# davide-coccomini/MINTIME-Multi-Identity-size-iNvariant-TIMEsformer-for-Video-Deepfake-Detection

Measured on AMD Instinct MI355X. Metric: clips/sec (8-frame, 2-identity, 224^2 crops) fwd+bwd, higher is better.
Workload: dtype f32; 1 GPU; config 3: EfficientNet-B0 + SizeInvariantTimeSformer(dim 512, depth 9, heads 8), B=32/GPU, 8 frames, 2 identities (identity-masked), 224x224 crops, random-init seeded weights (restored before every step), train-mode BN + drop-connect 0.2, step = fwd + BCE loss + bwd + SGD(lr .01, wd 1e-4); global_batch=32, frames=8, parallelism=dp1

## Files before the change

include/mintime_hip.h:

```cpp
#ifndef MINTIME_HIP_H
#define MINTIME_HIP_H
#include <stdint.h>
#ifdef __cplusplus
extern "C" {
#endif

#define MT_VERSION 121

int mt_version(void);
const char* mt_last_error(void);

int mt_set_deterministic(int on);
int mt_get_deterministic(void);
int mt_det_release(void* stream);
int mt_det_bn_sums(const float* x, const float* z, const float* mean_invstd, int64_t rows, int C, int mode, double* stats, void* stream);

typedef struct { int gin, gout, off; } mt_rowmap;

enum { MT_OP_NT = 0,
       MT_OP_NN = 1,
       MT_OP_TN = 2 };

enum { MT_PRO_NONE = 0, MT_PRO_BN_SWISH_GATE = 1, MT_PRO_BN_SWISH = 2, MT_PRO_AFFINE = 3,
       MT_PRO_BN_BWD = 4,
       MT_PRO_IM2COL = 5 };
enum { MT_BPRO_NONE = 0, MT_BPRO_BN_SWISH_GATE = 1, MT_BPRO_IM2COL = 2 };
enum { MT_EPI_STORE = 0, MT_EPI_BIAS_RES = 1, MT_EPI_GEGLU = 2, MT_EPI_STATS = 3, MT_EPI_ATOMIC = 4,
       MT_EPI_GEGLU_BWD = 5, MT_EPI_ACCUM = 6,
       MT_EPI_SE_RED = 7, MT_EPI_ACT_BWD = 8 };

typedef struct {
  int op, prologue, epilogue;
  const float* A; const float* B; float* C;
  int M, N, K;
  int64_t lda, ldb, ldc;
  mt_rowmap a_map, b_map, c_map;
  const float* bias;
  const float* R; int64_t ldr;
  const float* scale; const float* shift; const float* gate; int hw;
  float* C2; int64_t ldc2;
  double* stats; int stats_slots;
  int n_half;
  int split_k;
  const float* A2;
  int b_prologue; const float* b_scale; const float* b_shift; const float* b_gate; int b_hw;
  int conv_H, conv_W, conv_C, conv_Ho, conv_Wo, conv_k, conv_stride, conv_pad, conv_act;
  int conv_src_u8;
  float* col_sum;
  const void* b_planes;
  int64_t b_plane_stride;
  const float* e_scale; const float* e_shift;
  const float* e_gate; const float* e_dpool;
  const float* e_mi; int e_hw;
} mt_gemm_desc;

int mt_gemm(const mt_gemm_desc* d, void* stream);

int mt_gemm_set_split(int on);
int mt_gemm_get_split(void);

int mt_split_planes(const float* src, void* planes, int64_t n, void* stream);

int64_t mt_planes_elems(int rows, int cols);

int mt_split_planes_blk(const float* src, int64_t ld, int rows, int cols, void* planes, void* stream);

int mt_split_planes_blk_multi(const void* items, int count, int64_t total_blocks, void* stream);

int mt_bn_bwd_apply_planes(const float* du, const float* z, const float* kabc, void* planes, int rows, int C, void* stream);

typedef struct {
  int op;
  int epilogue;
  int M, N, K;
  const void* a_planes;
  const void* b_planes;
  float* C; int64_t ldc;
  const float* bias;
  const float* R; int64_t ldr;
  float* C2; int64_t ldc2;
  int n_half;
  float* col_sum;
  void* c_planes;
  int split_k;
  void* sk_workspace;
  int64_t sk_workspace_bytes;
  double* stats; int stats_slots;
} mt_gemm_planes_desc;

int mt_gemm_planes(const mt_gemm_planes_desc* d, void* stream);

int mt_mul_planes(const float* x, const float* m, void* planes, float* out, int rows, int cols, void* stream);
int mt_mul_add(const float* y, const float* m, const float* r, float* out, int64_t n, void* stream);
int mt_geglu_bwd(const float* dh, const float* m, const float* u, void* du_planes, float* du, int rows, int n_half, void* stream);
int64_t mt_gemm_planes_workspace_bytes(void);
int mt_gemm_planes_set_persist(int blocks_per_cu);


int mt_layernorm_fwd(const float* x, const float* gamma, const float* beta, float* y, float* stats,
                     int rows, int dim, float eps, void* y_planes, void* stream);

int mt_embed_fwd(float* x, const float* cls, const float* pos_emb, const float* size_emb,
                 const int64_t* positions, const int32_t* sizes, int B, int F, int n, int dim, int pos_rows, int size_rows,
                 int* err_flag, void* stream);

int mt_attn_fwd(const float* qkv, float* out, float* cls_att, const uint8_t* mask, const uint8_t* ident,
                int B, int H, int F, int n, int mode, float scale, void* out_planes, void* stream);

int mt_head_fwd(const float* x, const float* gamma, const float* beta, const float* w, const float* bias,
                float* logits, int B, int N, int dim, int classes, float eps, void* stream);


int mt_stem_conv_fwd(const void* x, int x_is_u8, const float* w, float* z, double* stats, int slots, int N, int H, int W,
                     void* stream);
int mt_stem_conv_fwd_valid(const void* x, int x_is_u8, const float* w, float* z, double* stats, int slots, int N, int H, int W,
                           void* stream);

int mt_dwconv_fwd(const float* zin, const float* scale, const float* shift, const float* w, float* zout,
                  double* stats, int slots, int N, int H, int W, int C, int k, int stride, int act, void* stream);
int mt_dwconv_rc_supported(int cin, int C, int k, int stride, int H);
int mt_dwconv_fwd_rc(const float* y, const float* we, int cin, const float* scale, const float* shift, const float* w, float* zout,
                     double* stats, int slots, int N, int H, int W, int C, int k, int stride, void* stream);
int mt_dwconv_fwd_planes(const float* zin, const float* scale, const float* shift, const float* w, void* planes, int N, int H,
                         int W, int C, int k, int stride, int act, void* stream);

int mt_bn_finalize(const double* stats, int slots, double count, const float* gamma, const float* beta,
                   float* running_mean, float* running_var, float* scale, float* shift, float* mean_invstd,
                   int C, float eps, float momentum, int training, void* stream);

int mt_se_pool_parts(int N, int HW, int C);
int mt_se_pool_fwd(const float* z, const float* scale, const float* shift, float* partial, int N, int HW, int C, int parts,
                   void* stream);

int mt_se_gate_fwd(const float* partial, int parts, const float* w1, const float* b1, const float* w2, const float* b2,
                   float* pooled, float* gate, float* hidden, int N, int C, int CS, void* stream);

int mt_bn_act_fwd(const float* z, const float* scale, const float* shift, const float* res, float* y,
                  int64_t rows, int C, int act, const float* rowscale, int rows_per_group, void* stream);

int mt_attn_aggregate(const float* space_att, const float* time_att, float* out, int BH, int N, int F,
                      float scale_factor, void* stream);

int mt_build_clip_inputs(const int* slots, const int* valid, const int* frames, const int* ratio, unsigned char* mask,
                         unsigned char* identities_mask, int* size_embedding, int64_t* positions, int B, int F,
                         int num_patches, int max_identities, int mask_mode, void* stream);


int mt_layernorm_bwd(const float* dy, const float* x, const float* stats, const float* gamma, float* dx,
                     float* dgamma, float* dbeta, int rows, int dim, int accumulate, float* dx_colsum, int skip_period,
                     const float* dx_in, void* stream);
int mt_layernorm_bwd_rows(const float* dy, const float* x, const float* stats, const float* gamma, float* dx, const float* dx_in,
                          int rows, int dim, void* dx_planes, void* stream);
int mt_layernorm_bwd_cols(const float* dy, const float* x, const float* stats, const float* dx_new, float* dgamma, float* dbeta,
                          float* dx_colsum, int skip_period, int rows, int dim, void* stream);

int mt_layernorm_bwd_rows_blocks(int rows);
int mt_layernorm_bwd_rows_sums(const float* dy, const float* x, const float* stats, const float* gamma, float* dx, const float* dx_in,
                               int rows, int dim, void* dx_planes, float* partials, int skip_period, void* stream);
int mt_layernorm_bwd_cols_reduce(const float* partials, int blocks, int dim, float* dgamma, float* dbeta, float* dx_colsum,
                                 void* stream);

int mt_colsum(const float* A, int64_t lda, mt_rowmap map, int M, int N, float* out, void* stream);

int mt_head_bwd(const float* dlogits, const float* x, const float* gamma, const float* beta, const float* w,
                float* dx, float* dgamma, float* dbeta, float* dw, float* dbias, int B, int N, int dim, int classes,
                float eps, void* stream);

int mt_embed_bwd(const float* dx, float* dcls, float* dpos_emb, float* dsize_emb, const int64_t* positions,
                 const int32_t* sizes, int B, int F, int n, int dim, int pos_rows, int size_rows, void* stream);

int mt_attn_bwd(const float* qkv, const float* dout, float* dqkv, const uint8_t* mask, const uint8_t* ident,
                int B, int H, int F, int n, int mode, float scale, void* dqkv_planes, void* stream);


int mt_bn_act_bwd(const float* din, const float* z, const float* scale, const float* shift,
                  const float* mean_invstd, const float* gate, const float* dpool, const float* rowscale,
                  float* dout, double* stats, int slots, int64_t rows, int C, int hw, int act, void* stream);

int mt_bn_bwd_finalize(const double* stats, int slots, double count, const float* gamma, const float* mean_invstd,
                       float* kabc, float* dgamma, float* dbeta, int C, int training, void* stream);

int mt_se_scratch_floats(int N, int C, int CS);
int mt_se_bwd(const float* da, const float* z, const float* scale, const float* shift, const float* gate,
              const float* hidden, const float* pooled, const float* w1, const float* w2, float* dgate,
              float* dpre2, float* dhid, float* dpooled, float* dw1, float* db1, float* dw2, float* db2, int N,
              int HW, int C, int CS, int parts, float* scratch, void* stream);

int mt_dwconv_bwd(const float* du, const float* z, const float* kabc, const float* w, const float* zin,
                  const float* scale_in, const float* shift_in, const float* mean_invstd_in, float* du_in,
                  double* stats_in, int slots, float* dw, int N, int H, int W, int C, int k, int stride,
                  int parts, int act, const float* res_pre, const float* res_post, void* stream);
int mt_dwconv_bwd_rc(const float* du, const float* z, const float* kabc, const float* w, const float* y, const float* we, int cin,
                     const float* scale_in, const float* shift_in, const float* mean_invstd_in, float* du_in, double* stats_in,
                     int slots, float* dw, int N, int H, int W, int C, int k, int stride, int parts, void* stream);
int mt_dwconv_bwd_res2(const float* du, const float* z, const float* kabc, const float* w, const float* zin,
                       const float* scale_in, const float* shift_in, const float* mean_invstd_in, float* du_in,
                       double* stats_in, int slots, float* dw, int N, int H, int W, int C, int k, int stride,
                       int parts, int act, const float* res_pre, const float* res_post, void* stream);

int mt_stem_conv_wgrad(const float* du, const float* z, const float* kabc, const void* x, int x_is_u8, float* dw, int N,
                       int H, int W, void* stream);
int mt_stem_conv_wgrad_valid(const float* du, const float* z, const float* kabc, const void* x, int x_is_u8, float* dw, int N,
                             int H, int W, void* stream);

int mt_conv1x1_wgrad_supported(int Cout, int Cin);
int mt_conv1x1_bwd_fused_supported(int Cout, int Cin);
int mt_se_stage_fused_supported(int Co, int C, int hw);
int mt_se_stage_fused(const float* du_p, const float* z_p, const float* kabc_p, const float* w_p, const float* z_d,
                      const float* scale_d, const float* shift_d, int mode, float* dgate, const float* gate, const float* dpooled,
                      const float* mean_invstd_d, float* du_d, double* stats, int slots, int64_t rows, int Co, int C, int hw,
                      void* stream);
int mt_conv1x1_bwd_fused(const float* du, const float* kabc, const float* x, const float* w, const float* res, float* dx,
                         float* dw, int64_t rows, int Cout, int Cin, void* stream);
int mt_conv1x1_wgrad(const float* du, const float* z, const float* kabc, const float* x, const float* sc, const float* sh,
                     const float* gate, int hw, float* dw, int64_t rows, int Cout, int Cin, void* stream);
int mt_conv1x1_wgrad_wide_supported(int Cout, int Cin);
int mt_conv1x1_wgrad_wide(const float* du, const float* z, const float* kabc, const float* x, const float* sc, const float* sh,
                          const float* gate, int hw, float* dw, int64_t rows, int Cout, int Cin, void* stream);

int mt_conv1x1_rows_supported(int Cin, int Cout, int amode);
int mt_conv1x1_rows_instance(int Cin, int Cout);
int mt_conv1x1_rows(const float* x, const float* x2, const float* w, int ldw, int w_transposed, const float* c0, const float* c1,
                    const float* c2, int hw, int amode, const float* res, float* out, double* stats, int slots, int64_t rows,
                    int Cin, int Cout, void* stream);

int mt_transpose_multi(const void* items, int count, int64_t total_tiles, void* stream);
int mt_bce_logits(const float* logits, const float* labels, float pos_weight, float* loss, float* dlogits, int n, void* stream);
int mt_sgd_multi(const void* items, int count, int64_t total_blocks, float lr, float weight_decay, void* stream);
int mt_adam_multi(const void* items, int count, int64_t total_blocks, float lr, float weight_decay, double beta1, double beta2,
                  float eps, float step_size, float bias_correction2_sqrt, int decoupled_weight_decay, void* stream);


int mt_conv_weight_pack(const float* w, float* out, int Co, int Ci, int k, int ld, int transpose, void* stream);
int mt_conv_weight_unpack_grad(const float* dwp, float* dw, int Co, int Ci, int k, int ld, void* stream);

int mt_maxpool_add_fwd(const float* z, const float* scale, const float* shift, const float* zs, const float* scale_s,
                       const float* shift_s, float* y, int N, int H, int W, int C, void* stream);
int mt_maxpool_bwd(const float* dy, const float* z, const float* scale, const float* shift, float* du, int N, int H,
                   int W, int C, void* stream);
int mt_maxpool_add_fwd_arg(const float* z, const float* scale, const float* shift, const float* zs, const float* scale_s,
                           const float* shift_s, float* y, uint8_t* arg, float* zmax, int N, int H, int W, int C, void* stream);
int mt_maxpool_bwd_arg(const float* dy, const uint8_t* arg, float* du, int N, int H, int W, int C, void* stream);
int mt_maxpool_bn_bwd_apply_planes(const float* dy, const uint8_t* arg, const float* z, const float* kabc, void* planes, int N, int H,
                                   int W, int C, void* stream);
int mt_bn_bwd_apply(const float* du, const float* z, const float* kabc, float* dz, int64_t rows, int C, void* stream);

int mt_bn_act_fwd_planes(const float* z, const float* scale, const float* shift, const float* res, float* y, int rows, int C, int act,
                         const float* rowscale, int rows_per_group, void* y_planes, void* stream);
int mt_bn_swish_gate_planes(const float* z, const float* scale, const float* shift, const float* gate, int hw, void* planes, int rows,
                            int C, void* stream);

int mt_baseline_head_fwd(const float* x, int layout, int n, int hw, int C, int m, const float* w1, const float* b1, const float* w2,
                         const float* b2, float* vc, float* pooled, float* part, float* logits, void* stream);
int mt_baseline_head_bwd(const float* dlogits, const float* pooled, const float* vc, int n, int hw, int C, int m, const float* w1,
                         const float* b1, const float* w2, float* dw1, float* db1, float* dw2, float* db2, float* dx, int layout,
                         float* work, void* stream);

typedef struct {
  int N, T, H, W, C;
  int To, Ho, Wo, K;
  int kt, kh, kw, st, sh, sw, pt, ph, pw;
  int64_t ldx, ldy;
} mt_conv3d_desc;
// ... 45 lines not shown
```

mintime-multi-identity-size-invariant-timesformer-for-video-deepfake-detection_amd/csrc/effnet_bwd.hip:

```cpp
#include "../../include/mintime_hip.h"
#include "common.hpp"
#include <type_traits>
#include "rc.hpp"
#include "det.hpp"
#include <stdlib.h>

using namespace mt;

namespace {

__device__ __forceinline__ float sigmoidf_(float x) { return __builtin_amdgcn_rcpf(1.0f + __expf(-x)); }
__device__ __forceinline__ float swishf_(float x) { return x * sigmoidf_(x); }
__device__ __forceinline__ float dswishf_(float u) { const float s = sigmoidf_(u); return s * (1.0f + u * (1.0f - s)); }

__device__ __forceinline__ float4 f4(float a, float b, float c, float d) { return make_float4(a, b, c, d); }
__device__ __forceinline__ float4 ld4(const float* p) { return *reinterpret_cast<const float4*>(p); }
__device__ __forceinline__ void st4(float* p, float4 v) { *reinterpret_cast<float4*>(p) = v; }
__device__ __forceinline__ float4 fma4(float4 a, float4 b, float4 c) {
  return f4(fmaf(a.x, b.x, c.x), fmaf(a.y, b.y, c.y), fmaf(a.z, b.z, c.z), fmaf(a.w, b.w, c.w));
}
__device__ __forceinline__ float4 mul4(float4 a, float4 b) { return f4(a.x * b.x, a.y * b.y, a.z * b.z, a.w * b.w); }
__device__ __forceinline__ float4 add4(float4 a, float4 b) { return f4(a.x + b.x, a.y + b.y, a.z + b.z, a.w + b.w); }

template <int ACT>
__device__ __forceinline__ float4 act4(float4 u) {
  if (ACT == 1) return f4(swishf_(u.x), swishf_(u.y), swishf_(u.z), swishf_(u.w));
  if (ACT == 2) return f4(fmaxf(u.x, 0.f), fmaxf(u.y, 0.f), fmaxf(u.z, 0.f), fmaxf(u.w, 0.f));
  return u;
}
template <int ACT>
__device__ __forceinline__ float4 dact4(float4 u) {
  if (ACT == 1) return f4(dswishf_(u.x), dswishf_(u.y), dswishf_(u.z), dswishf_(u.w));
  if (ACT == 2) return f4(u.x > 0.f ? 1.f : 0.f, u.y > 0.f ? 1.f : 0.f, u.z > 0.f ? 1.f : 0.f, u.w > 0.f ? 1.f : 0.f);
  return f4(1.f, 1.f, 1.f, 1.f);
}

__device__ __forceinline__ void reduce_stats(float* red, float4 s1, float4 s2, int cql, int pl, int CQB, int PB, int CQ,
                                             int C, double* stats, int slots) {
  if (pl < PB) {
    float* rr = red + (pl * CQB + cql) * 8;
    rr[0] = s1.x; rr[1] = s1.y; rr[2] = s1.z; rr[3] = s1.w;
    rr[4] = s2.x; rr[5] = s2.y; rr[6] = s2.z; rr[7] = s2.w;
  }
  __syncthreads();
  for (int i = threadIdx.x; i < CQB * 8; i += blockDim.x) {
    const int q = i >> 3, e = i & 7;
    const int cqq = blockIdx.y * CQB + q;
    if (cqq < CQ) {
      float v = 0.f;
      for (int p = 0; p < PB; ++p) v += red[(p * CQB + q) * 8 + e];
      const int ch = cqq * 4 + (e & 3), which = e >> 2;
      stat_add(stats + ((int64_t)(blockIdx.x % stat_slots(slots)) * 2 + which) * C + ch, stat_limb(slots, C), v);
    }
  }
}

__global__ __launch_bounds__(256) void bn_act_bwd_kernel(const float* __restrict__ din, const float* __restrict__ z,
                                                         const float* __restrict__ scale, const float* __restrict__ shift,
                                                         const float* __restrict__ mean_invstd, const float* __restrict__ gate,
                                                         const float* __restrict__ dpool, const float* __restrict__ rowscale,
                                                         float* __restrict__ dout, double* __restrict__ stats, int slots,
                                                         int64_t rows, int C, int hw, int act, int CQB, int PB) {
  extern __shared__ float red[];
  const int tid = threadIdx.x;
  const int cql = tid % CQB, pl = tid / CQB;
  const int CQ = C >> 2;
  const int cq = blockIdx.y * CQB + cql;
  float4 s1 = f4(0, 0, 0, 0), s2 = s1;
  if (pl < PB && cq < CQ) {
    const int c = cq * 4;
    const float4 sc = ld4(scale + c), sh = ld4(shift + c);
    const float4 mean = ld4(mean_invstd + c), istd = ld4(mean_invstd + C + c);
    const float inv_hw = 1.0f / (float)hw;
    for (int64_t r = (int64_t)blockIdx.x * PB + pl; r < rows; r += (int64_t)gridDim.x * PB) {
      const int n = (int)(r / hw);
      float4 d = ld4(din + r * C + c);
      const float4 zz = ld4(z + r * C + c);
      if (gate) {
        const float4 g = ld4(gate + (int64_t)n * C + c), dp = ld4(dpool + (int64_t)n * C + c);
        d = f4(fmaf(d.x, g.x, dp.x * inv_hw), fmaf(d.y, g.y, dp.y * inv_hw), fmaf(d.z, g.z, dp.z * inv_hw), fmaf(d.w, g.w, dp.w * inv_hw));
      }
      if (rowscale) { const float rs = rowscale[n]; d = f4(d.x * rs, d.y * rs, d.z * rs, d.w * rs); }
      if (act == 1) {
        const float4 u = fma4(zz, sc, sh);
        d = f4(d.x * dswishf_(u.x), d.y * dswishf_(u.y), d.z * dswishf_(u.z), d.w * dswishf_(u.w));
      } else if (act == 2) {
        const float4 u = fma4(zz, sc, sh);
        d = f4(u.x > 0.f ? d.x : 0.f, u.y > 0.f ? d.y : 0.f, u.z > 0.f ? d.z : 0.f, u.w > 0.f ? d.w : 0.f);
      }
      if (dout) st4(dout + r * C + c, d);
      const float4 xh = f4((zz.x - mean.x) * istd.x, (zz.y - mean.y) * istd.y, (zz.z - mean.z) * istd.z, (zz.w - mean.w) * istd.w);
      s1 = add4(s1, d);
      s2 = fma4(d, xh, s2);
    }
  }
  reduce_stats(red, s1, s2, cql, pl, CQB, PB, CQ, C, stats, slots);
}

__global__ __launch_bounds__(256) void bn_bwd_finalize_kernel(const double* __restrict__ stats, int slots, double count,
                                                              const float* __restrict__ gamma, const float* __restrict__ mean_invstd,
                                                              float* __restrict__ kabc, float* __restrict__ dgamma,
                                                              float* __restrict__ dbeta, int C, int training) {
  __shared__ double red[8][32][2];
  const int cl = threadIdx.x & 31, sg = threadIdx.x >> 5;
  const int c = blockIdx.x * 32 + cl;
  double a = 0.0, b = 0.0;
  if (c < C)
    for (int i = sg; i < stat_slots(slots); i += 8) {
      a += stat_get(stats + ((int64_t)i * 2) * C + c, stat_limb(slots, C));
      b += stat_get(stats + ((int64_t)i * 2 + 1) * C + c, stat_limb(slots, C));
    }
  red[sg][cl][0] = a; red[sg][cl][1] = b;
  __syncthreads();
  if (sg != 0 || c >= C) return;
  double s1 = 0.0, s2 = 0.0;
#pragma unroll
  for (int g = 0; g < 8; ++g) { s1 += red[g][cl][0]; s2 += red[g][cl][1]; }
  const float mean = mean_invstd[c], istd = mean_invstd[C + c];
  const float ka = gamma[c] * istd;
  float kb = 0.f, kc = 0.f;
  if (training) {
    const float c1 = (float)(s1 / count), c2 = (float)(s2 / count);
    kb = -ka * c2 * istd;
    kc = ka * c2 * istd * mean - ka * c1;
  }
  kabc[c] = ka; kabc[C + c] = kb; kabc[2 * C + c] = kc;
  if (dgamma) dgamma[c] += (float)s2;
  if (dbeta) dbeta[c] += (float)s1;
}

__global__ __launch_bounds__(256) void se_bwd_reduce_kernel(const float* __restrict__ da, const float* __restrict__ z,
                                                            const float* __restrict__ scale, const float* __restrict__ shift,
                                                            float* __restrict__ dgate, int HW, int C, int CQB, int PB) {
  extern __shared__ float red[];
  const int tid = threadIdx.x;
  const int cql = tid % CQB, pl = tid / CQB;
  const int cq = blockIdx.y * CQB + cql;
  const int CQ = C >> 2;
  const int n = blockIdx.x;
  float4 s = f4(0, 0, 0, 0);
  if (pl < PB && cq < CQ) {
    const float4 sc = ld4(scale + cq * 4), sh = ld4(shift + cq * 4);
    const int64_t base = (int64_t)n * HW * C + cq * 4;
    const int per = (HW + gridDim.z - 1) / gridDim.z;
    const int p_lo = blockIdx.z * per, p_hi = min(HW, p_lo + per);
    int p = p_lo + pl;
    for (; p + PB < p_hi; p += 2 * PB) {
      const float4 z0 = ld4(z + base + (int64_t)p * C), z1 = ld4(z + base + (int64_t)(p + PB) * C);
      const float4 d0 = ld4(da + base + (int64_t)p * C), d1 = ld4(da + base + (int64_t)(p + PB) * C);
      const float4 u0 = fma4(z0, sc, sh), u1 = fma4(z1, sc, sh);
      s = f4(fmaf(d0.x, swishf_(u0.x), s.x), fmaf(d0.y, swishf_(u0.y), s.y), fmaf(d0.z, swishf_(u0.z), s.z), fmaf(d0.w, swishf_(u0.w), s.w));
      s = f4(fmaf(d1.x, swishf_(u1.x), s.x), fmaf(d1.y, swishf_(u1.y), s.y), fmaf(d1.z, swishf_(u1.z), s.z), fmaf(d1.w, swishf_(u1.w), s.w));
    }
    for (; p < p_hi; p += PB) {
      const float4 u = fma4(ld4(z + base + (int64_t)p * C), sc, sh);
      const float4 d = ld4(da + base + (int64_t)p * C);
      s = f4(fmaf(d.x, swishf_(u.x), s.x), fmaf(d.y, swishf_(u.y), s.y), fmaf(d.z, swishf_(u.z), s.z), fmaf(d.w, swishf_(u.w), s.w));
    }
  }
  if (pl < PB) st4(red + (pl * CQB + cql) * 4, s);
  __syncthreads();
  if (pl == 0 && cq < CQ) {
    float4 t = f4(0, 0, 0, 0);
    for (int p = 0; p < PB; ++p) t = add4(t, ld4(red + (p * CQB + cql) * 4));
    float* out = dgate + (int64_t)n * C + cq * 4;
    if (gridDim.z == 1) {
      st4(out, t);
    } else {
      atomicAdd(out + 0, t.x); atomicAdd(out + 1, t.y); atomicAdd(out + 2, t.z); atomicAdd(out + 3, t.w);
    }
  }
}

constexpr int SE_SLAB = 128;
constexpr int SE_JW = 12;
__device__ __forceinline__ void se_load_slab(float* slab, const float* __restrict__ src, int count, int CS, int tid) {
  const int pitch = CS + 1;
  const float inv_cs = 1.0f / (float)CS;
  for (int e0 = tid; e0 < count; e0 += 256 * 8) {
    float v[8];
#pragma unroll
    for (int u = 0; u < 8; ++u) v[u] = src[min(e0 + 256 * u, count - 1)];
#pragma unroll
    for (int u = 0; u < 8; ++u) {
      const int e = e0 + 256 * u;
      const int r = (int)(((float)e + 0.5f) * inv_cs);
      if (e < count) slab[r * pitch + (e - r * CS)] = v[u];
    }
  }
}

__global__ __launch_bounds__(256) void se_bwd_slab_kernel(const float* __restrict__ dgate, const float* __restrict__ gate,
                                                          const float* __restrict__ w2, float* __restrict__ dpre2,
                                                          float* __restrict__ dh_part, int C, int CS) {
  extern __shared__ float sm[];
  float* dp2 = sm;
  float* slab = sm + SE_SLAB;
  const int n = blockIdx.x, sl = blockIdx.y, c0 = sl * SE_SLAB, tid = threadIdx.x, lane = tid & 63, wave = tid >> 6;
  const int rows = min(SE_SLAB, C - c0), pitch = CS + 1;
  if (tid < SE_SLAB) {
    float v = 0.f;
    if (tid < rows) {
      const float g = gate[(int64_t)n * C + c0 + tid];
      v = dgate[(int64_t)n * C + c0 + tid] * g * (1.0f - g);
      dpre2[(int64_t)n * C + c0 + tid] = v;
    }
    dp2[tid] = v;
  }
  se_load_slab(slab, w2 + (int64_t)c0 * CS, rows * CS, CS, tid);
  __syncthreads();
  const float d0 = dp2[lane], d1 = dp2[lane + 64];
// ... 189 lines not shown
        const float4 v = act4<ACT>(fma4(zraw, sc, sh));
        const bool ok = (pre_ok >> i) & 1u;
        st4(a_t + (iy * IWP + ix) * CC + f_q * 4, f4(ok ? v.x : 0.f, ok ? v.y : 0.f, ok ? v.z : 0.f, ok ? v.w : 0.f));
      }
    }
#pragma unroll
    for (int i = 0; i < ND; ++i) {
      const int pix = slot + i * NSL;
      if (pix < T * T) {
        const float4 v = fma4(ka, pdu[i], fma4(kb, pz[i], kc));
        const bool ok = (pd_ok >> i) & 1u;
        st4(dz_t + pix * CC + cq * 4, f4(ok ? v.x : 0.f, ok ? v.y : 0.f, ok ? v.z : 0.f, ok ? v.w : 0.f));
      }
    }
    __syncthreads();
    if (tile + tile_stride < ntiles) fetch(tile + tile_stride);
    if (worker) {
      for (int p = ps; p < T * T; p += PS) {
        const int oy = p / T, ox = p - oy * T;
        const float4 d = ld4(dz_t + p * CC + cq * 4);
        const float* arow = a_t + ((oy * S + kh) * IWP + ox * S) * CC + cq * 4;
#pragma unroll
        for (int kw = 0; kw < K; ++kw) acc[kw] = fma4(d, ld4(arow + kw * CC), acc[kw]);
      }
    }
  }
  __syncthreads();
  float* red = lds;
  if (worker) {
#pragma unroll
    for (int kw = 0; kw < K; ++kw) st4(red + (((ps * K + kh) * CQN + cq) * K + kw) * 4, acc[kw]);
  }
  __syncthreads();
  if (tid < K * CQN * K) {
    const int kw = tid % K, q = (tid / K) % CQN, khh = tid / (CQN * K);
    float4 t = f4(0, 0, 0, 0);
    for (int g = 0; g < PS; ++g) t = add4(t, ld4(red + (((g * K + khh) * CQN + q) * K + kw) * 4));
    const int c = c0 + q * 4, tp = khh * K + kw;
    if (det.vals) {
      const int rk = (int)tile0, jb = q * 4 * K * K + tp;
      det_put(det, chunk_id, rk, jb, t.x); det_put(det, chunk_id, rk, jb + K * K, t.y);
      det_put(det, chunk_id, rk, jb + 2 * K * K, t.z); det_put(det, chunk_id, rk, jb + 3 * K * K, t.w);
      if (rk == 0 && tid == 0) det_base(det, chunk_id, (int64_t)c0 * K * K);
    } else {
      atomicAdd(dw + (c + 0) * K * K + tp, t.x); atomicAdd(dw + (c + 1) * K * K + tp, t.y);
      atomicAdd(dw + (c + 2) * K * K + tp, t.z); atomicAdd(dw + (c + 3) * K * K + tp, t.w);
    }
  }
}

template <int K, int S, int T, int ACT, int CC, int RC = 0>
int launch_dw_wgrad_tiled(const float* du, const float* z, const float* kabc, const float* zin, const float* scale_in,
                          const float* shift_in, float* dw, int N, int H, int W, int C, int Ho, int Wo, hipStream_t s,
                          const float* we = nullptr) {
  constexpr int IH = (T - 1) * S + K;
  constexpr int IWP = IH | 1;
  constexpr int CQN = CC / 4;
  constexpr int PS = (256 / CQN) / K;
  size_t lds = (size_t)(IH * IWP * CC + T * T * CC) * sizeof(float);
  const size_t red = (size_t)PS * K * CQN * K * 4 * sizeof(float);
  if (red > lds) lds = red;
  const int chunks = C / CC;
  const int64_t ntiles = (int64_t)N * ((Ho + T - 1) / T) * ((Wo + T - 1) / T);
  const unsigned bx = xcd_chunk_grid(chunks, ntiles, 4096);
  auto k = dwconv_wgrad_tiled_kernel<K, S, T, ACT, CC, RC>;
  if (lds > 48 * 1024) {
    hipError_t e = ensure_dynamic_lds(reinterpret_cast<const void*>(k), lds);
    if (e != hipSuccess) return fail(MT_ERR_LAUNCH, "mt_dwconv_bwd: cannot reserve %zu B of LDS: %s", lds, hipGetErrorString(e));
  }
  DetScope det(s, chunks, (int)((bx >> 3) / chunks) * 8, CC * K * K);
  hipLaunchKernelGGL(k, dim3(bx), dim3(256), lds, s, du, z, kabc, zin, scale_in, shift_in, dw, N, H, W, C, Ho, Wo, det.log, we);
  const int rc = check_launch("mt_dwconv_bwd(weight, tiled)");
  return rc ? rc : det.reduce_f32(dw);
}

thread_local int g_res_stride = 1;

template <int K, int S, int T, int ACT, int CC, bool WG = false, int RC = 0>
__global__ __launch_bounds__(256) void dwconv_dgrad_tiled_kernel(
    const float* __restrict__ du, const float* __restrict__ z, const float* __restrict__ kabc, const float* __restrict__ w,
    const float* __restrict__ zin, const float* __restrict__ scale_in, const float* __restrict__ shift_in,
    const float* __restrict__ mi_in, float* __restrict__ du_in, double* __restrict__ stats, int slots, int N, int H, int W,
    int C, int Ho, int Wo, const float* __restrict__ res_pre, const float* __restrict__ res_post, float* __restrict__ dw,
    int res_stride, const float* __restrict__ we) {
  static_assert(RC == 0 || CC == 16, "the recompute yields 16-channel chunks");
  constexpr int P = S == 1 ? (K - 1) / 2 : (K - 2) / 2;
  constexpr int CQN = CC / 4, NSLOT = 256 / CQN;
  constexpr int OT = (T - 1 + K - 1) / S + 2;
  constexpr int OTP = OT | 1;
  extern __shared__ __attribute__((aligned(16))) float lds[];
  const int tid = threadIdx.x;
  const int cq = tid % CQN, slot = tid / CQN;
  int chunk_id; int64_t tile0, tile_stride;
  xcd_chunk_tile(C / CC, chunk_id, tile0, tile_stride);
  const int c0 = chunk_id * CC;
  const int ty_n = (H + T - 1) / T, tx_n = (W + T - 1) / T;
  const int64_t ntiles = (int64_t)N * ty_n * tx_n;
  const int c = c0 + cq * 4;
  const float4 sc = ld4(scale_in + c), sh = ld4(shift_in + c);
  const float4 mean = mi_in ? ld4(mi_in + c) : f4(0, 0, 0, 0), istd = mi_in ? ld4(mi_in + C + c) : f4(0, 0, 0, 0);
  constexpr bool WLDS = K > 3 || S == 1;
  float* w_t = lds + OT * OTP * CC;
  float* z_t = w_t + (WLDS ? K * K * CC : 0);
  constexpr int RCW = RC ? RC : 8;
  constexpr int NLZ = (T * T + 63) / 64;
  const int lane = tid & 63;
  const int f_q = lane >> 4, f_slot = (tid >> 6) * 16 + (lane & 15);
  RcFrag<RCW> wfrag, ypre[RC ? NLZ : 1];
  if constexpr (RC > 0) rc_load<RCW>(wfrag, we + (int64_t)(c0 + (lane & 15)) * RC, lane);
  float4 wt[WLDS ? 1 : K * K];
  if constexpr (WLDS) {
    if (slot == 0)
      for (int i = 0; i < K * K; ++i)
        st4(w_t + i * CC + cq * 4, f4(w[(c + 0) * K * K + i], w[(c + 1) * K * K + i], w[(c + 2) * K * K + i], w[(c + 3) * K * K + i]));
  } else {
#pragma unroll
    for (int i = 0; i < K * K; ++i)
      wt[i] = f4(w[(c + 0) * K * K + i], w[(c + 1) * K * K + i], w[(c + 2) * K * K + i], w[(c + 3) * K * K + i]);
  }
  const float4 ka = ld4(kabc + c), kb = ld4(kabc + C + c), kc = ld4(kabc + 2 * C + c);
  float4 s1 = f4(0, 0, 0, 0), s2 = s1;
  float* a_t = z_t + (RC ? T * T * CC : 0);
  constexpr int PS2 = NSLOT / K;
  const int r2 = tid / CQN, kh2 = r2 % K, ps2 = r2 / K;
  float4 wacc[WG ? K : 1];
#pragma unroll
  for (int i = 0; i < (WG ? K : 1); ++i) wacc[i] = f4(0, 0, 0, 0);
  constexpr int ND = (OT * OT + NSLOT - 1) / NSLOT;
  static_assert(ND <= 32, "validity mask is 32 bits");
  float4 pdu[ND], pz[ND];
  unsigned pd_ok = 0;
  auto lows = [&](int64_t tile, int& n, int& ih0, int& iw0, int& oh_lo, int& ow_lo) {
    int ty, tx;
    tile_nyx(tile, ty_n, tx_n, n, ty, tx);
    ih0 = ty * T; iw0 = tx * T;
    const int nh = ih0 + P - (K - 1), nw = iw0 + P - (K - 1);
    oh_lo = nh >= 0 ? (nh + S - 1) / S : -((-nh) / S);
    ow_lo = nw >= 0 ? (nw + S - 1) / S : -((-nw) / S);
  };
  auto fetch = [&](int64_t tile) {
    int n, ih0, iw0, oh_lo, ow_lo;
    lows(tile, n, ih0, iw0, oh_lo, ow_lo);
    const int64_t obase = (int64_t)n * Ho * Wo * C + c;
    pd_ok = 0;
#pragma unroll
    for (int i = 0; i < ND; ++i) {
      const int pix = slot + i * NSLOT;
      const int oy = pix / OT, ox = pix - oy * OT;
      const int oh = oh_lo + oy, ow = ow_lo + ox;
      if (pix < OT * OT && oh >= 0 && oh < Ho && ow >= 0 && ow < Wo) pd_ok |= 1u << i;
      const int64_t off = obase + ((int64_t)min(max(oh, 0), Ho - 1) * Wo + min(max(ow, 0), Wo - 1)) * C;
      pdu[i] = ld4(du + off);
      pz[i] = ld4(z + off);
    }
    if constexpr (RC > 0) {
      const float* img = zin + (int64_t)n * H * W * RC;
#pragma unroll
      for (int i = 0; i < NLZ; ++i) {
        const int pix = f_slot + i * 64;
        const int iy = pix / T, ix = pix - iy * T;
        rc_load<RCW>(ypre[i], img + ((int64_t)min(ih0 + iy, H - 1) * W + min(iw0 + ix, W - 1)) * RC, lane);
      }
    }
  };
  int64_t tile = tile0;
  if (tile < ntiles) fetch(tile);
  for (; tile < ntiles; tile += tile_stride) {
// ... 65 lines not shown
          auto taps = [&](auto PH, auto PW) {
            constexpr int ph_ = decltype(PH)::value, pw_ = decltype(PW)::value;
#pragma unroll
            for (int kh = ph_; kh < K; kh += 2) {
#pragma unroll
              for (int kw = pw_; kw < K; kw += 2) tap(kh, kw, oyb - (kh - ph_) / 2, oxb - (kw - pw_) / 2);
              __builtin_amdgcn_sched_barrier(0);
            }
          };
          using I0 = std::integral_constant<int, 0>;
          using I1 = std::integral_constant<int, 1>;
          if (ph == 0) { if (pw == 0) taps(I0{}, I0{}); else taps(I0{}, I1{}); }
          else { if (pw == 0) taps(I1{}, I0{}); else taps(I1{}, I1{}); }
        }
        const bool r_on = res_stride == 1 || !((ih | iw) & 1);
        const int64_t roff = res_stride == 1 ? off : (((int64_t)n * ((H + 1) >> 1) + (ih >> 1)) * ((W + 1) >> 1) + (iw >> 1)) * C + c;
        if (res_pre && r_on) acc = add4(acc, ld4(res_pre + roff));
        float4 d = mul4(acc, dact4<ACT>(u));
        if (res_post && r_on) d = add4(d, ld4(res_post + roff));
        st4(du_in + off, d);
        const float4 xh = f4((zz.x - mean.x) * istd.x, (zz.y - mean.y) * istd.y, (zz.z - mean.z) * istd.z, (zz.w - mean.w) * istd.w);
        s1 = add4(s1, d);
        s2 = fma4(d, xh, s2);
      }
    }
    if constexpr (WG) {
      __syncthreads();
      if (ps2 < PS2) {
        const int ohb = ih0 + P - kh2;
#pragma unroll 1
        for (int p = ps2; p < T * T; p += PS2) {
          const int iy = p / T, ix = p - iy * T;
          const int ohn = ohb + iy;
          if (S == 2 && (ohn & 1)) continue;
          const float4 a = ld4(a_t + p * CC + cq * 4);
          const float* drow = lds + (((ohn >> (S - 1)) - oh_lo) * OTP) * CC + cq * 4;
          const int owb = iw0 + ix + P;
          if constexpr (S == 1) {
#pragma unroll
            for (int kw = 0; kw < K; ++kw) wacc[kw] = fma4(ld4(drow + (owb - kw - ow_lo) * CC), a, wacc[kw]);
          } else {
            const int pw = owb & 1, oxb = ((owb - pw) >> 1) - ow_lo;
            if (pw == 0) {
#pragma unroll
              for (int kw = 0; kw < K; kw += 2) wacc[kw] = fma4(ld4(drow + (oxb - kw / 2) * CC), a, wacc[kw]);
            } else {
#pragma unroll
              for (int kw = 1; kw < K; kw += 2) wacc[kw] = fma4(ld4(drow + (oxb - (kw - 1) / 2) * CC), a, wacc[kw]);
            }
          }
        }
      }
    }
  }
  if constexpr (WG) {
    __syncthreads();
    float* red = lds;
    if (ps2 < PS2) {
#pragma unroll
      for (int kw = 0; kw < K; ++kw) st4(red + (((ps2 * K + kh2) * CQN + cq) * K + kw) * 4, wacc[kw]);
    }
    __syncthreads();
    if (tid < K * CQN * K) {
      const int kw = tid % K, q = (tid / K) % CQN, khh = tid / (CQN * K);
      float4 t = f4(0, 0, 0, 0);
      for (int g = 0; g < PS2; ++g) t = add4(t, ld4(red + (((g * K + khh) * CQN + q) * K + kw) * 4));
      const int ch = c0 + q * 4, tp = khh * K + kw;
      atomicAdd(dw + (ch + 0) * K * K + tp, t.x); atomicAdd(dw + (ch + 1) * K * K + tp, t.y);
      atomicAdd(dw + (ch + 2) * K * K + tp, t.z); atomicAdd(dw + (ch + 3) * K * K + tp, t.w);
    }
  }
  if (!stats) return;
  __syncthreads();
  float* rr = lds + tid * 8;
  rr[0] = s1.x; rr[1] = s1.y; rr[2] = s1.z; rr[3] = s1.w; rr[4] = s2.x; rr[5] = s2.y; rr[6] = s2.z; rr[7] = s2.w;
  __syncthreads();
  if (tid < CQN * 8) {
    const int q = tid >> 3, e = tid & 7;
    float v = 0.f;
    for (int sl = 0; sl < NSLOT; ++sl) v += lds[(sl * CQN + q) * 8 + e];
    const int ch = c0 + q * 4 + (e & 3), which = e >> 2;
    stat_add(stats + ((int64_t)(blockIdx.x % stat_slots(slots)) * 2 + which) * C + ch, stat_limb(slots, C), v);
  }
}

template <int K, int S, int T, int ACT, int CC, bool WG = false, int RC = 0>
int launch_dw_dgrad_tiled(const float* du, const float* z, const float* kabc, const float* w, const float* zin,
                          const float* scale_in, const float* shift_in, const float* mi_in, float* du_in, double* stats, int slots,
                          int N, int H, int W, int C, int Ho, int Wo, const float* res_pre, const float* res_post, hipStream_t s,
                          float* dw = nullptr, const float* we = nullptr) {
  constexpr int OT = (T - 1 + K - 1) / S + 2;
  constexpr int OTP = OT | 1;
  constexpr int CQN = CC / 4, NSLOT = 256 / CQN;
  size_t lds = (size_t)(OT * OTP * CC + ((K > 3 || S == 1) ? K * K * CC : 0) + (RC ? T * T * CC : 0) + (WG ? T * T * CC : 0)) * sizeof(float);
  if (lds < 256 * 8 * sizeof(float)) lds = 256 * 8 * sizeof(float);
  if (WG && lds < (size_t)(NSLOT / K) * K * CQN * K * 4 * sizeof(float)) lds = (size_t)(NSLOT / K) * K * CQN * K * 4 * sizeof(float);
  const int chunks = C / CC;
  const int64_t ntiles = (int64_t)N * ((H + T - 1) / T) * ((W + T - 1) / T);
  const unsigned bx = xcd_chunk_grid(chunks, ntiles, WG ? 4096 : 8192);
  auto kfn = dwconv_dgrad_tiled_kernel<K, S, T, ACT, CC, WG, RC>;
  if (lds > 48 * 1024) {
    hipError_t e = ensure_dynamic_lds(reinterpret_cast<const void*>(kfn), lds);
    if (e != hipSuccess) return fail(MT_ERR_LAUNCH, "mt_dwconv_bwd: cannot reserve %zu B of LDS: %s", lds, hipGetErrorString(e));
  }
  hipLaunchKernelGGL(kfn, dim3(bx), dim3(256), lds, s, du, z, kabc, w, zin,
                     scale_in, shift_in, mi_in, du_in, stats, slots != 0 ? slots : 1, N, H, W, C, Ho, Wo, res_pre, res_post, dw,
                     g_res_stride, we);
  return check_launch(WG ? "mt_dwconv_bwd(data + weight, fused)" : "mt_dwconv_bwd(data, tiled)");
}

template <int K, int S, int ACT>
int launch_dw_bwd_tiled_any(const float* du, const float* z, const float* kabc, const float* w, const float* zin, const float* scale_in,
                            const float* shift_in, const float* mi_in, float* du_in, double* stats, int slots, float* dw, int N, int H,
                            int W, int C, int Ho, int Wo, int parts, const float* res_pre, const float* res_post, hipStream_t s) {
  int rc = 0;
  static const int t7_mask = getenv("MT_DW_T7") ? atoi(getenv("MT_DW_T7")) : 0;
  const bool t14o = Ho >= 14 && !(t7_mask & 4), t14i = H >= 14 && !(t7_mask & 2);
  if (parts == 3) {
    if (C % 16 == 0) return t14i ? launch_dw_dgrad_tiled<K, S, 14, ACT, 16, true>(du, z, kabc, w, zin, scale_in, shift_in, mi_in, du_in, stats, slots, N, H, W, C, Ho, Wo, res_pre, res_post, s, dw)
                                 : launch_dw_dgrad_tiled<K, S, 7, ACT, 16, true>(du, z, kabc, w, zin, scale_in, shift_in, mi_in, du_in, stats, slots, N, H, W, C, Ho, Wo, res_pre, res_post, s, dw);
    return t14i ? launch_dw_dgrad_tiled<K, S, 14, ACT, 8, true>(du, z, kabc, w, zin, scale_in, shift_in, mi_in, du_in, stats, slots, N, H, W, C, Ho, Wo, res_pre, res_post, s, dw)
                : launch_dw_dgrad_tiled<K, S, 7, ACT, 8, true>(du, z, kabc, w, zin, scale_in, shift_in, mi_in, du_in, stats, slots, N, H, W, C, Ho, Wo, res_pre, res_post, s, dw);
  }
  if (parts & 1) {
    if (C % 16 == 0) rc = t14o ? launch_dw_wgrad_tiled<K, S, 14, ACT, 16>(du, z, kabc, zin, scale_in, shift_in, dw, N, H, W, C, Ho, Wo, s)
                               : launch_dw_wgrad_tiled<K, S, 7, ACT, 16>(du, z, kabc, zin, scale_in, shift_in, dw, N, H, W, C, Ho, Wo, s);
    else rc = t14o ? launch_dw_wgrad_tiled<K, S, 14, ACT, 8>(du, z, kabc, zin, scale_in, shift_in, dw, N, H, W, C, Ho, Wo, s)
                   : launch_dw_wgrad_tiled<K, S, 7, ACT, 8>(du, z, kabc, zin, scale_in, shift_in, dw, N, H, W, C, Ho, Wo, s);
    if (rc) return rc;
  }
  if (parts & 2) {
    if (C % 16 == 0) rc = t14i ? launch_dw_dgrad_tiled<K, S, 14, ACT, 16>(du, z, kabc, w, zin, scale_in, shift_in, mi_in, du_in, stats, slots, N, H, W, C, Ho, Wo, res_pre, res_post, s)
                               : launch_dw_dgrad_tiled<K, S, 7, ACT, 16>(du, z, kabc, w, zin, scale_in, shift_in, mi_in, du_in, stats, slots, N, H, W, C, Ho, Wo, res_pre, res_post, s);
    else rc = t14i ? launch_dw_dgrad_tiled<K, S, 14, ACT, 8>(du, z, kabc, w, zin, scale_in, shift_in, mi_in, du_in, stats, slots, N, H, W, C, Ho, Wo, res_pre, res_post, s)
                   : launch_dw_dgrad_tiled<K, S, 7, ACT, 8>(du, z, kabc, w, zin, scale_in, shift_in, mi_in, du_in, stats, slots, N, H, W, C, Ho, Wo, res_pre, res_post, s);
  }
  return rc;
}

__global__ __launch_bounds__(256) void stem_wgrad_kernel(const float* __restrict__ du, const float* __restrict__ z,
                                                         const float* __restrict__ kabc, const void* __restrict__ xv, int x_u8,
                                                         float* __restrict__ dw, int N, int H, int W, int Ho, int Wo, int pad0,
                                                         const DetLog det) {
  const float* x = reinterpret_cast<const float*>(xv);
  const uint8_t* xb = reinterpret_cast<const uint8_t*>(xv);
  constexpr int CO = 32, TP = 64, TAPS = 27;
  __shared__ float dzt[TP][CO + 1];
  __shared__ float xt[TP][TAPS + 1];
  const int tid = threadIdx.x;
  const int co = tid & 31, g = tid >> 5;
  const float ka = kabc[co], kb = kabc[CO + co], kc = kabc[2 * CO + co];
  float acc[4] = {0.f, 0.f, 0.f, 0.f};
  const int64_t total = (int64_t)N * Ho * Wo;
  const int64_t ntiles = (total + TP - 1) / TP;
  for (int64_t tile = blockIdx.x; tile < ntiles; tile += gridDim.x) {
    const int64_t p0 = tile * TP;
    __syncthreads();
    for (int i = tid; i < TP * CO; i += 256) {
      const int p = i >> 5, c2 = i & 31;
      const int64_t pix = p0 + p;
      float v = 0.f;
      if (pix < total) v = fmaf(kabc[c2], du[pix * CO + c2], fmaf(kabc[CO + c2], z[pix * CO + c2], kabc[2 * CO + c2]));
      dzt[p][c2] = v;
    }
    for (int i = tid; i < TP * TAPS; i += 256) {
      const int p = i / TAPS, tp = i - p * TAPS;
      const int ci = tp % 3, kk = tp / 3, kw = kk % 3, kh = kk / 3;
      const int64_t pix = p0 + p;
      float v = 0.f;
      if (pix < total) {
        const int ow = (int)(pix % Wo);
        const int64_t t = pix / Wo;
        const int oh = (int)(t % Ho), n = (int)(t / Ho);
        const int ih = oh * 2 + kh - pad0, iw = ow * 2 + kw - pad0;
        if (ih >= 0 && ih < H && iw >= 0 && iw < W) {
          const int64_t off = (((int64_t)n * H + ih) * W + iw) * 3 + ci;
          v = x_u8 ? (float)xb[off] : x[off];
        }
      }
      xt[p][tp] = v;
    }
    __syncthreads();
#pragma unroll 8
    for (int p = 0; p < TP; ++p) {
      const float d = dzt[p][co];
#pragma unroll
      for (int i = 0; i < 4; ++i) {
        const int tp = g + 8 * i;
        if (tp < TAPS) acc[i] = fmaf(d, xt[p][tp], acc[i]);
      }
    }
  }
  (void)ka; (void)kb; (void)kc;
#pragma unroll
  for (int i = 0; i < 4; ++i) {
    const int tp = g + 8 * i;
    if (tp < TAPS) {
      const int ci = tp % 3, kk = tp / 3, kw = kk % 3, kh = kk / 3;
      if (det.vals) det_put(det, 0, blockIdx.x, ((co * 3 + ci) * 3 + kh) * 3 + kw, acc[i]);
      else atomicAdd(dw + ((co * 3 + ci) * 3 + kh) * 3 + kw, acc[i]);
    }
  }
}

int pick_cqb(int CQ) {
  int best = 1;
  for (int d = 1; d <= 64 && d <= CQ; ++d)
    if (CQ % d == 0) best = d;
  return best;
}

template <int K, int S>
int launch_dw_bwd(const float* du, const float* z, const float* kabc, const float* w, const float* zin, const float* scale_in,
                  const float* shift_in, const float* mi_in, float* du_in, double* stats, int slots, float* dw, int N, int H,
                  int W, int C, int parts, int act, const float* res_pre, const float* res_post, hipStream_t s) {
  const int Ho = (H + S - 1) / S, Wo = (W + S - 1) / S;
  if (C % 8 != 0) return fail(MT_ERR_UNSUPPORTED, "mt_dwconv_bwd: channel count %d is not a multiple of 8", C);
  if (act == 1) return launch_dw_bwd_tiled_any<K, S, 1>(du, z, kabc, w, zin, scale_in, shift_in, mi_in, du_in, stats, slots, dw, N, H, W, C, Ho, Wo, parts, res_pre, res_post, s);
  if (act == 2) return launch_dw_bwd_tiled_any<K, S, 2>(du, z, kabc, w, zin, scale_in, shift_in, mi_in, du_in, stats, slots, dw, N, H, W, C, Ho, Wo, parts, res_pre, res_post, s);
  return launch_dw_bwd_tiled_any<K, S, 0>(du, z, kabc, w, zin, scale_in, shift_in, mi_in, du_in, stats, slots, dw, N, H, W, C, Ho, Wo, parts, res_pre, res_post, s);
}

}

extern "C" int mt_bn_act_bwd(const float* din, const float* z, const float* scale, const float* shift,
                             const float* mean_invstd, const float* gate, const float* dpool, const float* rowscale,
                             float* dout, double* stats, int slots, int64_t rows, int C, int hw, int act, void* stream) {
  if (!din || !z || !scale || !shift || !mean_invstd || !stats) return fail(MT_ERR_ARG, "mt_bn_act_bwd: null pointer");
  if ((gate == nullptr) != (dpool == nullptr)) return fail(MT_ERR_ARG, "mt_bn_act_bwd: gate and dpool go together");
  if (C & 3) return fail(MT_ERR_ARG, "mt_bn_act_bwd: C %% 4 != 0");
  const int CQ = C / 4, CQB = pick_cqb(CQ), PB = 256 / CQB;
  int64_t nb = (rows + PB - 1) / PB;
  const int64_t cap = 4096 / (CQ / CQB) > 0 ? 4096 / (CQ / CQB) : 1;
  if (nb > cap) nb = cap;
  hipLaunchKernelGGL(bn_act_bwd_kernel, dim3((unsigned)nb, CQ / CQB), dim3(CQB * PB), (size_t)PB * CQB * 8 * sizeof(float),
                     (hipStream_t)stream, din, z, scale, shift, mean_invstd, gate, dpool, rowscale, dout, stats,
                     slots != 0 ? slots : 1, rows, C, hw > 0 ? hw : 1, act, CQB, PB);
  return check_launch("mt_bn_act_bwd");
}

extern "C" int mt_bn_bwd_finalize(const double* stats, int slots, double count, const float* gamma, const float* mean_invstd,
                                  float* kabc, float* dgamma, float* dbeta, int C, int training, void* stream) {
  if (!stats || !gamma || !mean_invstd || !kabc) return fail(MT_ERR_ARG, "mt_bn_bwd_finalize: null pointer");
  hipLaunchKernelGGL(bn_bwd_finalize_kernel, dim3((C + 31) / 32), dim3(256), 0, (hipStream_t)stream, stats, slots, count, gamma,
                     mean_invstd, kabc, dgamma, dbeta, C, training);
  return check_launch("mt_bn_bwd_finalize");
}

static int se_adjoint(const float* dgate, const float* gate, const float* hidden, const float* w1, const float* w2, float* dpre2,
                      float* dhid, float* dpooled, float* scratch, int N, int C, int CS, hipStream_t s) {
  const int slabs = (C + SE_SLAB - 1) / SE_SLAB;
  hipLaunchKernelGGL(se_bwd_slab_kernel, dim3(N, slabs), dim3(256), (size_t)(SE_SLAB + SE_SLAB * (CS + 1)) * sizeof(float), s, dgate, gate,
                     w2, dpre2, scratch, C, CS);
  int rc = check_launch("mt_se_bwd(slab)");
  if (rc) return rc;
  hipLaunchKernelGGL(se_bwd_finish_kernel, dim3(N, (C + 255) / 256), dim3(256), (size_t)CS * sizeof(float), s, scratch, slabs, hidden, w1,
                     dhid, dpooled, C, CS);
  return check_launch("mt_se_bwd(finish)");
}

extern "C" int mt_se_scratch_floats(int N, int C, int CS) { return N * ((C + SE_SLAB - 1) / SE_SLAB) * CS; }

extern "C" int mt_se_bwd(const float* da, const float* z, const float* scale, const float* shift, const float* gate,
                         const float* hidden, const float* pooled, const float* w1, const float* w2, float* dgate,
                         float* dpre2, float* dhid, float* dpooled, float* dw1, float* db1, float* dw2, float* db2, int N,
                         int HW, int C, int CS, int parts_mask, float* scratch, void* stream) {
  if (((parts_mask & 1) && (!da || !z || !scale || !shift)) || !gate || !hidden || !pooled || !w1 || !w2 || !dgate || !dpre2 || !dhid ||
      !dpooled || !dw1 || !db1 || !dw2 || !db2 || ((parts_mask & 5) && !scratch))
    return fail(MT_ERR_ARG, "mt_se_bwd: null pointer");
  if (C & 3) return fail(MT_ERR_ARG, "mt_se_bwd: C %% 4 != 0");
  if (CS > CS_MAX) return fail(MT_ERR_UNSUPPORTED, "mt_se_bwd: squeeze width %d > %d", CS, CS_MAX);
  hipStream_t s = (hipStream_t)stream;
  const int CQ = C / 4, CQB = pick_cqb(CQ), PB = 256 / CQB;
  int rc = 0;
  if (parts_mask & 1) {
  int parts = 1;
  while ((int64_t)N * (CQ / CQB) * parts < 2048 && HW / (parts * 2) >= PB * 16) parts *= 2;
  if (det_enabled()) parts = 1;
  if (parts > 1 && hipMemsetAsync(dgate, 0, (size_t)N * C * sizeof(float), s) != hipSuccess)
    return fail(MT_ERR_LAUNCH, "mt_se_bwd: memset failed");
  hipLaunchKernelGGL(se_bwd_reduce_kernel, dim3(N, CQ / CQB, parts), dim3(CQB * PB), (size_t)PB * CQB * 4 * sizeof(float), s, da, z,
                     scale, shift, dgate, HW, C, CQB, PB);
  rc = check_launch("mt_se_bwd(reduce)");
  if (rc) return rc;
  rc = se_adjoint(dgate, gate, hidden, w1, w2, dpre2, dhid, dpooled, scratch, N, C, CS, s);
  if (rc) return rc;
  }
  if (parts_mask & 4) {
    rc = se_adjoint(dgate, gate, hidden, w1, w2, dpre2, dhid, dpooled, scratch, N, C, CS, s);
    if (rc) return rc;
  }
  if (!(parts_mask & 2)) return 0;
  int ipb = 64;
  while (ipb > 16 && (int64_t)((C + 63) / 64) * ((N + ipb - 1) / ipb) < 128) ipb >>= 1;
  if (det_enabled()) ipb = N;
  hipLaunchKernelGGL(se_wgrad_kernel, dim3((C + 63) / 64, (N + ipb - 1) / ipb), dim3(256), 0, s, dpre2, dhid, hidden, pooled, dw1,
                     db1, dw2, db2, N, C, CS, ipb);
  return check_launch("mt_se_bwd(wgrad)");
}

extern "C" int mt_dwconv_bwd(const float* du, const float* z, const float* kabc, const float* w, const float* zin,
                             const float* scale_in, const float* shift_in, const float* mean_invstd_in, float* du_in,
                             double* stats_in, int slots, float* dw, int N, int H, int W, int C, int k, int stride,
                             int parts, int act, const float* res_pre, const float* res_post, void* stream) {
  if (!du || !z || !kabc || !zin || !scale_in || !shift_in) return fail(MT_ERR_ARG, "mt_dwconv_bwd: null pointer");
  if ((parts & 1) && !dw) return fail(MT_ERR_ARG, "mt_dwconv_bwd: weight part needs dw");
  if ((parts & 2) && (!w || !du_in)) return fail(MT_ERR_ARG, "mt_dwconv_bwd: data part needs w and du_in");
  if ((parts & 2) && ((stats_in == nullptr) != (mean_invstd_in == nullptr))) return fail(MT_ERR_ARG, "mt_dwconv_bwd: stats_in and mean_invstd_in go together");
  if (stride == 2 && ((H & 1) || (W & 1))) return fail(MT_ERR_UNSUPPORTED, "mt_dwconv_bwd: stride 2 needs even H, W");
  hipStream_t s = (hipStream_t)stream;
  if (k == 3 && stride == 1) return launch_dw_bwd<3, 1>(du, z, kabc, w, zin, scale_in, shift_in, mean_invstd_in, du_in, stats_in, slots, dw, N, H, W, C, parts, act, res_pre, res_post, s);
  if (k == 3 && stride == 2) return launch_dw_bwd<3, 2>(du, z, kabc, w, zin, scale_in, shift_in, mean_invstd_in, du_in, stats_in, slots, dw, N, H, W, C, parts, act, res_pre, res_post, s);
  if (k == 5 && stride == 1) return launch_dw_bwd<5, 1>(du, z, kabc, w, zin, scale_in, shift_in, mean_invstd_in, du_in, stats_in, slots, dw, N, H, W, C, parts, act, res_pre, res_post, s);
  if (k == 5 && stride == 2) return launch_dw_bwd<5, 2>(du, z, kabc, w, zin, scale_in, shift_in, mean_invstd_in, du_in, stats_in, slots, dw, N, H, W, C, parts, act, res_pre, res_post, s);
  return fail(MT_ERR_UNSUPPORTED, "mt_dwconv_bwd: k=%d stride=%d unsupported", k, stride);
}

#define MT_DW_RC_INSTANCES(X) X(3, 2, 16, 14) X(3, 1, 24, 14) X(5, 2, 24, 7)
extern "C" int mt_dwconv_rc_supported(int cin, int C, int k, int stride, int H);

// ... 63 lines not shown
```

mintime-multi-identity-size-invariant-timesformer-for-video-deepfake-detection_amd/csrc/effnet_fwd.hip:

```cpp
#include "../../include/mintime_hip.h"
#include "common.hpp"
#include "planes.hpp"
#include "rc.hpp"
#include <stdlib.h>

using namespace mt;

#ifndef MT_DW_FWD_ROLL5
#define MT_DW_FWD_ROLL5 1
#endif

namespace {

__device__ __forceinline__ float sigmoidf_(float x) { return __builtin_amdgcn_rcpf(1.0f + __expf(-x)); }
__device__ __forceinline__ float swishf_(float x) { return x * sigmoidf_(x); }

__device__ __forceinline__ float4 bn_swish4(float4 z, float4 sc, float4 sh) {
  float4 a;
  a.x = swishf_(fmaf(z.x, sc.x, sh.x)); a.y = swishf_(fmaf(z.y, sc.y, sh.y));
  a.z = swishf_(fmaf(z.z, sc.z, sh.z)); a.w = swishf_(fmaf(z.w, sc.w, sh.w));
  return a;
}

__device__ __forceinline__ void atomic_add_f64(double* p, double v) { atomicAdd(p, v); }

template <int ACT>
__device__ __forceinline__ float4 act_affine4(float4 z, float4 sc, float4 sh) {
  float4 a = make_float4(fmaf(z.x, sc.x, sh.x), fmaf(z.y, sc.y, sh.y), fmaf(z.z, sc.z, sh.z), fmaf(z.w, sc.w, sh.w));
  if (ACT == 1) { a.x = swishf_(a.x); a.y = swishf_(a.y); a.z = swishf_(a.z); a.w = swishf_(a.w); }
  if (ACT == 2) { a.x = fmaxf(a.x, 0.f); a.y = fmaxf(a.y, 0.f); a.z = fmaxf(a.z, 0.f); a.w = fmaxf(a.w, 0.f); }
  return a;
}

template <int K, int S, int T, int ACT, int CC, int RC = 0>
__global__ __launch_bounds__(256) void dwconv_tiled_kernel(const float* __restrict__ zin, const float* __restrict__ scale,
                                                           const float* __restrict__ shift, const float* __restrict__ w,
                                                           float* __restrict__ zout, double* __restrict__ stats, int slots,
                                                           int N, int H, int W, int C, int Ho, int Wo, int pad0, PlaneRef po,
                                                           const float* __restrict__ we) {
  static_assert(RC == 0 || CC == 16, "the recompute yields 16-channel chunks");
  constexpr int CQN = CC / 4, NSLOT = 256 / CQN;
  constexpr int IH = (T - 1) * S + K;
  constexpr int IWP = IH | 1;
  extern __shared__ __attribute__((aligned(16))) float lds[];
  const int tid = threadIdx.x;
  const int cq = tid % CQN, slot = tid / CQN;
  int chunk_id; int64_t tile0, tile_stride;
  xcd_chunk_tile(C / CC, chunk_id, tile0, tile_stride);
  const int c0 = chunk_id * CC;
  const int ty_n = (Ho + T - 1) / T, tx_n = (Wo + T - 1) / T;
  const int64_t ntiles = (int64_t)N * ty_n * tx_n;
  constexpr bool WLDS = K > 3;
  constexpr bool ROLL5 = MT_DW_FWD_ROLL5;
  float* w_t = lds + IH * IWP * CC;
  float4 wt[WLDS ? 1 : K * K];
  {
    const int c = c0 + cq * 4;
    if constexpr (WLDS) {
      if (slot == 0)
        for (int i = 0; i < K * K; ++i)
          *reinterpret_cast<float4*>(w_t + i * CC + cq * 4) =
              make_float4(w[(c + 0) * K * K + i], w[(c + 1) * K * K + i], w[(c + 2) * K * K + i], w[(c + 3) * K * K + i]);
    } else {
#pragma unroll
      for (int i = 0; i < K * K; ++i)
        wt[i] = make_float4(w[(c + 0) * K * K + i], w[(c + 1) * K * K + i], w[(c + 2) * K * K + i], w[(c + 3) * K * K + i]);
    }
  }
  float4 s1 = make_float4(0.f, 0.f, 0.f, 0.f), s2 = s1;
  constexpr int NSL = 256 / CQN;
  constexpr int NL = (IH * IH + NSL - 1) / NSL;
  static_assert(NL <= 32, "validity mask is 32 bits");
  const int lane = tid & 63;
  const int f_q = RC ? (lane >> 4) : cq, f_slot = RC ? ((tid >> 6) * 16 + (lane & 15)) : slot;
  const float4 sc_q = *reinterpret_cast<const float4*>(scale + c0 + f_q * 4);
  const float4 sh_q = *reinterpret_cast<const float4*>(shift + c0 + f_q * 4);
  constexpr int RCW = RC ? RC : 8;
  RcFrag<RCW> wfrag, ypre[RC ? NL : 1];
  if constexpr (RC > 0) rc_load<RCW>(wfrag, we + (int64_t)(c0 + (lane & 15)) * RC, lane);
  float4 pre[RC ? 1 : NL];
  unsigned pre_ok = 0;
  auto fetch = [&](int64_t tile) {
    int n, ty, tx;
    tile_nyx(tile, ty_n, tx_n, n, ty, tx);
    const int ih0 = ty * T * S - pad0, iw0 = tx * T * S - pad0;
    const float* img = RC ? zin + (int64_t)n * H * W * RC : zin + (int64_t)n * H * W * C + c0 + cq * 4;
    pre_ok = 0;
#pragma unroll
    for (int i = 0; i < NL; ++i) {
      const int pix = f_slot + i * NSL;
      const int iy = pix / IH, ix = pix - iy * IH;
      const int ih = ih0 + iy, iw = iw0 + ix;
      if (pix < IH * IH && ih >= 0 && ih < H && iw >= 0 && iw < W) pre_ok |= 1u << i;
      const int ihc = min(max(ih, 0), H - 1), iwc = min(max(iw, 0), W - 1);
      if constexpr (RC > 0) rc_load<RCW>(ypre[i], img + ((int64_t)ihc * W + iwc) * RC, lane);
      else pre[i] = *reinterpret_cast<const float4*>(img + ((int64_t)ihc * W + iwc) * C);
    }
  };
  int64_t tile = tile0;
  if (tile < ntiles) fetch(tile);
  for (; tile < ntiles; tile += tile_stride) {
    int n, ty, tx;
    tile_nyx(tile, ty_n, tx_n, n, ty, tx);
    const int oh0 = ty * T, ow0 = tx * T;
    __syncthreads();
#pragma unroll
    for (int i = 0; i < NL; ++i) {
      const int pix = f_slot + i * NSL;
      float4 zraw;
      if constexpr (RC > 0) zraw = rc_mma<RCW>(wfrag, ypre[i]);
      else zraw = pre[i];
      if (pix < IH * IH) {
        const int iy = pix / IH, ix = pix - iy * IH;
        const float4 a = act_affine4<ACT>(zraw, sc_q, sh_q);
        const bool ok = (pre_ok >> i) & 1u;
        *reinterpret_cast<float4*>(lds + (iy * IWP + ix) * CC + f_q * 4) =
            make_float4(ok ? a.x : 0.f, ok ? a.y : 0.f, ok ? a.z : 0.f, ok ? a.w : 0.f);
      }
    }
    __syncthreads();
    if (tile + tile_stride < ntiles) fetch(tile + tile_stride);
    for (int p = slot; p < T * T; p += NSLOT) {
      const int oy = p / T, ox = p - oy * T;
      const int oh = oh0 + oy, ow = ow0 + ox;
      if (oh < Ho && ow < Wo) {
        float4 acc = make_float4(0.f, 0.f, 0.f, 0.f);
        const float* base = lds + ((oy * S) * IWP + ox * S) * CC + cq * 4;
        auto row = [&](int kh) {
#pragma unroll
          for (int kw = 0; kw < K; ++kw) {
            const float4 a = *reinterpret_cast<const float4*>(base + (kh * IWP + kw) * CC);
            float4 ww;
            if constexpr (WLDS) ww = *reinterpret_cast<const float4*>(w_t + (kh * K + kw) * CC + cq * 4);
            else ww = wt[kh * K + kw];
            acc.x = fmaf(a.x, ww.x, acc.x); acc.y = fmaf(a.y, ww.y, acc.y);
            acc.z = fmaf(a.z, ww.z, acc.z); acc.w = fmaf(a.w, ww.w, acc.w);
          }
        };
        if constexpr (WLDS && ROLL5) {
#pragma unroll 1
          for (int kh = 0; kh < K; ++kh) row(kh);
        } else {
#pragma unroll
          for (int kh = 0; kh < K; ++kh) row(kh);
        }
        if (po.p) {
          const int row = (n * Ho + oh) * Wo + ow, c = c0 + cq * 4;
          planes_store4(po, row, c, acc.x, acc.y, acc.z, acc.w);
          if (c + 4 == C)
            for (int cz = C; cz < po.cb16 * 16; cz += 4) planes_store4(po, row, cz, 0.f, 0.f, 0.f, 0.f);
        } else {
          *reinterpret_cast<float4*>(zout + (((int64_t)n * Ho + oh) * Wo + ow) * C + c0 + cq * 4) = acc;
        }
        s1.x += acc.x; s1.y += acc.y; s1.z += acc.z; s1.w += acc.w;
        s2.x += acc.x * acc.x; s2.y += acc.y * acc.y; s2.z += acc.z * acc.z; s2.w += acc.w * acc.w;
      }
    }
  }
  if (stats) {
    __syncthreads();
    float* rr = lds + tid * 8;
    rr[0] = s1.x; rr[1] = s1.y; rr[2] = s1.z; rr[3] = s1.w; rr[4] = s2.x; rr[5] = s2.y; rr[6] = s2.z; rr[7] = s2.w;
    __syncthreads();
    if (tid < CQN * 8) {
      const int q = tid >> 3, e = tid & 7;
      float v = 0.f;
      for (int sl = 0; sl < NSLOT; ++sl) v += lds[(sl * CQN + q) * 8 + e];
      const int ch = c0 + q * 4 + (e & 3), which = e >> 2;
      stat_add(stats + ((int64_t)(blockIdx.x % stat_slots(slots)) * 2 + which) * C + ch, stat_limb(slots, C), v);
    }
  }
}

template <int K, int S, int T, int ACT, int CC, int RC = 0>
int launch_dw_tiled(const float* zin, const float* scale, const float* shift, const float* w, float* zout, double* stats, int slots,
                    int N, int H, int W, int C, int Ho, int Wo, int pad0, hipStream_t s, const PlaneRef& po,
                    const float* we = nullptr) {
  constexpr int IH = (T - 1) * S + K;
  constexpr int IWP = IH | 1;
  size_t lds = (size_t)(IH * IWP * CC + (K > 3 ? K * K * CC : 0)) * sizeof(float);
  if (lds < 256 * 8 * sizeof(float)) lds = 256 * 8 * sizeof(float);
  const int chunks = C / CC;
  const int64_t ntiles = (int64_t)N * ((Ho + T - 1) / T) * ((Wo + T - 1) / T);
  const unsigned bx = xcd_chunk_grid(chunks, ntiles, 8192);
  auto k = dwconv_tiled_kernel<K, S, T, ACT, CC, RC>;
  if (lds > 48 * 1024) {
    hipError_t e = ensure_dynamic_lds(reinterpret_cast<const void*>(k), lds);
    if (e != hipSuccess) return fail(MT_ERR_LAUNCH, "mt_dwconv_fwd: cannot reserve %zu B of LDS: %s", lds, hipGetErrorString(e));
  }
  hipLaunchKernelGGL(k, dim3(bx), dim3(256), lds, s, zin, scale, shift, w, zout, stats, slots != 0 ? slots : 1, N, H,
                     W, C, Ho, Wo, pad0, po, we);
  return check_launch("mt_dwconv_fwd(tiled)");
}

template <int K, int S, int ACT>
int launch_dw_tiled_any(const float* zin, const float* scale, const float* shift, const float* w, float* zout, double* stats,
                        int slots, int N, int H, int W, int C, int Ho, int Wo, int pad0, hipStream_t s, const PlaneRef& po) {
  static const int t7_mask = getenv("MT_DW_T7") ? atoi(getenv("MT_DW_T7")) : 0;
  const bool t14 = Ho >= 14 && !(t7_mask & 1);
  if (C % 16 == 0) {
    if (t14) return launch_dw_tiled<K, S, 14, ACT, 16>(zin, scale, shift, w, zout, stats, slots, N, H, W, C, Ho, Wo, pad0, s, po);
    return launch_dw_tiled<K, S, 7, ACT, 16>(zin, scale, shift, w, zout, stats, slots, N, H, W, C, Ho, Wo, pad0, s, po);
  }
  if (t14) return launch_dw_tiled<K, S, 14, ACT, 8>(zin, scale, shift, w, zout, stats, slots, N, H, W, C, Ho, Wo, pad0, s, po);
  return launch_dw_tiled<K, S, 7, ACT, 8>(zin, scale, shift, w, zout, stats, slots, N, H, W, C, Ho, Wo, pad0, s, po);
}

__global__ __launch_bounds__(256) void bn_finalize_kernel(const double* __restrict__ stats, int slots, double count,
                                                          const float* __restrict__ gamma, const float* __restrict__ beta,
                                                          float* __restrict__ running_mean, float* __restrict__ running_var,
                                                          float* __restrict__ scale, float* __restrict__ shift,
                                                          float* __restrict__ mean_invstd, int C, float eps, float momentum,
                                                          int training) {
  __shared__ double red[8][32][2];
  const int cl = threadIdx.x & 31, sg = threadIdx.x >> 5;
  const int c = blockIdx.x * 32 + cl;
  if (training) {
    double s = 0.0, q = 0.0;
    if (c < C)
      for (int i = sg; i < stat_slots(slots); i += 8) {
        s += stat_get(stats + ((int64_t)i * 2) * C + c, stat_limb(slots, C));
        q += stat_get(stats + ((int64_t)i * 2 + 1) * C + c, stat_limb(slots, C));
      }
    red[sg][cl][0] = s; red[sg][cl][1] = q;
    __syncthreads();
  }
  if (sg != 0 || c >= C) return;
  float mean, var;
  if (training) {
    double s = 0.0, q = 0.0;
#pragma unroll
    for (int g = 0; g < 8; ++g) { s += red[g][cl][0]; q += red[g][cl][1]; }
    const double m = s / count;
    double v = q / count - m * m;
    if (v < 0.0) v = 0.0;
    mean = (float)m; var = (float)v;
    if (running_mean) {
      const double unb = count > 1.0 ? v * count / (count - 1.0) : v;
      running_mean[c] = (1.f - momentum) * running_mean[c] + momentum * mean;
      running_var[c] = (1.f - momentum) * running_var[c] + momentum * (float)unb;
    }
  } else {
    mean = running_mean[c]; var = running_var[c];
  }
  const float invstd = 1.0f / sqrtf(var + eps);
  const float sc = gamma[c] * invstd;
  scale[c] = sc;
  shift[c] = beta[c] - mean * sc;
  if (mean_invstd) { mean_invstd[c] = mean; mean_invstd[C + c] = invstd; }
}

__global__ __launch_bounds__(256) void se_pool_kernel(const float* __restrict__ z, const float* __restrict__ scale,
                                                      const float* __restrict__ shift, float* __restrict__ pooled,
                                                      int HW, int C, int CQB, int PB) {
  extern __shared__ float red[];
  const int tid = threadIdx.x;
  const int cql = tid % CQB, pl = tid / CQB;
  const int cq = blockIdx.y * CQB + cql;
  const int CQ = C >> 2;
  const int n = blockIdx.x;
  const int per = (HW + gridDim.z - 1) / gridDim.z;
  const int p_lo = blockIdx.z * per, p_hi = min(HW, p_lo + per);
  float4 s = make_float4(0.f, 0.f, 0.f, 0.f);
  if (pl < PB && cq < CQ) {
    const float4 sc = *reinterpret_cast<const float4*>(scale + cq * 4);
    const float4 sh = *reinterpret_cast<const float4*>(shift + cq * 4);
    const float* base = z + (int64_t)n * HW * C + cq * 4;
    int p = p_lo + pl;
    for (; p + 3 * PB < p_hi; p += 4 * PB) {
      const float4 v0 = *reinterpret_cast<const float4*>(base + (int64_t)p * C);
      const float4 v1 = *reinterpret_cast<const float4*>(base + (int64_t)(p + PB) * C);
      const float4 v2 = *reinterpret_cast<const float4*>(base + (int64_t)(p + 2 * PB) * C);
      const float4 v3 = *reinterpret_cast<const float4*>(base + (int64_t)(p + 3 * PB) * C);
      const float4 a0 = bn_swish4(v0, sc, sh), a1 = bn_swish4(v1, sc, sh), a2 = bn_swish4(v2, sc, sh), a3 = bn_swish4(v3, sc, sh);
      s.x += (a0.x + a1.x) + (a2.x + a3.x); s.y += (a0.y + a1.y) + (a2.y + a3.y);
      s.z += (a0.z + a1.z) + (a2.z + a3.z); s.w += (a0.w + a1.w) + (a2.w + a3.w);
    }
    for (; p < p_hi; p += PB) {
      const float4 a = bn_swish4(*reinterpret_cast<const float4*>(base + (int64_t)p * C), sc, sh);
      s.x += a.x; s.y += a.y; s.z += a.z; s.w += a.w;
    }
  }
  if (pl < PB) *reinterpret_cast<float4*>(red + (pl * CQB + cql) * 4) = s;
  __syncthreads();
  if (pl == 0 && cq < CQ) {
    float4 t = make_float4(0.f, 0.f, 0.f, 0.f);
    for (int q = 0; q < PB; ++q) {
      const float4 v = *reinterpret_cast<const float4*>(red + (q * CQB + cql) * 4);
      t.x += v.x; t.y += v.y; t.z += v.z; t.w += v.w;
    }
    const float inv = 1.0f / (float)HW;
    float* out = pooled + ((int64_t)n * gridDim.z + blockIdx.z) * C + cq * 4;
    *reinterpret_cast<float4*>(out) = make_float4(t.x * inv, t.y * inv, t.z * inv, t.w * inv);
  }
}

constexpr int SE_SLAB = 128;
__global__ __launch_bounds__(256) void se_hidden_kernel(const float* __restrict__ partial, int parts, const float* __restrict__ w1,
                                                        const float* __restrict__ b1, float* __restrict__ pooled,
                                                        float* __restrict__ hidden, int C, int CS) {
  extern __shared__ float pv[];
  const int n = blockIdx.x, tid = threadIdx.x, lane = tid & 63, wave = tid >> 6;
  for (int i = tid; i < C; i += 256) {
    float v = 0.f;
    for (int q = 0; q < parts; ++q) v += partial[((int64_t)n * parts + q) * C + i];
    pv[i] = v;
    if (pooled && blockIdx.y == 0) pooled[(int64_t)n * C + i] = v;
  }
  __syncthreads();
  const int j0 = (blockIdx.y * 4 + wave) * 4;
  if (j0 >= CS) return;
  const float* r0 = w1 + (int64_t)min(j0 + 0, CS - 1) * C;
  const float* r1 = w1 + (int64_t)min(j0 + 1, CS - 1) * C;
  const float* r2 = w1 + (int64_t)min(j0 + 2, CS - 1) * C;
  const float* r3 = w1 + (int64_t)min(j0 + 3, CS - 1) * C;
  float a0 = 0.f, a1 = 0.f, a2 = 0.f, a3 = 0.f;
#pragma unroll 2
  for (int i = lane; i < C; i += 64) {
    const float w0 = r0[i], w1v = r1[i], w2v = r2[i], w3 = r3[i], pvi = pv[i];
    a0 = fmaf(w0, pvi, a0); a1 = fmaf(w1v, pvi, a1); a2 = fmaf(w2v, pvi, a2); a3 = fmaf(w3, pvi, a3);
  }
#pragma unroll
  for (int o = 32; o > 0; o >>= 1) {
    a0 += __shfl_xor(a0, o); a1 += __shfl_xor(a1, o); a2 += __shfl_xor(a2, o); a3 += __shfl_xor(a3, o);
  }
  if (lane < 4 && j0 + lane < CS) {
    const float a = lane == 0 ? a0 : (lane == 1 ? a1 : (lane == 2 ? a2 : a3));
    hidden[(int64_t)n * CS + j0 + lane] = a + b1[j0 + lane];
  }
}

__device__ __forceinline__ void se_load_slab(float* slab, const float* __restrict__ src, int count, int CS, int tid) {
// ... 196 lines not shown
```

mintime-multi-identity-size-invariant-timesformer-for-video-deepfake-detection_amd/csrc/gen_plan.py:

```python
#!/usr/bin/env python3
import re
import sys


def prototypes(text):
    text = re.sub(r"/\*.*?\*/", " ", text, flags=re.S)
    out = []
    for m in re.finditer(r"^(int|int64_t)\s+(mt_\w+)\s*\(([^;{]*?)\)\s*;", text, flags=re.M | re.S):
        ret, name, params = m.group(1), m.group(2), " ".join(m.group(3).split())
        if params in ("void", ""):
            continue
        ps = []
        for p in params.split(","):
            p = p.strip()
            mm = re.match(r"^(.*?)(\w+)$", p)
            ps.append((mm.group(1).strip(), mm.group(2)))
        out.append((ret, name, ps))
    return out


SKIP = {"mt_plan_run", "mt_plan_fork"}


def main(header, rename_h, thunks_inc):
    protos = [p for p in prototypes(open(header).read())
              if p[2][-1] == ("void*", "stream") and p[0] == "int" and p[1] not in SKIP]
    with open(rename_h, "w") as f:
        f.write("// generated by gen_plan.py from include/mintime_hip.h -- do not edit\n#pragma once\n")
        for _, name, _ in protos:
            f.write(f"#define {name} mti_{name[3:]}\n")
    with open(thunks_inc, "w") as f:
        f.write("// generated by gen_plan.py from include/mintime_hip.h -- do not edit\n")
        for _, name, ps in protos:
            inner = "mti_" + name[3:]
            decl = ", ".join(f"{t} {n}" for t, n in ps)
            f.write(f'extern "C" int {inner}({decl});\n')
            f.write(f'extern "C" int {name}({decl}) {{\n')
            call, pre = [], []
            for t, n in ps:
                if re.match(r"^const mt_\w+_desc\s*\*$", t):
                    pre.append(f"    const auto {n}_v = *{n};\n")
                    call.append(f"&{n}_v")
                else:
                    call.append(n)
            f.write(f"  const int rc = {inner}({', '.join(n for _, n in ps)});\n")
            f.write("  if (rc == 0) if (mt::Plan* p_ = mt::plan_recording()) {\n")
            f.write("".join(pre))
            f.write(f"    p_->add(stream, [=]() {{ return {inner}({', '.join(call)}); }});\n")
            f.write("  }\n  return rc;\n}\n")
    return 0


if __name__ == "__main__":
    sys.exit(main(*sys.argv[1:4]))
```

mintime-multi-identity-size-invariant-timesformer-for-video-deepfake-detection_amd/csrc/plan.hip:

```cpp
#include <hip/hip_runtime.h>
#include <stdint.h>
#include <functional>
#include <vector>

#include "../../include/mintime_hip.h"
#include "common.hpp"

namespace mt {

struct PlanOp {
  std::function<int()> fn;
  int tag;
  double work;
  void* stream;
};

struct ProbeHit {
  int tag;
  double work;
  hipEvent_t e0, e1;
};

struct Plan {
  std::vector<PlanOp> ops;
  std::vector<hipEvent_t> fork_events;
  std::vector<hipEvent_t> free_timing;
  std::vector<ProbeHit> hits;
  int device = 0;
  bool recording = false;

  void add(void* stream, std::function<int()> fn);
};

static thread_local Plan* g_recording = nullptr;
static thread_local int g_next_tag = 0;
static thread_local double g_next_work = 0.0;

Plan* plan_recording() { return g_recording; }

void Plan::add(void* stream, std::function<int()> fn) {
  ops.push_back(PlanOp{std::move(fn), g_next_tag, g_next_work, stream});
  g_next_tag = 0;
  g_next_work = 0.0;
}

static hipEvent_t ring_event() {
  static thread_local hipEvent_t ring[64] = {nullptr};
  static thread_local int ring_dev[64];
  static thread_local unsigned next = 0;
  const unsigned i = next++ & 63;
  int dev = 0;
  (void)hipGetDevice(&dev);
  if (ring[i] && ring_dev[i] != dev) {
    (void)hipEventDestroy(ring[i]);
    ring[i] = nullptr;
  }
  if (!ring[i]) {
    if (hipEventCreateWithFlags(&ring[i], hipEventDisableTiming) != hipSuccess) return nullptr;
    ring_dev[i] = dev;
  }
  return ring[i];
}

static int fork_with(hipEvent_t ev, void* from, void* to) {
  hipError_t e = hipEventRecord(ev, (hipStream_t)from);
  if (e == hipSuccess) e = hipStreamWaitEvent((hipStream_t)to, ev, 0);
  if (e != hipSuccess) return fail(MT_ERR_LAUNCH, "mt_plan_fork: %s", hipGetErrorString(e));
  return 0;
}

}

using mt::fail;
using mt::Plan;

#include "plan_thunks.inc"

extern "C" int mt_plan_create(mt_plan** out) {
  if (!out) return fail(mt::MT_ERR_ARG, "mt_plan_create: null pointer");
  Plan* p = new Plan();
  (void)hipGetDevice(&p->device);
  *out = reinterpret_cast<mt_plan*>(p);
  return 0;
}

extern "C" int mt_plan_destroy(mt_plan* plan) {
  Plan* p = reinterpret_cast<Plan*>(plan);
  if (!p) return 0;
  if (mt::g_recording == p) mt::g_recording = nullptr;
  for (hipEvent_t e : p->fork_events) (void)hipEventDestroy(e);
  for (hipEvent_t e : p->free_timing) (void)hipEventDestroy(e);
  for (auto& h : p->hits) {
    (void)hipEventDestroy(h.e0);
    (void)hipEventDestroy(h.e1);
  }
  delete p;
  return 0;
}

extern "C" int mt_plan_record_begin(mt_plan* plan) {
  Plan* p = reinterpret_cast<Plan*>(plan);
  if (!p) return fail(mt::MT_ERR_ARG, "mt_plan_record_begin: null plan");
  if (mt::g_recording) return fail(mt::MT_ERR_ARG, "mt_plan_record_begin: this thread is already recording a plan");
  if (!p->ops.empty()) return fail(mt::MT_ERR_ARG, "mt_plan_record_begin: the plan already holds a recording");
  p->recording = true;
  mt::g_recording = p;
  mt::g_next_tag = 0;
  return 0;
}

extern "C" int mt_plan_record_end(mt_plan* plan) {
  Plan* p = reinterpret_cast<Plan*>(plan);
  if (!p || mt::g_recording != p) return fail(mt::MT_ERR_ARG, "mt_plan_record_end: this thread is not recording that plan");
  p->recording = false;
  mt::g_recording = nullptr;
  mt::g_next_tag = 0;
  return 0;
}

extern "C" int mt_plan_size(const mt_plan* plan) {
  const Plan* p = reinterpret_cast<const Plan*>(plan);
  return p ? (int)p->ops.size() : 0;
}

extern "C" int mt_plan_tag(int tag, double work) {
  if (tag < 0 || tag > 31) return fail(mt::MT_ERR_ARG, "mt_plan_tag: tag must lie in [0, 31]");
  mt::g_next_tag = tag;
  mt::g_next_work = work;
  return 0;
}

extern "C" int mt_plan_fork(void* from_stream, void* to_stream) {
  if (Plan* p = mt::plan_recording()) {
    hipEvent_t ev = nullptr;
    if (hipEventCreateWithFlags(&ev, hipEventDisableTiming) != hipSuccess) return fail(mt::MT_ERR_LAUNCH, "mt_plan_fork: event");
    p->fork_events.push_back(ev);
    const int rc = mt::fork_with(ev, from_stream, to_stream);
    if (rc == 0) p->add(to_stream, [=]() { return mt::fork_with(ev, from_stream, to_stream); });
    return rc;
  }
  hipEvent_t ev = mt::ring_event();
  if (!ev) return fail(mt::MT_ERR_LAUNCH, "mt_plan_fork: event");
  return mt::fork_with(ev, from_stream, to_stream);
}

extern "C" int mt_plan_run(mt_plan* plan, unsigned probe_mask) {
  Plan* p = reinterpret_cast<Plan*>(plan);
  if (!p) return fail(mt::MT_ERR_ARG, "mt_plan_run: null plan");
  if (p->recording) return fail(mt::MT_ERR_ARG, "mt_plan_run: the plan is still recording");
  if (mt::g_recording) return fail(mt::MT_ERR_ARG, "mt_plan_run: this thread is recording another plan");
  int dev = 0;
  (void)hipGetDevice(&dev);
  if (dev != p->device) return fail(mt::MT_ERR_ARG, "mt_plan_run: recorded on device %d, current device is %d", p->device, dev);
  const size_t n = p->ops.size();
  for (size_t i = 0; i < n; ++i) {
    mt::PlanOp& op = p->ops[i];
    const bool probe = op.tag && ((probe_mask >> op.tag) & 1u);
    hipEvent_t e0 = nullptr, e1 = nullptr;
    if (probe) {
      for (hipEvent_t* e : {&e0, &e1}) {
        if (!p->free_timing.empty()) {
          *e = p->free_timing.back();
          p->free_timing.pop_back();
        } else if (hipEventCreate(e) != hipSuccess) {
          return fail(mt::MT_ERR_LAUNCH, "mt_plan_run: probe event");
        }
      }
      (void)hipEventRecord(e0, (hipStream_t)op.stream);
    }
    const int rc = op.fn();
    if (probe) {
      (void)hipEventRecord(e1, (hipStream_t)op.stream);
      p->hits.push_back(mt::ProbeHit{op.tag, op.work, e0, e1});
    }
    if (rc != 0) return rc;
  }
  return 0;
}

extern "C" int mt_plan_probe_read(mt_plan* plan, int tag, int* launches, double* ms, double* work) {
  Plan* p = reinterpret_cast<Plan*>(plan);
  if (!p || !launches || !ms || !work) return fail(mt::MT_ERR_ARG, "mt_plan_probe_read: null pointer");
  int n = 0;
  double t = 0.0, w = 0.0;
  std::vector<mt::ProbeHit> rest;
  for (auto& h : p->hits) {
    if (h.tag != tag) {
      rest.push_back(h);
      continue;
    }
    float el = 0.f;
    hipError_t e = hipEventSynchronize(h.e1);
    if (e == hipSuccess) e = hipEventElapsedTime(&el, h.e0, h.e1);
    if (e != hipSuccess) return fail(mt::MT_ERR_LAUNCH, "mt_plan_probe_read: %s", hipGetErrorString(e));
    t += el;
    w += h.work;
    ++n;
    p->free_timing.push_back(h.e0);
    p->free_timing.push_back(h.e1);
  }
  p->hits.swap(rest);
  *launches = n;
  *ms = t;
  *work = w;
  return 0;
}

extern "C" int mti_memset_async(void* p, int value, int64_t bytes, void* stream) {
  if (bytes <= 0) return 0;
  if (!p) return fail(mt::MT_ERR_ARG, "mt_memset_async: null pointer");
  const hipError_t e = hipMemsetAsync(p, value, (size_t)bytes, (hipStream_t)stream);
  if (e != hipSuccess) return fail(mt::MT_ERR_LAUNCH, "mt_memset_async: %s", hipGetErrorString(e));
  return 0;
}

extern "C" int mti_copy_async(void* dst, const void* src, int64_t bytes, void* stream) {
  if (bytes <= 0) return 0;
  if (!dst || !src) return fail(mt::MT_ERR_ARG, "mt_copy_async: null pointer");
  const hipError_t e = hipMemcpyAsync(dst, src, (size_t)bytes, hipMemcpyDeviceToDevice, (hipStream_t)stream);
  if (e != hipSuccess) return fail(mt::MT_ERR_LAUNCH, "mt_copy_async: %s", hipGetErrorString(e));
  return 0;
}
```

mintime-multi-identity-size-invariant-timesformer-for-video-deepfake-detection_amd/effnet_backward.py:

```python
import torch

from . import arch
from . import lib as L
from .effnet_engine import SLOTS, STREAM_ROWS, _StatsPool


FUSED_DW = __import__("os").environ.get("MT_DW_FUSED", "3")
SE_FUSED = __import__("os").environ.get("MT_SE_FUSED", "0") != "0"
EXPAND_FUSED = __import__("os").environ.get("MT_EXPAND_FUSED", "1") != "0"
WIDE_WGRAD = __import__("os").environ.get("MT_WIDE_WGRAD", "1") != "0"
SE_STREAM = __import__("os").environ.get("MT_SE_STREAM", "1") != "0"


def _new(dev, *shape):
    return torch.empty(*shape, dtype=torch.float32, device=dev)


def _splits(rows):
    return max(1, min(64, rows // 1024))


LAST_RUN = {"blocks_run": 0, "wgrad_launches": 0, "stem_run": False}


def effnet_backward(model, params, saved, shape, training, dfeat, need_dx, need_dparams, keep_saved=False, plan=None):
    lib = L.get()
    st = L.stream_ptr()
    dev = dfeat.device
    N, H, W = shape
    blocks = model._blocks
    P = list(params)
    grads, flat_grads = L.zero_grads(list(params), with_flat=True)
    pos = 3
    bidx = []
    for blk in blocks:
        d = {}
        if blk.spec.has_expand:
            d["e"] = pos
            pos += 3
        d["d"] = pos
        d["se"] = pos + 3
        d["p"] = pos + 7
        pos += 10
        bidx.append(d)
    ih = pos
    need = [bool(x) for x in need_dparams]
    first_of = [3 if bi == 0 else (bidx[bi]["e"] if "e" in bidx[bi] else bidx[bi]["d"]) for bi in range(len(blocks))]
    need_below = [any(need[:first_of[bi]]) for bi in range(len(blocks))]
    lowest = min((bi for bi in range(len(blocks)) if any(need[first_of[bi]:(first_of[bi + 1] if bi + 1 < len(blocks) else ih)])),
                 default=len(blocks))
    if any(need[:3]):
        lowest = -1
    run = {"blocks_run": 0, "wgrad_launches": 0, "stem_run": False}
    total_c = arch.STEM_COUT + arch.HEAD_COUT + sum((b.spec.cexp if b.spec.has_expand else 0) + b.spec.cexp + b.spec.cout
                                                    for b in blocks)
    tr = 1 if training else 0
    side = L.SideStream(dev, hold=True)

    det = L.deterministic()
    pool = _StatsPool(dev, total_c, det)
    slots = -SLOTS if det else SLOTS
    expand_fused, wide_wgrad, se_stream, se_fused = (EXPAND_FUSED and not det, WIDE_WGRAD and not det, SE_STREAM and not det,
                                                     SE_FUSED and not det)
    fused_dw = "0" if det else FUSED_DW

    def bn_finalize(bnctx, sums, gidx_gamma, d=None, z=None, rows=0):
        kabc = _new(dev, 3, bnctx.C)
        L.check(lib.mt_bn_bwd_finalize(L.ptr(sums), slots, bnctx.count, L.ptr(P[gidx_gamma]), L.ptr(bnctx.mean_invstd), L.ptr(kabc),
                                       L.ptr(grads[gidx_gamma]), L.ptr(grads[gidx_gamma + 1]), bnctx.C, tr, st), "mt_bn_bwd_finalize")
        return kabc

    def act_bwd(din, z, bnctx, dout, rows, hw, act, gate=None, dpool=None, rowscale=None):
        sums = pool.take(bnctx.C)
        L.check(lib.mt_bn_act_bwd(L.ptr(din), L.ptr(z), L.ptr(bnctx.scale), L.ptr(bnctx.shift), L.ptr(bnctx.mean_invstd), L.ptr(gate),
                                  L.ptr(dpool), L.ptr(rowscale), L.ptr(dout), L.ptr(sums), slots, rows, bnctx.C, hw, act, st),
                "mt_bn_act_bwd")
        return sums

    def conv1x1_bwd(du, z, kabc, w, x_in, rows, cout, cin, gw_idx, need_dx_in, res=None, b_pro=None, epi=None, pl=None):
        if pl is not None and epi is None:
            dz_p = L.planes_empty(rows, cout, dev)
            L.check(lib.mt_bn_bwd_apply_planes(L.ptr(du), L.ptr(z), L.ptr(kabc), L.ptr(dz_p), rows, cout, st), "mt_bn_bwd_apply_planes")
            wdone = False
            if need[gw_idx] and pl.get("x_p") is not None:
                run["wgrad_launches"] += 1
                side.launch(lambda: L.gemm_planes(L.OP_TN, dz_p, pl["x_p"], cout, cin, rows, Cout=grads[gw_idx].view(cout, cin), ldc=cin,
                                                  epilogue=L.EPI_ATOMIC), reads=(dz_p, pl["x_p"]))
                wdone = True
            dx_in = None
            if need_dx_in:
                dx_in = _new(dev, rows, cin)
                if res is not None:
                    L.gemm_planes(L.OP_NN, dz_p, pl["w_p"], rows, cin, cout, Cout=dx_in, ldc=cin, epilogue=L.EPI_BIAS_RES, R=res, ldr=cin)
                else:
                    L.gemm_planes(L.OP_NN, dz_p, pl["w_p"], rows, cin, cout, Cout=dx_in, ldc=cin)
            if wdone or not need[gw_idx]:
                return dx_in
            need_dx_in, keep_dx = False, dx_in
        else:
            keep_dx = None
        kw = {}
        if b_pro is not None:
            kw = dict(b_prologue=L.BPRO_BN_SWISH_GATE, b_scale=b_pro[0], b_shift=b_pro[1], b_gate=b_pro[2], b_hw=b_pro[3])
        reads = (du, z, x_in, kabc) + (tuple(b_pro[:3]) if b_pro is not None else ())
        if (expand_fused and b_pro is None and epi is None and need[gw_idx] and need_dx_in and rows >= 100000
                and lib.mt_conv1x1_bwd_fused_supported(cout, cin)):
            run["wgrad_launches"] += 1
            dx_in = _new(dev, rows, cin)
            L.check(lib.mt_conv1x1_bwd_fused(L.ptr(du), L.ptr(kabc), L.ptr(x_in), L.ptr(w), L.ptr(res), L.ptr(dx_in),
                                             L.ptr(grads[gw_idx]), rows, cout, cin, st), "mt_conv1x1_bwd_fused")
            return dx_in
        if not need[gw_idx]:
            pass
        elif rows >= 100000 and not det and lib.mt_conv1x1_wgrad_supported(cout, cin):
            run["wgrad_launches"] += 1
            bp = b_pro if b_pro is not None else (None, None, None, 1)
            side.launch(lambda: L.check(lib.mt_conv1x1_wgrad(L.ptr(du), L.ptr(z), L.ptr(kabc), L.ptr(x_in), L.ptr(bp[0]), L.ptr(bp[1]),
                                                             L.ptr(bp[2]), bp[3], L.ptr(grads[gw_idx]), rows, cout, cin,
                                                             L.stream_ptr()), "mt_conv1x1_wgrad"), reads=reads)
        elif wide_wgrad and b_pro is not None and lib.mt_conv1x1_wgrad_wide_supported(cout, cin):
            run["wgrad_launches"] += 1
            side.launch(lambda: L.check(lib.mt_conv1x1_wgrad_wide(L.ptr(du), L.ptr(z), L.ptr(kabc), L.ptr(x_in), L.ptr(b_pro[0]),
                                                                  L.ptr(b_pro[1]), L.ptr(b_pro[2]), b_pro[3], L.ptr(grads[gw_idx]), rows,
                                                                  cout, cin, L.stream_ptr()), "mt_conv1x1_wgrad_wide"), reads=reads)
        else:
            run["wgrad_launches"] += 1
            side.launch(lambda: L.gemm(L.OP_TN, du, x_in, grads[gw_idx], cout, cin, rows, cout, cin, cin, prologue=L.PRO_BN_BWD,
                                       epilogue=L.EPI_ATOMIC, split_k=0, A2=z, scale=kabc[0], shift=kabc[1], gate=kabc[2], **kw),
                        reads=reads)
        if not need_dx_in:
            return keep_dx
        if epi is not None:
            for kind, out, kw2 in epi:
                L.gemm(L.OP_NN, du, w, out, rows, cin, cout, cout, cin, cin, prologue=L.PRO_BN_BWD, epilogue=kind, A2=z,
                       scale=kabc[0], shift=kabc[1], gate=kabc[2], **kw2)
            return None
        dx_in = _new(dev, rows, cin)
        if rows >= STREAM_ROWS and lib.mt_conv1x1_rows_supported(cout, cin, 2):
            L.check(lib.mt_conv1x1_rows(L.ptr(du), L.ptr(z), L.ptr(w), cin, 1, L.ptr(kabc[0]), L.ptr(kabc[1]), L.ptr(kabc[2]), 1, 2,
                                        L.ptr(res), L.ptr(dx_in), None, 1, rows, cout, cin, st), "mt_conv1x1_rows")
            return dx_in
        if res is not None:
            L.gemm(L.OP_NN, du, w, dx_in, rows, cin, cout, cout, cin, cin, prologue=L.PRO_BN_BWD, epilogue=L.EPI_BIAS_RES, A2=z,
                   scale=kabc[0], shift=kabc[1], gate=kabc[2], R=res, ldr=cin)
        else:
            L.gemm(L.OP_NN, du, w, dx_in, rows, cin, cout, cout, cin, cin, prologue=L.PRO_BN_BWD, A2=z, scale=kabc[0], shift=kabc[1],
                   gate=kabc[2])
        return dx_in

    hd = saved["head"]
    s_last = blocks[-1].spec
    M = N * s_last.hout * s_last.hout
    du_h = _new(dev, M, arch.HEAD_COUT)
    sums = act_bwd(dfeat, hd["z"], hd["bn"], du_h, M, 1, 1)
    kabc = bn_finalize(hd["bn"], sums, ih + 1, du_h, hd["z"], M)
    dy = conv1x1_bwd(du_h, hd["z"], kabc, P[ih], hd["y_in"], M, arch.HEAD_COUT, arch.HEAD_CIN, ih, lowest < len(blocks),
                     pl=dict(w_p=hd["w_p"], x_p=hd["y_p"]) if hd.get("w_p") is not None else None)
    del du_h

    for bi in reversed(range(len(blocks))):
        if bi < lowest:
            break
        run["blocks_run"] += 1
        blk, rec, ix = blocks[bi], saved["blocks"][bi], bidx[bi]
        s = rec["spec"]
        M_in, M_out = N * s.hin * s.hin, N * s.hout * s.hout
        hw = s.hout * s.hout
        dc = rec["dc"]
        dyb = _new(dev, M_out, s.cout) if dc is not None else None
        sums = act_bwd(dy, rec["z_p"], rec["bn_p"], dyb, M_out, hw, 0, rowscale=dc)
        dsrc = dyb if dc is not None else dy
        kabc_p = bn_finalize(rec["bn_p"], sums, ix["p"] + 1, dsrc, rec["z_p"], M_out)
        bn_d = rec["bn_d"]
        b_pro = (bn_d.scale, bn_d.shift, rec["gate"], hw)
        dgate, dpre2, dpooled = _new(dev, N, s.cexp), _new(dev, N, s.cexp), _new(dev, N, s.cexp)
        dhid = _new(dev, N, s.cse)
        se_scr = _new(dev, lib.mt_se_scratch_floats(N, s.cexp, s.cse))
        se = ix["se"]
        def se_part(parts, _da=None, _rec=rec, _bn=bn_d, _se=se, _s=s, _dg=dgate, _dp=dpre2, _dh=dhid, _dpo=dpooled, _hw=hw, _scr=se_scr):
            L.check(lib.mt_se_bwd(L.ptr(_da), L.ptr(_rec["z_d"]), L.ptr(_bn.scale), L.ptr(_bn.shift), L.ptr(_rec["gate"]),
                                  L.ptr(_rec["hidden"]), L.ptr(_rec["pooled"]), L.ptr(P[_se]), L.ptr(P[_se + 2]), L.ptr(_dg), L.ptr(_dp),
                                  L.ptr(_dh), L.ptr(_dpo), L.ptr(grads[_se]), L.ptr(grads[_se + 1]), L.ptr(grads[_se + 2]),
                                  L.ptr(grads[_se + 3]), N, _hw, _s.cexp, _s.cse, parts, L.ptr(_scr), L.stream_ptr()), "mt_se_bwd")
        if (se_stream and not se_fused and M_out >= 100000
                and lib.mt_se_stage_fused_supported(s.cout, s.cexp, hw)):
            conv1x1_bwd(dsrc, rec["z_p"], kabc_p, P[ix["p"]], rec["z_d"], M_out, s.cout, s.cexp, ix["p"], False, b_pro=b_pro)
            def stage(mode, dg, g_, dpo, mi, out, st_):
                L.check(lib.mt_se_stage_fused(L.ptr(dsrc), L.ptr(rec["z_p"]), L.ptr(kabc_p), L.ptr(P[ix["p"]]), L.ptr(rec["z_d"]),
                                              L.ptr(bn_d.scale), L.ptr(bn_d.shift), mode, L.ptr(dg), L.ptr(g_), L.ptr(dpo), L.ptr(mi),
                                              L.ptr(out), L.ptr(st_), slots, M_out, s.cout, s.cexp, hw, st), "mt_se_stage_fused")
            L.zero_(dgate)
            stage(0, dgate, None, None, None, None, None)
            se_part(4)
            if any(need[se:se + 4]):
                run["wgrad_launches"] += 1
                side.launch(lambda: se_part(2), reads=(dpre2, dhid, rec["hidden"], rec["pooled"]))
            da = _new(dev, M_out, s.cexp)
            sums = pool.take(s.cexp)
            stage(1, None, rec["gate"], dpooled, bn_d.mean_invstd, da, sums)
        elif se_fused:
            L.zero_(dgate)
            conv1x1_bwd(dsrc, rec["z_p"], kabc_p, P[ix["p"]], rec["z_d"], M_out, s.cout, s.cexp, ix["p"], True, b_pro=b_pro,
                        epi=[(L.EPI_SE_RED, dgate, dict(C2=rec["z_d"], ldc2=s.cexp, epi=(bn_d.scale, bn_d.shift, None, None, None, hw)))])
            se_part(4)
            if any(need[se:se + 4]):
                run["wgrad_launches"] += 1
                side.launch(lambda: se_part(2), reads=(dpre2, dhid, rec["hidden"], rec["pooled"]))
            da = _new(dev, M_out, s.cexp)
            sums = pool.take(s.cexp)
            need_save, need[ix["p"]] = need[ix["p"]], False
            conv1x1_bwd(dsrc, rec["z_p"], kabc_p, P[ix["p"]], rec["z_d"], M_out, s.cout, s.cexp, ix["p"], True, b_pro=b_pro,
                        epi=[(L.EPI_ACT_BWD, da, dict(C2=rec["z_d"], ldc2=s.cexp, stats=sums, stats_slots=slots,
                                                      epi=(bn_d.scale, bn_d.shift, rec["gate"], dpooled, bn_d.mean_invstd, hw)))])
            need[ix["p"]] = need_save
        else:
            da = conv1x1_bwd(dsrc, rec["z_p"], kabc_p, P[ix["p"]], rec["z_d"], M_out, s.cout, s.cexp, ix["p"], True, b_pro=b_pro,
                             pl=dict(w_p=rec["wp_p"], x_p=rec["a_p"]) if rec.get("wp_p") is not None else None)
            se_part(1, da)
            if any(need[se:se + 4]):
                run["wgrad_launches"] += 1
                side.launch(lambda: se_part(2), reads=(dpre2, dhid, rec["hidden"], rec["pooled"]))
            sums = act_bwd(da, rec["z_d"], bn_d, da, M_out, hw, 1, gate=rec["gate"], dpool=dpooled)
        kabc_d = bn_finalize(bn_d, sums, ix["d"] + 1, da, rec["z_d"], M_out)
        in_bn = rec["dw_bn"]
        du_in = _new(dev, M_in, s.cexp)
        sums_in = pool.take(s.cexp)
        def dw_part(parts, _da=da, _rec=rec, _kabc=kabc_d, _bn=in_bn, _du_in=du_in, _sums=sums_in, _s=s, _ix=ix):
            if _rec.get("rc"):
                L.check(lib.mt_dwconv_bwd_rc(L.ptr(_da), L.ptr(_rec["z_d"]), L.ptr(_kabc), L.ptr(P[_ix["d"]]), L.ptr(_rec["y_in"]),
                                             L.ptr(_rec["w_e"]), _s.cin, L.ptr(_bn.scale), L.ptr(_bn.shift), L.ptr(_bn.mean_invstd),
                                             L.ptr(_du_in), L.ptr(_sums), slots, L.ptr(grads[_ix["d"]]), N, _s.hin, _s.hin, _s.cexp,
                                             _s.k, _s.s, parts, L.stream_ptr()), "mt_dwconv_bwd_rc")
                return
            L.check(lib.mt_dwconv_bwd(L.ptr(_da), L.ptr(_rec["z_d"]), L.ptr(_kabc), L.ptr(P[_ix["d"]]), L.ptr(_rec["dw_in"]),
                                      L.ptr(_bn.scale), L.ptr(_bn.shift), L.ptr(_bn.mean_invstd), L.ptr(_du_in), L.ptr(_sums), slots,
                                      L.ptr(grads[_ix["d"]]), N, _s.hin, _s.hin, _s.cexp, _s.k, _s.s, parts, 1, None, None, L.stream_ptr()),
                    "mt_dwconv_bwd")
        need_du_in = need_below[bi] or (s.has_expand and any(need[ix["e"]:ix["e"] + 3]))
        dw_src = rec["y_in"] if rec.get("rc") else rec["dw_in"]
        dw_bytes = (4.0 * (s.cexp * (2 * M_out + M_in) + s.cin * M_in) if rec.get("rc") else 4.0 * s.cexp * (2 * M_out + 2 * M_in))
        if not need_du_in or not need[ix["d"]]:
            if need[ix["d"]]:
                run["wgrad_launches"] += 1
                side.launch(lambda: dw_part(1), reads=(da, rec["z_d"], kabc_d, dw_src, in_bn.scale, in_bn.shift))
            if need_du_in:
                L.timed("dwconv_dgrad", lambda: dw_part(2), dw_bytes)
        elif not rec.get("rc") and (fused_dw == "1" or (fused_dw == "3" and s.k == 3)):
            run["wgrad_launches"] += 1
            L.timed("dwconv_dgrad", lambda: dw_part(3), 4.0 * s.cexp * (2 * M_out + 2 * M_in))
        else:
            run["wgrad_launches"] += 1
            side.launch(lambda: dw_part(1), reads=(da, rec["z_d"], kabc_d, dw_src, in_bn.scale, in_bn.shift))
            L.timed("dwconv_dgrad", lambda: dw_part(2), dw_bytes)
        del da
        if not need_du_in:
            dy = None
        elif s.has_expand:
            kabc_e = bn_finalize(in_bn, sums_in, ix["e"] + 1, du_in, rec["dw_in"], M_in)
            z_e = rec["z_e"]
            if z_e is None and not (expand_fused and need[ix["e"]] and need_below[bi] and M_in >= 100000
                                    and lib.mt_conv1x1_bwd_fused_supported(s.cexp, s.cin)):
                z_e = _new(dev, M_in, s.cexp)
                L.gemm(L.OP_NT, rec["y_in"], P[ix["e"]], z_e, M_in, s.cexp, s.cin, s.cin, s.cin, s.cexp)
            dy = conv1x1_bwd(du_in, z_e, kabc_e, P[ix["e"]], rec["y_in"], M_in, s.cexp, s.cin, ix["e"], need_below[bi],
                             res=dy if s.skip else None,
                             pl=dict(w_p=rec["we_p"], x_p=rec["y_p"]) if rec.get("we_p") is not None else None)
        else:
            kabc0 = bn_finalize(in_bn, sums_in, 1, du_in, rec["dw_in"], M_in)
            stem = saved["stem"]
            run["stem_run"] = True
            if need[0]:
                run["wgrad_launches"] += 1
                L.check(lib.mt_stem_conv_wgrad(L.ptr(du_in), L.ptr(stem["z"]), L.ptr(kabc0), L.ptr(stem["x"]), 1 if stem["x"].dtype == torch.uint8 else 0, L.ptr(grads[0]), N, H, W, st),
                        "mt_stem_conv_wgrad")
            dy = None
        del du_in
        if not keep_saved:
            rec.clear()
        side.release_point()

    side.wait()
    if need_dx:
        raise NotImplementedError("gradient w.r.t. the input crops is not part of the MINTIME training path "
                                  "(train.py never sets requires_grad on videos)")
    LAST_RUN.update(run)
    if plan is not None:
        plan.extra.update(flat_grads=flat_grads, last_run=dict(LAST_RUN))
    L.grads_ready(model, params, flat_grads)
    out = [g if nd else None for nd, g in zip(need_dparams, grads)]
    return None, out
```

mintime-multi-identity-size-invariant-timesformer-for-video-deepfake-detection_amd/effnet_engine.py:

```python
import threading

import torch

from . import arch
from . import lib as L
from . import plans

SLOTS = 32
STEM_DIRECT = __import__("os").environ.get("MT_STEM_DIRECT", "1") != "0"
STREAM_ROWS = int(__import__("os").environ.get("MT_STREAM_ROWS", "100000"))
EF_RC = __import__("os").environ.get("MT_EF_RC", "0") != "0"
EF_RC_MIN_ROWS = int(__import__("os").environ.get("MT_EF_RC_ROWS", "100000"))
EF_PLANES = __import__("os").environ.get("MT_EF_PLANES", "1") != "0"
EF_PLANES_EXPAND_HW = int(__import__("os").environ.get("MT_EF_PLANES_EXPAND_HW", "14"))
EF_PLANES_PROJECT_HW = int(__import__("os").environ.get("MT_EF_PLANES_PROJECT_HW", "7"))


def _new(dev, *shape):
    return torch.empty(*shape, dtype=torch.float32, device=dev)


def param_list(model):
    ps = [model._conv_stem.weight, model._bn0.weight, model._bn0.bias]
    for blk in model._blocks:
        if blk.spec.has_expand:
            ps += [blk._expand_conv.weight, blk._bn0.weight, blk._bn0.bias]
        ps += [blk._depthwise_conv.weight, blk._bn1.weight, blk._bn1.bias, blk._se_reduce.weight, blk._se_reduce.bias,
               blk._se_expand.weight, blk._se_expand.bias, blk._project_conv.weight, blk._bn2.weight, blk._bn2.bias]
    ps += [model._conv_head.weight, model._bn1.weight, model._bn1.bias]
    return ps


class _BNCtx:

    def __init__(self, dev, C, training, stats_pool):
        self.C = C
        self.scale, self.shift = _new(dev, C), _new(dev, C)
        self.mean_invstd = _new(dev, 2, C)
        self.stats = stats_pool.take(C) if training else None
        self.count = 0.0


class _StatsPool:

    def __init__(self, dev, total_channels, det=False):
        self.limbs = 2 if det else 1
        self.buf = L.zeros(total_channels * 2 * SLOTS * self.limbs, torch.float64, dev)
        self.off = 0

    def take(self, C):
        n = 2 * SLOTS * C * self.limbs
        v = self.buf[self.off:self.off + n]
        self.off += n
        return v


def _finalize(lib, st, bn_mod, ctx, count, training, gamma, beta, slots=SLOTS):
    ctx.count = float(count)
    L.check(lib.mt_bn_finalize(L.ptr(ctx.stats), slots, float(count), L.ptr(gamma), L.ptr(beta), L.ptr(bn_mod.running_mean),
                               L.ptr(bn_mod.running_var), L.ptr(ctx.scale), L.ptr(ctx.shift), L.ptr(ctx.mean_invstd), ctx.C,
                               bn_mod.eps, bn_mod.momentum, 1 if training else 0, st), "mt_bn_finalize")
    if training:
        _track(bn_mod.num_batches_tracked)


_TLS = threading.local()


def _track(counter):
    if not hasattr(_TLS, "tracked"):
        _TLS.tracked = []
    _TLS.tracked.append(counter)


def planes_scope(model, N):
    on = EF_PLANES and L.gemm_split_enabled()
    blocks = model._blocks
    exp = [on and b.spec.has_expand and b.spec.hin <= EF_PLANES_EXPAND_HW and N * b.spec.hin * b.spec.hin >= 512 and b.spec.cin % 4 == 0
           for b in blocks]
    proj = [on and b.spec.hout <= EF_PLANES_PROJECT_HW and N * b.spec.hout * b.spec.hout >= 512 for b in blocks]
    last = blocks[-1].spec
    head = on and last.hout <= EF_PLANES_EXPAND_HW and N * last.hout * last.hout >= 512
    return exp, proj, head


def weight_planes(model, params, exp, proj, head):
    lib = L.get()
    blocks = model._blocks
    sel, pos = [], 3
    for bi, blk in enumerate(blocks):
        if blk.spec.has_expand:
            if exp[bi]:
                sel.append((("e", bi), params[pos], blk.spec.cexp, blk.spec.cin))
            pos += 3
        if proj[bi]:
            sel.append((("p", bi), params[pos + 7], blk.spec.cout, blk.spec.cexp))
        pos += 10
    if head:
        sel.append(("head", params[pos], arch.HEAD_COUT, arch.HEAD_CIN))
    if not sel:
        return {}, None
    ident = tuple((k, w.data_ptr()) for k, w, _, _ in sel)
    caches = model.__dict__.setdefault("_ef_wplanes_cache", {})
    if len(caches) > 4 and ident not in caches:
        caches.pop(next(iter(caches)))
    cache = caches.get(ident)
    if cache is None:
        holder, rows, first = {}, [], 0
        dev = sel[0][1].device
        for key, w, r, c in sel:
            if w.dtype != torch.float32 or not w.is_contiguous() or w.numel() != r * c:
                raise L.MintimeHipError("plane path needs contiguous fp32 1x1-conv weights")
            t = L.planes_empty(r, c, dev)
            holder[key] = t
            rows.append((w.data_ptr(), t.data_ptr(), r, c, first))
            first += t.shape[1] * t.shape[2]
        host = torch.tensor(rows, dtype=torch.int64).pin_memory()
        cache = caches[ident] = dict(holder=holder, host=host, table=host.to(dev, non_blocking=True), blocks=first, count=len(rows),
                                     serial=plans.PlaneSerial("the 1x1-conv weights"))
    L.check(lib.mt_split_planes_blk_multi(L.ptr(cache["table"]), cache["count"], cache["blocks"], L.stream_ptr()),
            "mt_split_planes_blk_multi")
    return cache["holder"], cache["serial"].touch([w for _, w, _, _ in sel])


def _bump_tracked(plan=None):
    tracked = getattr(_TLS, "tracked", None)
    if tracked:
        if plan is not None:
            plan.extra["tracked"] = list(tracked)
        torch._foreach_add_(tracked, 1)
        tracked.clear()


def _dc_gates(model, N, dev):
    blocks = model._blocks
    if not (model.training and model.drop_connect_rate > 0):
        return [], None
    gated = [bi for bi, blk in enumerate(blocks) if blk.spec.skip and model.drop_connect_rate * float(bi) / len(blocks) > 0]
    if not gated:
        return [], None
    sampler = getattr(model, "drop_connect_uniform", None)
    u = sampler(len(gated), N, dev) if sampler is not None else torch.rand(len(gated), N, device=dev, dtype=torch.float32)
    cache = model.__dict__.setdefault("_dc_keep_cache", {})
    key = (str(dev), model.drop_connect_rate)
    if key not in cache:
        cache[key] = torch.tensor([1.0 - model.drop_connect_rate * float(bi) / len(blocks) for bi in gated],
                                  dtype=torch.float32, device=dev).unsqueeze(1)
    keep = cache[key]
    return gated, torch.floor(keep + u.to(device=dev, dtype=torch.float32)) / keep


def effnet_forward(model, x_nhwc, params, training, save, want_blocks=False, plan=None):
    lib = L.get()
    st = L.stream_ptr()
    dev = x_nhwc.device
    N, H, W, _ = x_nhwc.shape
    blocks = model._blocks
    total_c = arch.STEM_COUT + arch.HEAD_COUT + sum((b.spec.cexp if b.spec.has_expand else 0) + b.spec.cexp + b.spec.cout
                                                    for b in blocks)
    det = training and L.deterministic()
    pool = _StatsPool(dev, total_c, det) if training else None
    it = iter(params)
    slots = -SLOTS if det else SLOTS
    epi = L.EPI_STATS if training else L.EPI_STORE
    sptr = (lambda b_: L.ptr(b_.stats)) if training else (lambda b_: None)
    saved = {"blocks": []} if save else None
    pl_exp, pl_proj, pl_head = planes_scope(model, N)
    wpl, w_serial = weight_planes(model, params, pl_exp, pl_proj, pl_head)
    y_p = None

    w_stem, g0, b0 = next(it), next(it), next(it)
    Hc, Wc = (H + 1) // 2, (W + 1) // 2
    bn = _BNCtx(dev, arch.STEM_COUT, training, pool)
    z = _new(dev, N * Hc * Wc, arch.STEM_COUT)
    if W <= 512 and H == W and STEM_DIRECT:
        L.check(lib.mt_stem_conv_fwd(L.ptr(x_nhwc), 1 if x_nhwc.dtype == torch.uint8 else 0, L.ptr(w_stem), L.ptr(z),
                                     sptr(bn), slots, N, H, W, st), "mt_stem_conv_fwd")
    else:
        wp = _new(dev, arch.STEM_COUT, 28)
        L.check(lib.mt_conv_weight_pack(L.ptr(w_stem), L.ptr(wp), arch.STEM_COUT, 3, 3, 28, 0, st), "mt_conv_weight_pack")
        L.gemm(L.OP_NT, x_nhwc, wp, z, N * Hc * Wc, arch.STEM_COUT, 28, 28, 28, arch.STEM_COUT, prologue=L.PRO_IM2COL, epilogue=epi,
               stats=bn.stats, stats_slots=slots, conv=(H, W, 3, Hc, Wc, 3, 2, 0, 0, 1 if x_nhwc.dtype == torch.uint8 else 0))
    _finalize(lib, st, model._bn0, bn, N * Hc * Wc, training, g0, b0, slots)
    if save:
        saved["stem"] = dict(x=x_nhwc, z=z, bn=bn)
    cur_z, cur_bn = z, bn
    y = None
    ys = [] if want_blocks else None

    gated, gates = _dc_gates(model, N, dev) if training else ([], None)
    dc_gates = {bi: gates[j] for j, bi in enumerate(gated)}
    if plan is not None:
        plan.extra["gates"] = gates
    for bi, blk in enumerate(blocks):
        s = blk.spec
        M_in = N * s.hin * s.hin
        M_out = N * s.hout * s.hout
        rec = {"spec": s}
        if s.has_expand:
            w_e, g, b = next(it), next(it), next(it)
            bn_e = _BNCtx(dev, s.cexp, training, pool)
            rc_on = (EF_RC and not L.deterministic() and M_in >= EF_RC_MIN_ROWS and w_e.data_ptr() % 16 == 0
                     and lib.mt_dwconv_rc_supported(s.cin, s.cexp, s.k, s.s, s.hin) and lib.mt_conv1x1_rows_instance(s.cin, s.cexp))
            z_e = None if rc_on else _new(dev, M_in, s.cexp)
            if rc_on:
                if training:
                    L.check(lib.mt_conv1x1_rows(L.ptr(y), None, L.ptr(w_e), s.cin, 0, None, None, None, 1, 0, None, None,
                                                sptr(bn_e), slots, M_in, s.cin, s.cexp, st), "mt_conv1x1_rows")
            elif pl_exp[bi]:
                L.gemm_planes(L.OP_NT, y_p, wpl[("e", bi)], M_in, s.cexp, s.cin, Cout=z_e, ldc=s.cexp, epilogue=epi, stats=bn_e.stats,
                              stats_slots=slots)
                rec.update(y_p=y_p, we_p=wpl[("e", bi)])
            elif M_in >= STREAM_ROWS and lib.mt_conv1x1_rows_supported(s.cin, s.cexp, 0):
                L.check(lib.mt_conv1x1_rows(L.ptr(y), None, L.ptr(w_e), s.cin, 0, None, None, None, 1, 0, None, L.ptr(z_e),
                                            sptr(bn_e), slots, M_in, s.cin, s.cexp, st), "mt_conv1x1_rows")
            else:
                L.gemm(L.OP_NT, y, w_e, z_e, M_in, s.cexp, s.cin, s.cin, s.cin, s.cexp, epilogue=epi, stats=bn_e.stats, stats_slots=slots)
            _finalize(lib, st, blk._bn0, bn_e, M_in, training, g, b, slots)
            rec.update(z_e=z_e, bn_e=bn_e, rc=rc_on, w_e=w_e)
            dw_in, dw_bn = z_e, bn_e
        else:
            rc_on = False
            dw_in, dw_bn = cur_z, cur_bn
        w_d, g, b = next(it), next(it), next(it)
        bn_d = _BNCtx(dev, s.cexp, training, pool)
        z_d = _new(dev, M_out, s.cexp)
        if rc_on:
            L.check(lib.mt_dwconv_fwd_rc(L.ptr(y), L.ptr(w_e), s.cin, L.ptr(dw_bn.scale), L.ptr(dw_bn.shift), L.ptr(w_d), L.ptr(z_d),
                                         sptr(bn_d), slots, N, s.hin, s.hin, s.cexp, s.k, s.s, st), "mt_dwconv_fwd_rc")
        else:
            L.check(lib.mt_dwconv_fwd(L.ptr(dw_in), L.ptr(dw_bn.scale), L.ptr(dw_bn.shift), L.ptr(w_d), L.ptr(z_d), sptr(bn_d),
                                      slots, N, s.hin, s.hin, s.cexp, s.k, s.s, 1, st), "mt_dwconv_fwd")
        _finalize(lib, st, blk._bn1, bn_d, M_out, training, g, b, slots)
        w_r, b_r, w_x, b_x = next(it), next(it), next(it), next(it)
        pooled, gate = _new(dev, N, s.cexp), _new(dev, N, s.cexp)
        hidden = _new(dev, N, s.cse)
        hw = s.hout * s.hout
        parts = lib.mt_se_pool_parts(N, hw, s.cexp)
        partial = _new(dev, N, parts, s.cexp)
        L.check(lib.mt_se_pool_fwd(L.ptr(z_d), L.ptr(bn_d.scale), L.ptr(bn_d.shift), L.ptr(partial), N, hw, s.cexp, parts, st),
                "mt_se_pool_fwd")
        L.check(lib.mt_se_gate_fwd(L.ptr(partial), parts, L.ptr(w_r), L.ptr(b_r), L.ptr(w_x), L.ptr(b_x), L.ptr(pooled), L.ptr(gate),
                                   L.ptr(hidden), N, s.cexp, s.cse, st), "mt_se_gate_fwd")
        w_p, g, b = next(it), next(it), next(it)
        bn_p = _BNCtx(dev, s.cout, training, pool)
        z_p = _new(dev, M_out, s.cout)
        if pl_proj[bi]:
            a_p = L.planes_empty(M_out, s.cexp, dev)
            L.check(lib.mt_bn_swish_gate_planes(L.ptr(z_d), L.ptr(bn_d.scale), L.ptr(bn_d.shift), L.ptr(gate), hw, L.ptr(a_p), M_out,
                                                s.cexp, st), "mt_bn_swish_gate_planes")
            L.gemm_planes(L.OP_NT, a_p, wpl[("p", bi)], M_out, s.cout, s.cexp, Cout=z_p, ldc=s.cout, epilogue=epi, stats=bn_p.stats,
                          stats_slots=slots)
            rec.update(a_p=a_p, wp_p=wpl[("p", bi)])
        elif M_out >= STREAM_ROWS and lib.mt_conv1x1_rows_supported(s.cexp, s.cout, 1):
            L.check(lib.mt_conv1x1_rows(L.ptr(z_d), None, L.ptr(w_p), s.cexp, 0, L.ptr(bn_d.scale), L.ptr(bn_d.shift), L.ptr(gate), hw, 1,
                                        None, L.ptr(z_p), sptr(bn_p), slots, M_out, s.cexp, s.cout, st), "mt_conv1x1_rows")
        else:
            L.gemm(L.OP_NT, z_d, w_p, z_p, M_out, s.cout, s.cexp, s.cexp, s.cexp, s.cout, prologue=L.PRO_BN_SWISH_GATE, epilogue=epi,
                   scale=bn_d.scale, shift=bn_d.shift, gate=gate, hw=hw, stats=bn_p.stats, stats_slots=slots)
        _finalize(lib, st, blk._bn2, bn_p, M_out, training, g, b, slots)
        dc = dc_gates.get(bi)
        y_new = _new(dev, M_out, s.cout)
        next_planes = pl_exp[bi + 1] if bi + 1 < len(blocks) else pl_head
        if next_planes:
            y_p = L.planes_empty(M_out, s.cout, dev)
            L.check(lib.mt_bn_act_fwd_planes(L.ptr(z_p), L.ptr(bn_p.scale), L.ptr(bn_p.shift), L.ptr(y if s.skip else None), L.ptr(y_new),
                                             M_out, s.cout, 0, L.ptr(dc), hw, L.ptr(y_p), st), "mt_bn_act_fwd_planes")
        else:
            y_p = None
            L.check(lib.mt_bn_act_fwd(L.ptr(z_p), L.ptr(bn_p.scale), L.ptr(bn_p.shift), L.ptr(y if s.skip else None), L.ptr(y_new),
                                      M_out, s.cout, 0, L.ptr(dc), hw, st), "mt_bn_act_fwd")
        if save:
            rec.update(y_in=y, dw_in=dw_in, dw_bn=dw_bn, z_d=z_d, bn_d=bn_d, pooled=pooled, hidden=hidden, gate=gate, z_p=z_p,
                       bn_p=bn_p, dc=dc)
            saved["blocks"].append(rec)
        y = y_new
        if want_blocks:
            ys.append(y.view(N, s.hout, s.hout, s.cout).permute(0, 3, 1, 2))

    w_h, g, b = next(it), next(it), next(it)
    s = blocks[-1].spec
    M = N * s.hout * s.hout
    bn_h = _BNCtx(dev, arch.HEAD_COUT, training, pool)
    z_h = _new(dev, M, arch.HEAD_COUT)
    if pl_head:
        L.gemm_planes(L.OP_NT, y_p, wpl["head"], M, arch.HEAD_COUT, arch.HEAD_CIN, Cout=z_h, ldc=arch.HEAD_COUT, epilogue=epi,
                      stats=bn_h.stats, stats_slots=slots)
    else:
        L.gemm(L.OP_NT, y, w_h, z_h, M, arch.HEAD_COUT, arch.HEAD_CIN, arch.HEAD_CIN, arch.HEAD_CIN, arch.HEAD_COUT, epilogue=epi,
               stats=bn_h.stats, stats_slots=slots)
    _finalize(lib, st, model._bn1, bn_h, M, training, g, b, slots)
    feat = _new(dev, M, arch.HEAD_COUT)
    L.check(lib.mt_bn_act_fwd(L.ptr(z_h), L.ptr(bn_h.scale), L.ptr(bn_h.shift), None, L.ptr(feat), M, arch.HEAD_COUT, 1, None, 1,
                              st), "mt_bn_act_fwd")
    if save:
        saved["head"] = dict(y_in=y, z=z_h, bn=bn_h, y_p=y_p if pl_head else None, w_p=wpl.get("head"))
        saved["w_serial"] = w_serial
    _bump_tracked(plan)
    return feat, saved, ys


class _EffNetFunction(torch.autograd.Function):
    @staticmethod
    def forward(ctx, model, want_blocks, x_nhwc, *params):
        want_blocks, grad_on = want_blocks
        save = grad_on and any(ctx.needs_input_grad)
        N, H, W, _ = x_nhwc.shape
        ctx.shape = (N, H, W)
        ctx.model, ctx.params, ctx.training = model, params, model.training
        stream = key = state = None
        if save and not want_blocks:
            stream = torch.cuda.current_stream(x_nhwc.device).cuda_stream
            state = list(params) + list(model.buffers())
            key = ("ef", tuple(x_nhwc.shape), x_nhwc.dtype, model.training, L.deterministic(), L.gemm_split_enabled(),
                   float(model.drop_connect_rate), tuple(ctx.needs_input_grad[3:]), stream,
                   float(model._bn0.momentum), float(model._bn0.eps))
# ... 43 lines not shown
```

mintime-multi-identity-size-invariant-timesformer-for-video-deepfake-detection_amd/lib.py:

```python
import ctypes as C
import os
import subprocess
import threading

import torch

_HERE = os.path.dirname(os.path.abspath(__file__))
CSRC = os.path.join(_HERE, "csrc")
LIB_PATH = os.environ.get("MT_LIB") or os.path.join(CSRC, "libmintime_hip.so")

_lib = None

f32p = C.c_void_p
i64 = C.c_int64


class RowMap(C.Structure):
    _fields_ = [("gin", C.c_int), ("gout", C.c_int), ("off", C.c_int)]


class Conv3dDesc(C.Structure):
    _fields_ = [(n, C.c_int) for n in ("N", "T", "H", "W", "C", "To", "Ho", "Wo", "K", "kt", "kh", "kw", "st", "sh", "sw", "pt", "ph",
                                       "pw")] + [("ldx", i64), ("ldy", i64)]


class GemmDesc(C.Structure):
    _fields_ = [("op", C.c_int), ("prologue", C.c_int), ("epilogue", C.c_int),
                ("A", C.c_void_p), ("B", C.c_void_p), ("C", C.c_void_p),
                ("M", C.c_int), ("N", C.c_int), ("K", C.c_int),
                ("lda", i64), ("ldb", i64), ("ldc", i64),
                ("a_map", RowMap), ("b_map", RowMap), ("c_map", RowMap),
                ("bias", C.c_void_p), ("R", C.c_void_p), ("ldr", i64),
                ("scale", C.c_void_p), ("shift", C.c_void_p), ("gate", C.c_void_p), ("hw", C.c_int),
                ("C2", C.c_void_p), ("ldc2", i64), ("stats", C.c_void_p), ("stats_slots", C.c_int),
                ("n_half", C.c_int), ("split_k", C.c_int),
                ("A2", C.c_void_p), ("b_prologue", C.c_int), ("b_scale", C.c_void_p), ("b_shift", C.c_void_p),
                ("b_gate", C.c_void_p), ("b_hw", C.c_int),
                ("conv_H", C.c_int), ("conv_W", C.c_int), ("conv_C", C.c_int), ("conv_Ho", C.c_int), ("conv_Wo", C.c_int),
                ("conv_k", C.c_int), ("conv_stride", C.c_int), ("conv_pad", C.c_int), ("conv_act", C.c_int), ("conv_src_u8", C.c_int),
                ("col_sum", C.c_void_p), ("b_planes", C.c_void_p), ("b_plane_stride", C.c_int64),
                ("e_scale", C.c_void_p), ("e_shift", C.c_void_p), ("e_gate", C.c_void_p), ("e_dpool", C.c_void_p),
                ("e_mi", C.c_void_p), ("e_hw", C.c_int)]


class GemmPlanesDesc(C.Structure):
    _fields_ = [("op", C.c_int), ("epilogue", C.c_int), ("M", C.c_int), ("N", C.c_int), ("K", C.c_int),
                ("a_planes", C.c_void_p), ("b_planes", C.c_void_p), ("C", C.c_void_p), ("ldc", i64),
                ("bias", C.c_void_p), ("R", C.c_void_p), ("ldr", i64), ("C2", C.c_void_p), ("ldc2", i64),
                ("n_half", C.c_int), ("col_sum", C.c_void_p), ("c_planes", C.c_void_p), ("split_k", C.c_int),
                ("sk_workspace", C.c_void_p), ("sk_workspace_bytes", i64), ("stats", C.c_void_p), ("stats_slots", C.c_int)]


OP_NT, OP_NN, OP_TN = 0, 1, 2
PRO_NONE, PRO_BN_SWISH_GATE, PRO_BN_SWISH, PRO_AFFINE, PRO_BN_BWD, PRO_IM2COL = 0, 1, 2, 3, 4, 5
BPRO_NONE, BPRO_BN_SWISH_GATE, BPRO_IM2COL = 0, 1, 2
EPI_STORE, EPI_BIAS_RES, EPI_GEGLU, EPI_STATS, EPI_ATOMIC, EPI_GEGLU_BWD, EPI_ACCUM, EPI_SE_RED, EPI_ACT_BWD = 0, 1, 2, 3, 4, 5, 6, 7, 8

PROTOTYPES = {
    "mt_version": [],
    "mt_last_error": [],
    "mt_set_deterministic": [C.c_int],
    "mt_get_deterministic": [],
    "mt_det_release": [C.c_void_p],
    "mt_det_bn_sums": [f32p, f32p, f32p, i64, C.c_int, C.c_int, C.c_void_p, C.c_void_p],
    "mt_gemm": [C.POINTER(GemmDesc), C.c_void_p],
    "mt_gemm_set_split": [C.c_int],
    "mt_gemm_get_split": [],
    "mt_split_planes": [f32p, C.c_void_p, C.c_int64, C.c_void_p],
    "mt_planes_elems": [C.c_int, C.c_int],
    "mt_split_planes_blk": [f32p, i64, C.c_int, C.c_int, C.c_void_p, C.c_void_p],
    "mt_split_planes_blk_multi": [C.c_void_p, C.c_int, i64, C.c_void_p],
    "mt_bn_bwd_apply_planes": [f32p, f32p, f32p, C.c_void_p, C.c_int, C.c_int, C.c_void_p],
    "mt_gemm_planes": [C.POINTER(GemmPlanesDesc), C.c_void_p],
    "mt_gemm_planes_workspace_bytes": [],
    "mt_gemm_planes_set_persist": [C.c_int],
    "mt_mul_planes": [f32p, f32p, C.c_void_p, f32p, C.c_int, C.c_int, C.c_void_p],
    "mt_mul_add": [f32p, f32p, f32p, f32p, i64, C.c_void_p],
    "mt_geglu_bwd": [f32p, f32p, f32p, C.c_void_p, f32p, C.c_int, C.c_int, C.c_void_p],
    "mt_layernorm_fwd": [f32p, f32p, f32p, f32p, f32p, C.c_int, C.c_int, C.c_float, C.c_void_p, C.c_void_p],
    "mt_embed_fwd": [f32p, f32p, f32p, f32p, C.c_void_p, C.c_void_p, C.c_int, C.c_int, C.c_int, C.c_int, C.c_int, C.c_int, C.c_void_p,
                     C.c_void_p],
    "mt_attn_fwd": [f32p, f32p, f32p, C.c_void_p, C.c_void_p, C.c_int, C.c_int, C.c_int, C.c_int, C.c_int, C.c_float,
                    C.c_void_p, C.c_void_p],
    "mt_head_fwd": [f32p, f32p, f32p, f32p, f32p, f32p, C.c_int, C.c_int, C.c_int, C.c_int, C.c_float, C.c_void_p],
    "mt_stem_conv_fwd": [C.c_void_p, C.c_int, f32p, f32p, C.c_void_p, C.c_int, C.c_int, C.c_int, C.c_int, C.c_void_p],
    "mt_stem_conv_fwd_valid": [C.c_void_p, C.c_int, f32p, f32p, C.c_void_p, C.c_int, C.c_int, C.c_int, C.c_int, C.c_void_p],
    "mt_dwconv_fwd": [f32p, f32p, f32p, f32p, f32p, C.c_void_p, C.c_int, C.c_int, C.c_int, C.c_int, C.c_int, C.c_int, C.c_int,
                      C.c_int, C.c_void_p],
    "mt_dwconv_fwd_planes": [f32p] * 4 + [C.c_void_p] + [C.c_int] * 7 + [C.c_void_p],
    "mt_dwconv_rc_supported": [C.c_int] * 5,
    "mt_dwconv_fwd_rc": [f32p, f32p, C.c_int, f32p, f32p, f32p, f32p, C.c_void_p] + [C.c_int] * 7 + [C.c_void_p],
    "mt_dwconv_bwd_rc": [f32p] * 6 + [C.c_int] + [f32p] * 4 + [C.c_void_p, C.c_int, f32p] + [C.c_int] * 7 + [C.c_void_p],
    "mt_bn_finalize": [C.c_void_p, C.c_int, C.c_double, f32p, f32p, f32p, f32p, f32p, f32p, f32p, C.c_int, C.c_float,
                       C.c_float, C.c_int, C.c_void_p],
    "mt_se_pool_parts": [C.c_int, C.c_int, C.c_int],
    "mt_se_pool_fwd": [f32p, f32p, f32p, f32p, C.c_int, C.c_int, C.c_int, C.c_int, C.c_void_p],
    "mt_se_gate_fwd": [f32p, C.c_int, f32p, f32p, f32p, f32p, f32p, f32p, f32p, C.c_int, C.c_int, C.c_int, C.c_void_p],
    "mt_bn_act_fwd": [f32p, f32p, f32p, f32p, f32p, i64, C.c_int, C.c_int, f32p, C.c_int, C.c_void_p],
    "mt_attn_aggregate": [f32p, f32p, f32p, C.c_int, C.c_int, C.c_int, C.c_float, C.c_void_p],
    "mt_build_clip_inputs": [C.c_void_p] * 8 + [C.c_int] * 5 + [C.c_void_p],
    "mt_layernorm_bwd": [f32p, f32p, f32p, f32p, f32p, f32p, f32p, C.c_int, C.c_int, C.c_int, f32p, C.c_int, f32p, C.c_void_p],
    "mt_layernorm_bwd_rows": [f32p, f32p, f32p, f32p, f32p, f32p, C.c_int, C.c_int, C.c_void_p, C.c_void_p],
    "mt_layernorm_bwd_cols": [f32p, f32p, f32p, f32p, f32p, f32p, f32p, C.c_int, C.c_int, C.c_int, C.c_void_p],
    "mt_layernorm_bwd_rows_blocks": [C.c_int],
    "mt_layernorm_bwd_rows_sums": [f32p, f32p, f32p, f32p, f32p, f32p, C.c_int, C.c_int, C.c_void_p, f32p, C.c_int, C.c_void_p],
    "mt_layernorm_bwd_cols_reduce": [f32p, C.c_int, C.c_int, f32p, f32p, f32p, C.c_void_p],
    "mt_colsum": [f32p, i64, RowMap, C.c_int, C.c_int, f32p, C.c_void_p],
    "mt_head_bwd": [f32p, f32p, f32p, f32p, f32p, f32p, f32p, f32p, f32p, f32p, C.c_int, C.c_int, C.c_int, C.c_int, C.c_float,
                    C.c_void_p],
    "mt_embed_bwd": [f32p, f32p, f32p, f32p, C.c_void_p, C.c_void_p, C.c_int, C.c_int, C.c_int, C.c_int, C.c_int, C.c_int, C.c_void_p],
    "mt_attn_bwd": [f32p, f32p, f32p, C.c_void_p, C.c_void_p, C.c_int, C.c_int, C.c_int, C.c_int, C.c_int, C.c_float,
                    C.c_void_p, C.c_void_p],
    "mt_bn_act_bwd": [f32p] * 9 + [C.c_void_p, C.c_int, i64, C.c_int, C.c_int, C.c_int, C.c_void_p],
    "mt_bn_bwd_finalize": [C.c_void_p, C.c_int, C.c_double, f32p, f32p, f32p, f32p, f32p, C.c_int, C.c_int, C.c_void_p],
    "mt_se_bwd": [f32p] * 17 + [C.c_int, C.c_int, C.c_int, C.c_int, C.c_int, f32p, C.c_void_p],
    "mt_se_scratch_floats": [C.c_int, C.c_int, C.c_int],
    "mt_dwconv_bwd": [f32p] * 9 + [C.c_void_p, C.c_int, f32p, C.c_int, C.c_int, C.c_int, C.c_int, C.c_int, C.c_int, C.c_int,
                      C.c_int, f32p, f32p, C.c_void_p],
    "mt_dwconv_bwd_res2": [f32p] * 9 + [C.c_void_p, C.c_int, f32p, C.c_int, C.c_int, C.c_int, C.c_int, C.c_int, C.c_int, C.c_int,
                           C.c_int, f32p, f32p, C.c_void_p],
    "mt_conv_weight_pack": [f32p, f32p, C.c_int, C.c_int, C.c_int, C.c_int, C.c_int, C.c_void_p],
    "mt_conv_weight_unpack_grad": [f32p, f32p, C.c_int, C.c_int, C.c_int, C.c_int, C.c_void_p],
    "mt_maxpool_add_fwd": [f32p] * 7 + [C.c_int, C.c_int, C.c_int, C.c_int, C.c_void_p],
    "mt_maxpool_bwd": [f32p] * 5 + [C.c_int, C.c_int, C.c_int, C.c_int, C.c_void_p],
    "mt_maxpool_add_fwd_arg": [f32p] * 7 + [C.c_void_p, f32p, C.c_int, C.c_int, C.c_int, C.c_int, C.c_void_p],
    "mt_maxpool_bwd_arg": [f32p, C.c_void_p, f32p, C.c_int, C.c_int, C.c_int, C.c_int, C.c_void_p],
    "mt_maxpool_bn_bwd_apply_planes": [f32p, C.c_void_p, f32p, f32p, C.c_void_p, C.c_int, C.c_int, C.c_int, C.c_int, C.c_void_p],
    "mt_bn_bwd_apply": [f32p, f32p, f32p, f32p, i64, C.c_int, C.c_void_p],
    "mt_conv1x1_rows_supported": [C.c_int, C.c_int, C.c_int],
    "mt_conv1x1_rows_instance": [C.c_int, C.c_int],
    "mt_conv1x1_rows": [f32p, f32p, f32p, C.c_int, C.c_int, f32p, f32p, f32p, C.c_int, C.c_int, f32p, f32p, C.c_void_p, C.c_int, C.c_int64,
                        C.c_int, C.c_int, C.c_void_p],
    "mt_bce_logits": [f32p, f32p, C.c_float, f32p, f32p, C.c_int, C.c_void_p],
    "mt_transpose_multi": [C.c_void_p, C.c_int, C.c_int64, C.c_void_p],
    "mt_sgd_multi": [C.c_void_p, C.c_int, C.c_int64, C.c_float, C.c_float, C.c_void_p],
    "mt_adam_multi": [C.c_void_p, C.c_int, C.c_int64, C.c_float, C.c_float, C.c_double, C.c_double, C.c_float, C.c_float, C.c_float,
                      C.c_int, C.c_void_p],
    "mt_conv1x1_wgrad_supported": [C.c_int, C.c_int],
    "mt_conv1x1_wgrad": [f32p] * 7 + [C.c_int, f32p, C.c_int64, C.c_int, C.c_int, C.c_void_p],
    "mt_conv1x1_wgrad_wide_supported": [C.c_int, C.c_int],
    "mt_conv1x1_wgrad_wide": [f32p] * 7 + [C.c_int, f32p, C.c_int64, C.c_int, C.c_int, C.c_void_p],
    "mt_conv1x1_bwd_fused_supported": [C.c_int, C.c_int],
    "mt_se_stage_fused_supported": [C.c_int, C.c_int, C.c_int],
    "mt_se_stage_fused": [f32p] * 7 + [C.c_int] + [f32p] * 5 + [C.c_void_p, C.c_int, C.c_int64, C.c_int, C.c_int, C.c_int, C.c_void_p],
    "mt_conv1x1_bwd_fused": [f32p] * 7 + [C.c_int64, C.c_int, C.c_int, C.c_void_p],
    "mt_stem_conv_wgrad": [f32p] * 4 + [C.c_int, f32p, C.c_int, C.c_int, C.c_int, C.c_void_p],
    "mt_stem_conv_wgrad_valid": [f32p] * 4 + [C.c_int, f32p, C.c_int, C.c_int, C.c_int, C.c_void_p],
    "mt_bn_act_fwd_planes": [f32p, f32p, f32p, f32p, f32p, C.c_int, C.c_int, C.c_int, f32p, C.c_int, C.c_void_p, C.c_void_p],
    "mt_bn_swish_gate_planes": [f32p, f32p, f32p, f32p, C.c_int, C.c_void_p, C.c_int, C.c_int, C.c_void_p],
    "mt_baseline_head_fwd": [f32p, C.c_int, C.c_int, C.c_int, C.c_int, C.c_int] + [f32p] * 8 + [C.c_void_p],
    "mt_baseline_head_bwd": [f32p, f32p, f32p, C.c_int, C.c_int, C.c_int, C.c_int] + [f32p] * 8 + [C.c_int, f32p, C.c_void_p],
    "mt_conv3d_part_floats": [C.c_void_p],
    "mt_conv3d_wgrad_splits": [C.c_void_p],
    "mt_conv3d_fwd": [C.c_void_p, f32p, f32p, f32p, f32p, f32p, C.c_int, f32p, C.c_void_p, C.c_void_p],
    "mt_conv3d_dgrad": [C.c_void_p, f32p, f32p, f32p, C.c_int, C.c_void_p],
    "mt_conv3d_wgrad": [C.c_void_p, f32p, f32p, f32p, f32p, f32p, f32p, C.c_int, C.c_void_p],
    "mt_sf_bn_relu_fwd": [f32p, i64, f32p, f32p, f32p, i64, f32p, f32p, f32p, i64, i64, C.c_int, C.c_void_p],
    "mt_sf_bn_bwd_part_floats": [i64, C.c_int],
    "mt_sf_bn_relu_bwd_stats": [f32p, i64, f32p, i64, f32p, f32p, f32p, i64, f32p, f32p, C.c_void_p, i64, C.c_int, C.c_void_p],
    "mt_sf_bn_relu_bwd_apply": [f32p, i64, f32p, i64, f32p, f32p, f32p, i64, f32p, f32p, i64, C.c_int, i64, C.c_int, C.c_void_p],
    "mt_sf_maxpool_fwd": [f32p, f32p, f32p, f32p, i64, C.c_void_p, i64, C.c_int, C.c_int, C.c_int, C.c_void_p],
    "mt_sf_maxpool_bwd": [f32p, i64, C.c_void_p, f32p, i64, C.c_int, C.c_int, C.c_int, C.c_void_p],
    "mt_sf_head_pool": [f32p, i64, f32p, f32p] + [C.c_int] * 10 + [C.c_void_p],
    "mt_sf_head_proj": [f32p, f32p, f32p, f32p, C.c_int, C.c_int, C.c_int, C.c_int, C.c_void_p],
    "mt_sf_head_bwd": [f32p] * 7 + [C.c_int] * 4 + [C.c_void_p],
    "mt_sf_head_dfeat": [f32p, f32p, i64] + [C.c_int] * 10 + [C.c_void_p],
    "mt_sf_ingest": [C.c_void_p, C.c_int, i64, i64, i64, i64, i64, C.c_void_p] + [C.c_int] * 6 + [f32p, f32p, C.c_void_p],
    "mt_plan_create": [C.POINTER(C.c_void_p)],
    "mt_plan_destroy": [C.c_void_p],
    "mt_plan_record_begin": [C.c_void_p],
    "mt_plan_record_end": [C.c_void_p],
    "mt_plan_size": [C.c_void_p],
    "mt_plan_tag": [C.c_int, C.c_double],
    "mt_plan_fork": [C.c_void_p, C.c_void_p],
    "mt_plan_run": [C.c_void_p, C.c_uint],
    "mt_plan_probe_read": [C.c_void_p, C.c_int, C.POINTER(C.c_int), C.POINTER(C.c_double), C.POINTER(C.c_double)],
    "mt_memset_async": [C.c_void_p, C.c_int, i64, C.c_void_p],
    "mt_copy_async": [C.c_void_p, C.c_void_p, i64, C.c_void_p],
}
_RESTYPES = {"mt_last_error": C.c_char_p, "mt_planes_elems": C.c_int64, "mt_gemm_planes_workspace_bytes": C.c_int64,
             "mt_conv3d_part_floats": C.c_int64, "mt_sf_bn_bwd_part_floats": C.c_int64}


class MintimeHipError(RuntimeError):
    pass


def build(verbose: bool = False):
    cmd = ["make", "-C", CSRC, "-j", str(min(16, os.cpu_count() or 4))]
    res = subprocess.run(cmd, capture_output=True, text=True)
    if res.returncode != 0:
        raise MintimeHipError("building libmintime_hip.so failed:\n" + res.stdout[-4000:] + res.stderr[-8000:])
    if verbose:
        print(res.stdout[-2000:])
    global _lib
    _lib = None
    return LIB_PATH


ABI_VERSION = 121


def header_version() -> int:
    import re
    with open(os.path.join(_HERE, "..", "include", "mintime_hip.h")) as f:
        return int(re.search(r"#define\s+MT_VERSION\s+(\d+)", f.read()).group(1))


def get():
    global _lib
    if _lib is not None:
        return _lib
    if not os.path.exists(LIB_PATH):
        raise MintimeHipError(
            f"{LIB_PATH} is missing: the MINTIME hot path has no CPU/eager fallback. "
            "Build it with `python -c 'import __graft_entry__ as g; g.build()'` (needs hipcc).")
    lib = C.CDLL(LIB_PATH)
    for name, argtypes in PROTOTYPES.items():
        try:
            fn = getattr(lib, name)
        except AttributeError as e:
            raise MintimeHipError(f"libmintime_hip.so does not export {name}; rebuild it") from e
        fn.argtypes = argtypes
        fn.restype = _RESTYPES.get(name, C.c_int)
    v = lib.mt_version()
    if v != ABI_VERSION:
        raise MintimeHipError(f"libmintime_hip.so version {v} != binding version {ABI_VERSION}; rebuild it "
                              "(`python -c 'import __graft_entry__ as g; g.build()'`)")
    _lib = lib
    return lib


def set_deterministic(on: bool) -> bool:
    prev = bool(get().mt_get_deterministic())
    get().mt_set_deterministic(1 if on else 0)
    return prev


def deterministic() -> bool:
    return bool(get().mt_get_deterministic())


def set_gemm_split(on: bool) -> bool:
    return bool(get().mt_gemm_set_split(1 if on else 0))


def split_planes(w):
    w = w.detach()
    if not w.is_contiguous() or w.numel() % 8:
        raise MintimeHipError("split_planes: contiguous tensor with numel % 8 == 0 expected")
    out = torch.empty((3,) + tuple(w.shape), dtype=torch.bfloat16, device=w.device)
    check(get().mt_split_planes(ptr(w), ptr(out), w.numel(), stream_ptr()), "mt_split_planes")
    return out


def planes_shape(rows, cols):
    return (3, (rows + 31) // 32, (cols + 15) // 16, 32, 16)


def planes_empty(rows, cols, device):
    return torch.empty(planes_shape(rows, cols), dtype=torch.bfloat16, device=device)


def split_planes_blk(x, rows=None, cols=None, ld=None, out=None):
    if rows is None:
        rows, cols = x.shape[-2], x.shape[-1]
    if ld is None:
        ld = cols
    if out is None:
        out = planes_empty(rows, cols, x.device)
    check(get().mt_split_planes_blk(ptr(x), ld, rows, cols, ptr(out), stream_ptr()), "mt_split_planes_blk")
    return out


def planes_to_float(planes, rows, cols):
    p = planes.float().sum(0)
    return p.permute(0, 2, 1, 3).reshape(p.shape[0] * 32, p.shape[1] * 16)[:rows, :cols]


_SK_WORKSPACES = {}


def streamk_workspace(device=None):
# ... 337 lines not shown
```

Before: 708.1 clips/s.

## Fold BatchNorm finalize into producer kernels via last-block ticket tail

Adds an armed 'fold' mechanism: instead of launching separate BN finalize kernels after the depthwise conv forward, bn_act backward and dwconv backward kernels, the producer kernel's last block per channel group (found with an atomic ticket counter) reduces the stats and writes scale/shift or kabc directly. This removes several small finalize launches per MBConv block in forward and backward, and the serialization gaps around them. In exchange each producer kernel carries extra LDS and a tail path with atomics plus cross-block visibility of the stats. It also depends on thread-local arming state, which must match the next producer launch exactly.

```diff
diff --git a/include/mintime_hip.h b/include/mintime_hip.h
--- a/include/mintime_hip.h
+++ b/include/mintime_hip.h
@@ -5,7 +5,7 @@
 extern "C" {
 #endif
 
-#define MT_VERSION 121
+#define MT_VERSION 122
 
 int mt_version(void);
 const char* mt_last_error(void);
@@ -127,6 +127,9 @@
 int mt_bn_finalize(const double* stats, int slots, double count, const float* gamma, const float* beta,
                    float* running_mean, float* running_var, float* scale, float* shift, float* mean_invstd,
                    int C, float eps, float momentum, int training, void* stream);
+int mt_bn_finalize_fold(const double* stats, int slots, double count, const float* gamma, const float* beta,
+                        float* running_mean, float* running_var, float* scale, float* shift, float* mean_invstd,
+                        int C, float eps, float momentum, int training, void* stream);
 
 int mt_se_pool_parts(int N, int HW, int C);
 int mt_se_pool_fwd(const float* z, const float* scale, const float* shift, float* partial, int N, int HW, int C, int parts,
@@ -179,6 +182,8 @@
 
 int mt_bn_bwd_finalize(const double* stats, int slots, double count, const float* gamma, const float* mean_invstd,
                        float* kabc, float* dgamma, float* dbeta, int C, int training, void* stream);
+int mt_bn_bwd_finalize_fold(const double* stats, int slots, double count, const float* gamma, const float* mean_invstd,
+                            float* kabc, float* dgamma, float* dbeta, int C, int training, void* stream);
 
 int mt_se_scratch_floats(int N, int C, int CS);
 int mt_se_bwd(const float* da, const float* z, const float* scale, const float* shift, const float* gate,
diff --git a/mintime-multi-identity-size-invariant-timesformer-for-video-deepfake-detection_amd/csrc/bn_fold.hip b/mintime-multi-identity-size-invariant-timesformer-for-video-deepfake-detection_amd/csrc/bn_fold.hip
--- /dev/null
+++ b/mintime-multi-identity-size-invariant-timesformer-for-video-deepfake-detection_amd/csrc/bn_fold.hip
@@ -0,0 +1,88 @@
+#include "../../include/mintime_hip.h"
+#include "bn_fold.hpp"
+
+namespace mt {
+
+namespace {
+struct Armed {
+  BnFold f;
+  const void* stats;
+  int slots, C;
+  hipStream_t stream;
+};
+thread_local Armed g_armed{};
+
+unsigned* fold_tickets(hipStream_t stream) {
+  static std::mutex mu;
+  static std::map<std::pair<int, hipStream_t>, unsigned*> arenas;
+  int dev = 0;
+  (void)hipGetDevice(&dev);
+  std::lock_guard<std::mutex> g(mu);
+  unsigned*& p = arenas[std::make_pair(dev, stream)];
+  if (!p) {
+    if (hipMalloc(&p, FOLD_MAX_GROUPS * sizeof(unsigned)) != hipSuccess) { p = nullptr; return nullptr; }
+    if (hipMemset(p, 0, FOLD_MAX_GROUPS * sizeof(unsigned)) != hipSuccess || hipStreamSynchronize(nullptr) != hipSuccess) { (void)hipFree(p); p = nullptr; return nullptr; }
+  }
+  return p;
+}
+
+int arm(const BnFold& f, const void* stats, int slots, int C, void* stream, const char* who) {
+  if (g_armed.f.kind != 0) {
+    fold_clear();
+    return fail(MT_ERR_ARG, "%s: another BatchNorm fold is still armed on this thread (no producer took it)", who);
+  }
+  g_armed.f = f;
+  g_armed.stats = stats;
+  g_armed.slots = slots != 0 ? slots : 1;
+  g_armed.C = C;
+  g_armed.stream = (hipStream_t)stream;
+  return 0;
+}
+}
+
+bool fold_pending() { return g_armed.f.kind != 0; }
+void fold_clear() { g_armed = Armed{}; }
+
+int fold_take(const void* stats, int slots, int C, int groups, hipStream_t stream, BnFold* out, const char* who) {
+  *out = BnFold{};
+  if (g_armed.f.kind == 0) return 0;
+  const Armed a = g_armed;
+  fold_clear();
+  if (!stats || a.stats != stats || a.slots != slots || a.C != C || a.stream != stream)
+    return fail(MT_ERR_ARG, "%s: the armed BatchNorm fold is for other sums (stats %p / slots %d / C %d, this launch %p / %d / %d, or "
+                "another stream)", who, a.stats, a.slots, a.C, stats, slots, C);
+  if (groups < 1 || groups > FOLD_MAX_GROUPS) return fail(MT_ERR_UNSUPPORTED, "%s: %d channel groups (fold arena holds %d)", who, groups, (int)FOLD_MAX_GROUPS);
+  *out = a.f;
+  out->tickets = fold_tickets(stream);
+  if (!out->tickets) {
+    *out = BnFold{};
+    return fail(MT_ERR_LAUNCH, "%s: cannot allocate the fold's ticket arena", who);
+  }
+  return 0;
+}
+
+}
+
+using namespace mt;
+
+extern "C" int mt_bn_finalize_fold(const double* stats, int slots, double count, const float* gamma, const float* beta,
+                                   float* running_mean, float* running_var, float* scale, float* shift, float* mean_invstd, int C,
+                                   float eps, float momentum, int training, void* stream) {
+  if (!stats || !gamma || !beta || !scale || !shift) return fail(MT_ERR_ARG, "mt_bn_finalize_fold: null pointer");
+  if (!training) return fail(MT_ERR_ARG, "mt_bn_finalize_fold: eval mode has no producer (use mt_bn_finalize)");
+  if ((running_mean == nullptr) != (running_var == nullptr)) return fail(MT_ERR_ARG, "mt_bn_finalize_fold: running_mean and running_var go together");
+  BnFold f{};
+  f.kind = 1; f.training = 1; f.count = count; f.gamma = gamma; f.beta = beta;
+  f.running_mean = running_mean; f.running_var = running_var; f.scale = scale; f.shift = shift; f.mean_invstd = mean_invstd;
+  f.eps = eps; f.momentum = momentum;
+  return arm(f, stats, slots, C, stream, "mt_bn_finalize_fold");
+}
+
+extern "C" int mt_bn_bwd_finalize_fold(const double* stats, int slots, double count, const float* gamma, const float* mean_invstd,
+                                       float* kabc, float* dgamma, float* dbeta, int C, int training, void* stream) {
+  if (!stats || !gamma || !mean_invstd || !kabc) return fail(MT_ERR_ARG, "mt_bn_bwd_finalize_fold: null pointer");
+  BnFold f{};
+  f.kind = 2; f.training = training; f.count = count; f.gamma = gamma; f.mean_invstd_in = mean_invstd;
+  f.kabc = kabc; f.dgamma = dgamma; f.dbeta = dbeta;
+  return arm(f, stats, slots, C, stream, "mt_bn_bwd_finalize_fold");
+}
diff --git a/mintime-multi-identity-size-invariant-timesformer-for-video-deepfake-detection_amd/csrc/bn_fold.hpp b/mintime-multi-identity-size-invariant-timesformer-for-video-deepfake-detection_amd/csrc/bn_fold.hpp
--- /dev/null
+++ b/mintime-multi-identity-size-invariant-timesformer-for-video-deepfake-detection_amd/csrc/bn_fold.hpp
@@ -0,0 +1,145 @@
+#pragma once
+#include "common.hpp"
+
+namespace mt {
+
+struct BnFold {
+  int kind;
+  int training;
+  unsigned* tickets;
+  double count;
+  const float* gamma;
+  const float* beta;
+  const float* mean_invstd_in;
+  float* running_mean;
+  float* running_var;
+  float* scale;
+  float* shift;
+  float* mean_invstd;
+  float* kabc;
+  float* dgamma;
+  float* dbeta;
+  float eps, momentum;
+};
+
+enum { FOLD_MAX_GROUPS = 4096 };
+
+bool fold_pending();
+void fold_clear();
+int fold_take(const void* stats, int slots, int C, int groups, hipStream_t stream, BnFold* out, const char* who);
+int fold_left_armed(int rc, const char* who);
+
+__device__ __forceinline__ void bn_fwd_finish(int c, int C, double s, double q, double count, const float* __restrict__ gamma,
+                                              const float* __restrict__ beta, float* __restrict__ running_mean,
+                                              float* __restrict__ running_var, float* __restrict__ scale, float* __restrict__ shift,
+                                              float* __restrict__ mean_invstd, float eps, float momentum, int training) {
+  float mean, var;
+  if (training) {
+    const double m = s / count;
+    double v = q / count - m * m;
+    if (v < 0.0) v = 0.0;
+    mean = (float)m; var = (float)v;
+    if (running_mean) {
+      const double unb = count > 1.0 ? v * count / (count - 1.0) : v;
+      running_mean[c] = (1.f - momentum) * running_mean[c] + momentum * mean;
+      running_var[c] = (1.f - momentum) * running_var[c] + momentum * (float)unb;
+    }
+  } else {
+    mean = running_mean[c]; var = running_var[c];
+  }
+  const float invstd = 1.0f / sqrtf(var + eps);
+  const float sc = gamma[c] * invstd;
+  scale[c] = sc;
+  shift[c] = beta[c] - mean * sc;
+  if (mean_invstd) { mean_invstd[c] = mean; mean_invstd[C + c] = invstd; }
+}
+
+__device__ __forceinline__ void bn_bwd_finish(int c, int C, double s1, double s2, double count, const float* __restrict__ gamma,
+                                              const float* __restrict__ mean_invstd, float* __restrict__ kabc,
+                                              float* __restrict__ dgamma, float* __restrict__ dbeta, int training) {
+  const float mean = mean_invstd[c], istd = mean_invstd[C + c];
+  const float ka = gamma[c] * istd;
+  float kb = 0.f, kc = 0.f;
+  if (training) {
+    const float c1 = (float)(s1 / count), c2 = (float)(s2 / count);
+    kb = -ka * c2 * istd;
+    kc = ka * c2 * istd * mean - ka * c1;
+  }
+  kabc[c] = ka; kabc[C + c] = kb; kabc[2 * C + c] = kc;
+  if (dgamma) dgamma[c] += (float)s2;
+  if (dbeta) dbeta[c] += (float)s1;
+}
+
+__device__ __forceinline__ unsigned long long fold_peek(const double* p) {
+  return __hip_atomic_fetch_or(reinterpret_cast<unsigned long long*>(const_cast<double*>(p)), 0ull, __ATOMIC_RELAXED,
+                               __HIP_MEMORY_SCOPE_AGENT);
+}
+__device__ __forceinline__ double fold_decode(unsigned long long hi, unsigned long long lo, bool det) {
+  if (!det) return __longlong_as_double((long long)hi);
+  return (double)(long long)hi + (double)(long long)lo * 5.684341886080801486968994140625e-14;
+}
+
+enum { FOLD_LDS_BYTES = 8 * 64 * 2 * 8 + 8 };
+__device__ __forceinline__ void bn_fold_tail(const BnFold& f, const double* stats, int slots, int C, int group, unsigned members,
+                                             int c_lo, int c_n, int tid, int nt, void* lds) {
+  if (f.kind == 0) return;
+  double* red = reinterpret_cast<double*>(lds);
+  unsigned* last = reinterpret_cast<unsigned*>(red + 8 * 64 * 2);
+  asm volatile("s_waitcnt vmcnt(0)" ::: "memory");
+  __syncthreads();
+  if (tid == 0)
+    *last = __hip_atomic_fetch_add(f.tickets + group, 1u, __ATOMIC_RELAXED, __HIP_MEMORY_SCOPE_AGENT) + 1u == members;
+  __syncthreads();
+  if (!*last) return;
+  const int ns = stat_slots(slots);
+  const bool det = slots < 0;
+  const int64_t limb = stat_limb(slots, C);
+  for (int cb = 0; cb < c_n; cb += 64) {
+    for (int idx = tid; idx < 256; idx += nt) {
+      const int cl = idx & 31, sg = idx >> 5;
+      double a[2] = {0.0, 0.0}, b[2] = {0.0, 0.0};
+      for (int i0 = sg; i0 < ns; i0 += 32) {
+        unsigned long long va[2][4], vb[2][4], wa[2][4], wb[2][4];
+#pragma unroll
+        for (int h = 0; h < 2; ++h) {
+          const int c = c_lo + cb + h * 32 + cl;
+#pragma unroll
+          for (int u = 0; u < 4; ++u) va[h][u] = vb[h][u] = wa[h][u] = wb[h][u] = 0ull;
+          if (cb + h * 32 + cl < c_n && c < C) {
+#pragma unroll
+            for (int u = 0; u < 4; ++u) {
+              const double* pa = stats + ((int64_t)min(i0 + 8 * u, ns - 1) * 2) * C + c;
+              va[h][u] = fold_peek(pa); vb[h][u] = fold_peek(pa + C);
+              if (det) { wa[h][u] = fold_peek(pa + limb); wb[h][u] = fold_peek(pa + C + limb); }
+            }
+          }
+        }
+#pragma unroll
+        for (int h = 0; h < 2; ++h)
+#pragma unroll
+          for (int u = 0; u < 4; ++u)
+            if (i0 + 8 * u < ns) { a[h] += fold_decode(va[h][u], wa[h][u], det); b[h] += fold_decode(vb[h][u], wb[h][u], det); }
+      }
+#pragma unroll
+      for (int h = 0; h < 2; ++h) { red[(sg * 64 + h * 32 + cl) * 2] = a[h]; red[(sg * 64 + h * 32 + cl) * 2 + 1] = b[h]; }
+    }
+    __syncthreads();
+    for (int cl = tid; cl < 64; cl += nt) {
+      const int c = c_lo + cb + cl;
+      if (cb + cl < c_n && c < C) {
+        double a = 0.0, b = 0.0;
+#pragma unroll
+        for (int g = 0; g < 8; ++g) { a += red[(g * 64 + cl) * 2]; b += red[(g * 64 + cl) * 2 + 1]; }
+        if (f.kind == 1)
+          bn_fwd_finish(c, C, a, b, f.count, f.gamma, f.beta, f.running_mean, f.running_var, f.scale, f.shift, f.mean_invstd, f.eps,
+                        f.momentum, f.training);
+        else
+          bn_bwd_finish(c, C, a, b, f.count, f.gamma, f.mean_invstd_in, f.kabc, f.dgamma, f.dbeta, f.training);
+      }
+    }
+    __syncthreads();
+  }
+  if (tid == 0) __hip_atomic_store(f.tickets + group, 0u, __ATOMIC_RELAXED, __HIP_MEMORY_SCOPE_AGENT);
+}
+
+}
diff --git a/mintime-multi-identity-size-invariant-timesformer-for-video-deepfake-detection_amd/csrc/effnet_bwd.hip b/mintime-multi-identity-size-invariant-timesformer-for-video-deepfake-detection_amd/csrc/effnet_bwd.hip
--- a/mintime-multi-identity-size-invariant-timesformer-for-video-deepfake-detection_amd/csrc/effnet_bwd.hip
+++ b/mintime-multi-identity-size-invariant-timesformer-for-video-deepfake-detection_amd/csrc/effnet_bwd.hip
@@ -1,5 +1,6 @@
 #include "../../include/mintime_hip.h"
 #include "common.hpp"
+#include "bn_fold.hpp"
 #include <type_traits>
 #include "rc.hpp"
 #include "det.hpp"
@@ -60,7 +61,7 @@
                                                          const float* __restrict__ mean_invstd, const float* __restrict__ gate,
                                                          const float* __restrict__ dpool, const float* __restrict__ rowscale,
                                                          float* __restrict__ dout, double* __restrict__ stats, int slots,
-                                                         int64_t rows, int C, int hw, int act, int CQB, int PB) {
+                                                         int64_t rows, int C, int hw, int act, int CQB, int PB, const BnFold fold) {
   extern __shared__ float red[];
   const int tid = threadIdx.x;
   const int cql = tid % CQB, pl = tid / CQB;
@@ -95,6 +96,7 @@
     }
   }
   reduce_stats(red, s1, s2, cql, pl, CQB, PB, CQ, C, stats, slots);
+  bn_fold_tail(fold, stats, slots, C, blockIdx.y, gridDim.x, blockIdx.y * CQB * 4, CQB * 4, tid, blockDim.x, red);
 }
 
 __global__ __launch_bounds__(256) void bn_bwd_finalize_kernel(const double* __restrict__ stats, int slots, double count,
@@ -116,17 +118,7 @@
   double s1 = 0.0, s2 = 0.0;
 #pragma unroll
   for (int g = 0; g < 8; ++g) { s1 += red[g][cl][0]; s2 += red[g][cl][1]; }
-  const float mean = mean_invstd[c], istd = mean_invstd[C + c];
-  const float ka = gamma[c] * istd;
-  float kb = 0.f, kc = 0.f;
-  if (training) {
-    const float c1 = (float)(s1 / count), c2 = (float)(s2 / count);
-    kb = -ka * c2 * istd;
-    kc = ka * c2 * istd * mean - ka * c1;
-  }
-  kabc[c] = ka; kabc[C + c] = kb; kabc[2 * C + c] = kc;
-  if (dgamma) dgamma[c] += (float)s2;
-  if (dbeta) dbeta[c] += (float)s1;
+  bn_bwd_finish(c, C, s1, s2, count, gamma, mean_invstd, kabc, dgamma, dbeta, training);
 }
 
 __global__ __launch_bounds__(256) void se_bwd_reduce_kernel(const float* __restrict__ da, const float* __restrict__ z,
@@ -482,7 +474,7 @@
     const float* __restrict__ zin, const float* __restrict__ scale_in, const float* __restrict__ shift_in,
     const float* __restrict__ mi_in, float* __restrict__ du_in, double* __restrict__ stats, int slots, int N, int H, int W,
     int C, int Ho, int Wo, const float* __restrict__ res_pre, const float* __restrict__ res_post, float* __restrict__ dw,
-    int res_stride, const float* __restrict__ we) {
+    int res_stride, const float* __restrict__ we, const BnFold fold) {
   static_assert(RC == 0 || CC == 16, "the recompute yields 16-channel chunks");
   constexpr int P = S == 1 ? (K - 1) / 2 : (K - 2) / 2;
   constexpr int CQN = CC / 4, NSLOT = 256 / CQN;
@@ -714,6 +706,7 @@
     const int ch = c0 + q * 4 + (e & 3), which = e >> 2;
     stat_add(stats + ((int64_t)(blockIdx.x % stat_slots(slots)) * 2 + which) * C + ch, stat_limb(slots, C), v);
   }
+  bn_fold_tail(fold, stats, slots, C, chunk_id, gridDim.x / (unsigned)(C / CC), c0, CC, tid, 256, lds);
 }
 
 template <int K, int S, int T, int ACT, int CC, bool WG = false, int RC = 0>
@@ -726,10 +719,13 @@
   constexpr int CQN = CC / 4, NSLOT = 256 / CQN;
   size_t lds = (size_t)(OT * OTP * CC + ((K > 3 || S == 1) ? K * K * CC : 0) + (RC ? T * T * CC : 0) + (WG ? T * T * CC : 0)) * sizeof(float);
   if (lds < 256 * 8 * sizeof(float)) lds = 256 * 8 * sizeof(float);
+  if (lds < FOLD_LDS_BYTES) lds = FOLD_LDS_BYTES;
   if (WG && lds < (size_t)(NSLOT / K) * K * CQN * K * 4 * sizeof(float)) lds = (size_t)(NSLOT / K) * K * CQN * K * 4 * sizeof(float);
   const int chunks = C / CC;
   const int64_t ntiles = (int64_t)N * ((H + T - 1) / T) * ((W + T - 1) / T);
   const unsigned bx = xcd_chunk_grid(chunks, ntiles, WG ? 4096 : 8192);
+  BnFold fold;
+  if (const int rc = fold_take(stats, slots != 0 ? slots : 1, C, chunks, s, &fold, "mt_dwconv_bwd")) return rc;
   auto kfn = dwconv_dgrad_tiled_kernel<K, S, T, ACT, CC, WG, RC>;
   if (lds > 48 * 1024) {
     hipError_t e = ensure_dynamic_lds(reinterpret_cast<const void*>(kfn), lds);
@@ -737,7 +733,7 @@
   }
   hipLaunchKernelGGL(kfn, dim3(bx), dim3(256), lds, s, du, z, kabc, w, zin,
                      scale_in, shift_in, mi_in, du_in, stats, slots != 0 ? slots : 1, N, H, W, C, Ho, Wo, res_pre, res_post, dw,
-                     g_res_stride, we);
+                     g_res_stride, we, fold);
   return check_launch(WG ? "mt_dwconv_bwd(data + weight, fused)" : "mt_dwconv_bwd(data, tiled)");
 }
 
@@ -865,9 +861,13 @@
   int64_t nb = (rows + PB - 1) / PB;
   const int64_t cap = 4096 / (CQ / CQB) > 0 ? 4096 / (CQ / CQB) : 1;
   if (nb > cap) nb = cap;
-  hipLaunchKernelGGL(bn_act_bwd_kernel, dim3((unsigned)nb, CQ / CQB), dim3(CQB * PB), (size_t)PB * CQB * 8 * sizeof(float),
-                     (hipStream_t)stream, din, z, scale, shift, mean_invstd, gate, dpool, rowscale, dout, stats,
-                     slots != 0 ? slots : 1, rows, C, hw > 0 ? hw : 1, act, CQB, PB);
+  BnFold fold;
+  if (const int rc = fold_take(stats, slots != 0 ? slots : 1, C, CQ / CQB, (hipStream_t)stream, &fold, "mt_bn_act_bwd")) return rc;
+  size_t lds = (size_t)PB * CQB * 8 * sizeof(float);
+  if (lds < FOLD_LDS_BYTES) lds = FOLD_LDS_BYTES;
+  hipLaunchKernelGGL(bn_act_bwd_kernel, dim3((unsigned)nb, CQ / CQB), dim3(CQB * PB), lds, (hipStream_t)stream, din, z, scale, shift,
+                     mean_invstd, gate, dpool, rowscale, dout, stats, slots != 0 ? slots : 1, rows, C, hw > 0 ? hw : 1, act, CQB, PB,
+                     fold);
   return check_launch("mt_bn_act_bwd");
 }
 
diff --git a/mintime-multi-identity-size-invariant-timesformer-for-video-deepfake-detection_amd/csrc/effnet_fwd.hip b/mintime-multi-identity-size-invariant-timesformer-for-video-deepfake-detection_amd/csrc/effnet_fwd.hip
--- a/mintime-multi-identity-size-invariant-timesformer-for-video-deepfake-detection_amd/csrc/effnet_fwd.hip
+++ b/mintime-multi-identity-size-invariant-timesformer-for-video-deepfake-detection_amd/csrc/effnet_fwd.hip
@@ -1,5 +1,6 @@
 #include "../../include/mintime_hip.h"
 #include "common.hpp"
+#include "bn_fold.hpp"
 #include "planes.hpp"
 #include "rc.hpp"
 #include <stdlib.h>
@@ -37,7 +38,7 @@
                                                            const float* __restrict__ shift, const float* __restrict__ w,
                                                            float* __restrict__ zout, double* __restrict__ stats, int slots,
                                                            int N, int H, int W, int C, int Ho, int Wo, int pad0, PlaneRef po,
-                                                           const float* __restrict__ we) {
+                                                           const float* __restrict__ we, const BnFold fold) {
   static_assert(RC == 0 || CC == 16, "the recompute yields 16-channel chunks");
   constexpr int CQN = CC / 4, NSLOT = 256 / CQN;
   constexpr int IH = (T - 1) * S + K;
@@ -169,6 +170,7 @@
       const int ch = c0 + q * 4 + (e & 3), which = e >> 2;
       stat_add(stats + ((int64_t)(blockIdx.x % stat_slots(slots)) * 2 + which) * C + ch, stat_limb(slots, C), v);
     }
+    bn_fold_tail(fold, stats, slots, C, chunk_id, gridDim.x / (unsigned)(C / CC), c0, CC, tid, 256, lds);
   }
 }
 
@@ -180,16 +182,19 @@
   constexpr int IWP = IH | 1;
   size_t lds = (size_t)(IH * IWP * CC + (K > 3 ? K * K * CC : 0)) * sizeof(float);
   if (lds < 256 * 8 * sizeof(float)) lds = 256 * 8 * sizeof(float);
+  if (lds < FOLD_LDS_BYTES) lds = FOLD_LDS_BYTES;
   const int chunks = C / CC;
   const int64_t ntiles = (int64_t)N * ((Ho + T - 1) / T) * ((Wo + T - 1) / T);
   const unsigned bx = xcd_chunk_grid(chunks, ntiles, 8192);
+  BnFold fold;
+  if (const int rc = fold_take(stats, slots != 0 ? slots : 1, C, chunks, s, &fold, "mt_dwconv_fwd")) return rc;
   auto k = dwconv_tiled_kernel<K, S, T, ACT, CC, RC>;
   if (lds > 48 * 1024) {
     hipError_t e = ensure_dynamic_lds(reinterpret_cast<const void*>(k), lds);
     if (e != hipSuccess) return fail(MT_ERR_LAUNCH, "mt_dwconv_fwd: cannot reserve %zu B of LDS: %s", lds, hipGetErrorString(e));
   }
   hipLaunchKernelGGL(k, dim3(bx), dim3(256), lds, s, zin, scale, shift, w, zout, stats, slots != 0 ? slots : 1, N, H,
-                     W, C, Ho, Wo, pad0, po, we);
+                     W, C, Ho, Wo, pad0, po, we, fold);
   return check_launch("mt_dwconv_fwd(tiled)");
 }
 
@@ -226,28 +231,12 @@
     __syncthreads();
   }
   if (sg != 0 || c >= C) return;
-  float mean, var;
+  double s = 0.0, q = 0.0;
   if (training) {
-    double s = 0.0, q = 0.0;
 #pragma unroll
     for (int g = 0; g < 8; ++g) { s += red[g][cl][0]; q += red[g][cl][1]; }
-    const double m = s / count;
-    double v = q / count - m * m;
-    if (v < 0.0) v = 0.0;
-    mean = (float)m; var = (float)v;
-    if (running_mean) {
-      const double unb = count > 1.0 ? v * count / (count - 1.0) : v;
-      running_mean[c] = (1.f - momentum) * running_mean[c] + momentum * mean;
-      running_var[c] = (1.f - momentum) * running_var[c] + momentum * (float)unb;
-    }
-  } else {
-    mean = running_mean[c]; var = running_var[c];
-  }
-  const float invstd = 1.0f / sqrtf(var + eps);
-  const float sc = gamma[c] * invstd;
-  scale[c] = sc;
-  shift[c] = beta[c] - mean * sc;
-  if (mean_invstd) { mean_invstd[c] = mean; mean_invstd[C + c] = invstd; }
+  }
+  bn_fwd_finish(c, C, s, q, count, gamma, beta, running_mean, running_var, scale, shift, mean_invstd, eps, momentum, training);
 }
 
 __global__ __launch_bounds__(256) void se_pool_kernel(const float* __restrict__ z, const float* __restrict__ scale,
diff --git a/mintime-multi-identity-size-invariant-timesformer-for-video-deepfake-detection_amd/csrc/gen_plan.py b/mintime-multi-identity-size-invariant-timesformer-for-video-deepfake-detection_amd/csrc/gen_plan.py
--- a/mintime-multi-identity-size-invariant-timesformer-for-video-deepfake-detection_amd/csrc/gen_plan.py
+++ b/mintime-multi-identity-size-invariant-timesformer-for-video-deepfake-detection_amd/csrc/gen_plan.py
@@ -20,6 +20,7 @@
 
 
 SKIP = {"mt_plan_run", "mt_plan_fork"}
+FOLD_ARM = {"mt_bn_finalize_fold", "mt_bn_bwd_finalize_fold"}
 
 
 def main(header, rename_h, thunks_inc):
@@ -43,7 +44,9 @@
                     call.append(f"&{n}_v")
                 else:
                     call.append(n)
-            f.write(f"  const int rc = {inner}({', '.join(n for _, n in ps)});\n")
+            f.write(f"  {'const ' if name in FOLD_ARM else ''}int rc = {inner}({', '.join(n for _, n in ps)});\n")
+            if name not in FOLD_ARM:
+                f.write(f'  if (mt::fold_pending()) rc = mt::fold_left_armed(rc, "{name}");\n')
             f.write("  if (rc == 0) if (mt::Plan* p_ = mt::plan_recording()) {\n")
             f.write("".join(pre))
             f.write(f"    p_->add(stream, [=]() {{ return {inner}({', '.join(call)}); }});\n")
diff --git a/mintime-multi-identity-size-invariant-timesformer-for-video-deepfake-detection_amd/csrc/plan.hip b/mintime-multi-identity-size-invariant-timesformer-for-video-deepfake-detection_amd/csrc/plan.hip
--- a/mintime-multi-identity-size-invariant-timesformer-for-video-deepfake-detection_amd/csrc/plan.hip
+++ b/mintime-multi-identity-size-invariant-timesformer-for-video-deepfake-detection_amd/csrc/plan.hip
@@ -5,6 +5,7 @@
 
 #include "../../include/mintime_hip.h"
 #include "common.hpp"
+#include "bn_fold.hpp"
 
 namespace mt {
 
@@ -37,6 +38,12 @@
 static thread_local double g_next_work = 0.0;
 
 Plan* plan_recording() { return g_recording; }
+
+int fold_left_armed(int rc, const char* who) {
+  fold_clear();
+  if (rc != 0) return rc;
+  return fail(MT_ERR_ARG, "%s: a BatchNorm finalize fold was armed, and this entry point did not take it (the fold is dropped)", who);
+}
 
 void Plan::add(void* stream, std::function<int()> fn) {
   ops.push_back(PlanOp{std::move(fn), g_next_tag, g_next_work, stream});
@@ -131,6 +138,7 @@
 }
 
 extern "C" int mt_plan_fork(void* from_stream, void* to_stream) {
+  if (mt::fold_pending()) return mt::fold_left_armed(0, "mt_plan_fork");
   if (Plan* p = mt::plan_recording()) {
     hipEvent_t ev = nullptr;
     if (hipEventCreateWithFlags(&ev, hipEventDisableTiming) != hipSuccess) return fail(mt::MT_ERR_LAUNCH, "mt_plan_fork: event");
@@ -147,6 +155,7 @@
 extern "C" int mt_plan_run(mt_plan* plan, unsigned probe_mask) {
   Plan* p = reinterpret_cast<Plan*>(plan);
   if (!p) return fail(mt::MT_ERR_ARG, "mt_plan_run: null plan");
+  if (mt::fold_pending()) return mt::fold_left_armed(0, "mt_plan_run");
   if (p->recording) return fail(mt::MT_ERR_ARG, "mt_plan_run: the plan is still recording");
   if (mt::g_recording) return fail(mt::MT_ERR_ARG, "mt_plan_run: this thread is recording another plan");
   int dev = 0;
diff --git a/mintime-multi-identity-size-invariant-timesformer-for-video-deepfake-detection_amd/effnet_backward.py b/mintime-multi-identity-size-invariant-timesformer-for-video-deepfake-detection_amd/effnet_backward.py
--- a/mintime-multi-identity-size-invariant-timesformer-for-video-deepfake-detection_amd/effnet_backward.py
+++ b/mintime-multi-identity-size-invariant-timesformer-for-video-deepfake-detection_amd/effnet_backward.py
@@ -64,18 +64,20 @@
                                                      SE_FUSED and not det)
     fused_dw = "0" if det else FUSED_DW
 
-    def bn_finalize(bnctx, sums, gidx_gamma, d=None, z=None, rows=0):
+    def bn_finalize(bnctx, sums, gidx_gamma, d=None, z=None, rows=0, fold=False):
         kabc = _new(dev, 3, bnctx.C)
-        L.check(lib.mt_bn_bwd_finalize(L.ptr(sums), slots, bnctx.count, L.ptr(P[gidx_gamma]), L.ptr(bnctx.mean_invstd), L.ptr(kabc),
-                                       L.ptr(grads[gidx_gamma]), L.ptr(grads[gidx_gamma + 1]), bnctx.C, tr, st), "mt_bn_bwd_finalize")
+        fn, what = (lib.mt_bn_bwd_finalize_fold, "mt_bn_bwd_finalize_fold") if fold else (lib.mt_bn_bwd_finalize, "mt_bn_bwd_finalize")
+        L.check(fn(L.ptr(sums), slots, bnctx.count, L.ptr(P[gidx_gamma]), L.ptr(bnctx.mean_invstd), L.ptr(kabc),
+                   L.ptr(grads[gidx_gamma]), L.ptr(grads[gidx_gamma + 1]), bnctx.C, tr, st), what)
         return kabc
 
-    def act_bwd(din, z, bnctx, dout, rows, hw, act, gate=None, dpool=None, rowscale=None):
+    def act_bwd(din, z, bnctx, dout, rows, hw, act, gidx_gamma, gate=None, dpool=None, rowscale=None):
         sums = pool.take(bnctx.C)
+        kabc = bn_finalize(bnctx, sums, gidx_gamma, fold=True)
         L.check(lib.mt_bn_act_bwd(L.ptr(din), L.ptr(z), L.ptr(bnctx.scale), L.ptr(bnctx.shift), L.ptr(bnctx.mean_invstd), L.ptr(gate),
                                   L.ptr(dpool), L.ptr(rowscale), L.ptr(dout), L.ptr(sums), slots, rows, bnctx.C, hw, act, st),
                 "mt_bn_act_bwd")
-        return sums
+        return kabc
 
     def conv1x1_bwd(du, z, kabc, w, x_in, rows, cout, cin, gw_idx, need_dx_in, res=None, b_pro=None, epi=None, pl=None):
         if pl is not None and epi is None:
@@ -152,8 +154,7 @@
     s_last = blocks[-1].spec
     M = N * s_last.hout * s_last.hout
     du_h = _new(dev, M, arch.HEAD_COUT)
-    sums = act_bwd(dfeat, hd["z"], hd["bn"], du_h, M, 1, 1)
-    kabc = bn_finalize(hd["bn"], sums, ih + 1, du_h, hd["z"], M)
+    kabc = act_bwd(dfeat, hd["z"], hd["bn"], du_h, M, 1, 1, ih + 1)
     dy = conv1x1_bwd(du_h, hd["z"], kabc, P[ih], hd["y_in"], M, arch.HEAD_COUT, arch.HEAD_CIN, ih, lowest < len(blocks),
                      pl=dict(w_p=hd["w_p"], x_p=hd["y_p"]) if hd.get("w_p") is not None else None)
     del du_h
@@ -168,9 +169,8 @@
         hw = s.hout * s.hout
         dc = rec["dc"]
         dyb = _new(dev, M_out, s.cout) if dc is not None else None
-        sums = act_bwd(dy, rec["z_p"], rec["bn_p"], dyb, M_out, hw, 0, rowscale=dc)
+        kabc_p = act_bwd(dy, rec["z_p"], rec["bn_p"], dyb, M_out, hw, 0, ix["p"] + 1, rowscale=dc)
         dsrc = dyb if dc is not None else dy
-        kabc_p = bn_finalize(rec["bn_p"], sums, ix["p"] + 1, dsrc, rec["z_p"], M_out)
         bn_d = rec["bn_d"]
         b_pro = (bn_d.scale, bn_d.shift, rec["gate"], hw)
         dgate, dpre2, dpooled = _new(dev, N, s.cexp), _new(dev, N, s.cexp), _new(dev, N, s.cexp)
@@ -198,6 +198,7 @@
             da = _new(dev, M_out, s.cexp)
             sums = pool.take(s.cexp)
             stage(1, None, rec["gate"], dpooled, bn_d.mean_invstd, da, sums)
+            kabc_d = bn_finalize(bn_d, sums, ix["d"] + 1, da, rec["z_d"], M_out)
         elif se_fused:
             L.zero_(dgate)
             conv1x1_bwd(dsrc, rec["z_p"], kabc_p, P[ix["p"]], rec["z_d"], M_out, s.cout, s.cexp, ix["p"], True, b_pro=b_pro,
@@ -213,6 +214,7 @@
                         epi=[(L.EPI_ACT_BWD, da, dict(C2=rec["z_d"], ldc2=s.cexp, stats=sums, stats_slots=slots,
                                                       epi=(bn_d.scale, bn_d.shift, rec["gate"], dpooled, bn_d.mean_invstd, hw)))])
             need[ix["p"]] = need_save
+            kabc_d = bn_finalize(bn_d, sums, ix["d"] + 1, da, rec["z_d"], M_out)
         else:
             da = conv1x1_bwd(dsrc, rec["z_p"], kabc_p, P[ix["p"]], rec["z_d"], M_out, s.cout, s.cexp, ix["p"], True, b_pro=b_pro,
                              pl=dict(w_p=rec["wp_p"], x_p=rec["a_p"]) if rec.get("wp_p") is not None else None)
@@ -220,8 +222,7 @@
             if any(need[se:se + 4]):
                 run["wgrad_launches"] += 1
                 side.launch(lambda: se_part(2), reads=(dpre2, dhid, rec["hidden"], rec["pooled"]))
-            sums = act_bwd(da, rec["z_d"], bn_d, da, M_out, hw, 1, gate=rec["gate"], dpool=dpooled)
-        kabc_d = bn_finalize(bn_d, sums, ix["d"] + 1, da, rec["z_d"], M_out)
+            kabc_d = act_bwd(da, rec["z_d"], bn_d, da, M_out, hw, 1, ix["d"] + 1, gate=rec["gate"], dpool=dpooled)
         in_bn = rec["dw_bn"]
         du_in = _new(dev, M_in, s.cexp)
         sums_in = pool.take(s.cexp)
@@ -236,6 +237,10 @@
                                       L.ptr(_bn.scale), L.ptr(_bn.shift), L.ptr(_bn.mean_invstd), L.ptr(_du_in), L.ptr(_sums), slots,
                                       L.ptr(grads[_ix["d"]]), N, _s.hin, _s.hin, _s.cexp, _s.k, _s.s, parts, 1, None, None, L.stream_ptr()),
                     "mt_dwconv_bwd")
+        kabc_in = []
+        def dw_data(parts, _bn=in_bn, _sums=sums_in, _g=(ix["e"] if s.has_expand else 0) + 1, _out=kabc_in):
+            _out.append(bn_finalize(_bn, _sums, _g, fold=True))
+            dw_part(parts)
         need_du_in = need_below[bi] or (s.has_expand and any(need[ix["e"]:ix["e"] + 3]))
         dw_src = rec["y_in"] if rec.get("rc") else rec["dw_in"]
         dw_bytes = (4.0 * (s.cexp * (2 * M_out + M_in) + s.cin * M_in) if rec.get("rc") else 4.0 * s.cexp * (2 * M_out + 2 * M_in))
@@ -244,19 +249,19 @@
                 run["wgrad_launches"] += 1
                 side.launch(lambda: dw_part(1), reads=(da, rec["z_d"], kabc_d, dw_src, in_bn.scale, in_bn.shift))
             if need_du_in:
-                L.timed("dwconv_dgrad", lambda: dw_part(2), dw_bytes)
+                L.timed("dwconv_dgrad", lambda: dw_data(2), dw_bytes)
         elif not rec.get("rc") and (fused_dw == "1" or (fused_dw == "3" and s.k == 3)):
             run["wgrad_launches"] += 1
-            L.timed("dwconv_dgrad", lambda: dw_part(3), 4.0 * s.cexp * (2 * M_out + 2 * M_in))
+            L.timed("dwconv_dgrad", lambda: dw_data(3), 4.0 * s.cexp * (2 * M_out + 2 * M_in))
         else:
             run["wgrad_launches"] += 1
             side.launch(lambda: dw_part(1), reads=(da, rec["z_d"], kabc_d, dw_src, in_bn.scale, in_bn.shift))
-            L.timed("dwconv_dgrad", lambda: dw_part(2), dw_bytes)
+            L.timed("dwconv_dgrad", lambda: dw_data(2), dw_bytes)
         del da
         if not need_du_in:
             dy = None
         elif s.has_expand:
-            kabc_e = bn_finalize(in_bn, sums_in, ix["e"] + 1, du_in, rec["dw_in"], M_in)
+            kabc_e = kabc_in[0]
             z_e = rec["z_e"]
             if z_e is None and not (expand_fused and need[ix["e"]] and need_below[bi] and M_in >= 100000
                                     and lib.mt_conv1x1_bwd_fused_supported(s.cexp, s.cin)):
@@ -266,7 +271,7 @@
                              res=dy if s.skip else None,
                              pl=dict(w_p=rec["we_p"], x_p=rec["y_p"]) if rec.get("we_p") is not None else None)
         else:
-            kabc0 = bn_finalize(in_bn, sums_in, 1, du_in, rec["dw_in"], M_in)
+            kabc0 = kabc_in[0]
             stem = saved["stem"]
             run["stem_run"] = True
             if need[0]:
diff --git a/mintime-multi-identity-size-invariant-timesformer-for-video-deepfake-detection_amd/effnet_engine.py b/mintime-multi-identity-size-invariant-timesformer-for-video-deepfake-detection_amd/effnet_engine.py
--- a/mintime-multi-identity-size-invariant-timesformer-for-video-deepfake-detection_amd/effnet_engine.py
+++ b/mintime-multi-identity-size-invariant-timesformer-for-video-deepfake-detection_amd/effnet_engine.py
@@ -55,11 +55,12 @@
         return v
 
 
-def _finalize(lib, st, bn_mod, ctx, count, training, gamma, beta, slots=SLOTS):
+def _finalize(lib, st, bn_mod, ctx, count, training, gamma, beta, slots=SLOTS, fold=False):
     ctx.count = float(count)
-    L.check(lib.mt_bn_finalize(L.ptr(ctx.stats), slots, float(count), L.ptr(gamma), L.ptr(beta), L.ptr(bn_mod.running_mean),
-                               L.ptr(bn_mod.running_var), L.ptr(ctx.scale), L.ptr(ctx.shift), L.ptr(ctx.mean_invstd), ctx.C,
-                               bn_mod.eps, bn_mod.momentum, 1 if training else 0, st), "mt_bn_finalize")
+    fn, what = (lib.mt_bn_finalize_fold, "mt_bn_finalize_fold") if fold else (lib.mt_bn_finalize, "mt_bn_finalize")
+    L.check(fn(L.ptr(ctx.stats), slots, float(count), L.ptr(gamma), L.ptr(beta), L.ptr(bn_mod.running_mean),
+               L.ptr(bn_mod.running_var), L.ptr(ctx.scale), L.ptr(ctx.shift), L.ptr(ctx.mean_invstd), ctx.C,
+               bn_mod.eps, bn_mod.momentum, 1 if training else 0, st), what)
     if training:
         _track(bn_mod.num_batches_tracked)
 
@@ -225,13 +226,16 @@
         w_d, g, b = next(it), next(it), next(it)
         bn_d = _BNCtx(dev, s.cexp, training, pool)
         z_d = _new(dev, M_out, s.cexp)
+        if training:
+            _finalize(lib, st, blk._bn1, bn_d, M_out, training, g, b, slots, fold=True)
         if rc_on:
             L.check(lib.mt_dwconv_fwd_rc(L.ptr(y), L.ptr(w_e), s.cin, L.ptr(dw_bn.scale), L.ptr(dw_bn.shift), L.ptr(w_d), L.ptr(z_d),
                                          sptr(bn_d), slots, N, s.hin, s.hin, s.cexp, s.k, s.s, st), "mt_dwconv_fwd_rc")
         else:
             L.check(lib.mt_dwconv_fwd(L.ptr(dw_in), L.ptr(dw_bn.scale), L.ptr(dw_bn.shift), L.ptr(w_d), L.ptr(z_d), sptr(bn_d),
                                       slots, N, s.hin, s.hin, s.cexp, s.k, s.s, 1, st), "mt_dwconv_fwd")
-        _finalize(lib, st, blk._bn1, bn_d, M_out, training, g, b, slots)
+        if not training:
+            _finalize(lib, st, blk._bn1, bn_d, M_out, training, g, b, slots)
         w_r, b_r, w_x, b_x = next(it), next(it), next(it), next(it)
         pooled, gate = _new(dev, N, s.cexp), _new(dev, N, s.cexp)
         hidden = _new(dev, N, s.cse)
diff --git a/mintime-multi-identity-size-invariant-timesformer-for-video-deepfake-detection_amd/lib.py b/mintime-multi-identity-size-invariant-timesformer-for-video-deepfake-detection_amd/lib.py
--- a/mintime-multi-identity-size-invariant-timesformer-for-video-deepfake-detection_amd/lib.py
+++ b/mintime-multi-identity-size-invariant-timesformer-for-video-deepfake-detection_amd/lib.py
@@ -93,6 +93,8 @@
     "mt_dwconv_bwd_rc": [f32p] * 6 + [C.c_int] + [f32p] * 4 + [C.c_void_p, C.c_int, f32p] + [C.c_int] * 7 + [C.c_void_p],
     "mt_bn_finalize": [C.c_void_p, C.c_int, C.c_double, f32p, f32p, f32p, f32p, f32p, f32p, f32p, C.c_int, C.c_float,
                        C.c_float, C.c_int, C.c_void_p],
+    "mt_bn_finalize_fold": [C.c_void_p, C.c_int, C.c_double, f32p, f32p, f32p, f32p, f32p, f32p, f32p, C.c_int, C.c_float,
+                            C.c_float, C.c_int, C.c_void_p],
     "mt_se_pool_parts": [C.c_int, C.c_int, C.c_int],
     "mt_se_pool_fwd": [f32p, f32p, f32p, f32p, C.c_int, C.c_int, C.c_int, C.c_int, C.c_void_p],
     "mt_se_gate_fwd": [f32p, C.c_int, f32p, f32p, f32p, f32p, f32p, f32p, f32p, C.c_int, C.c_int, C.c_int, C.c_void_p],
@@ -113,6 +115,7 @@
                     C.c_void_p, C.c_void_p],
     "mt_bn_act_bwd": [f32p] * 9 + [C.c_void_p, C.c_int, i64, C.c_int, C.c_int, C.c_int, C.c_void_p],
     "mt_bn_bwd_finalize": [C.c_void_p, C.c_int, C.c_double, f32p, f32p, f32p, f32p, f32p, C.c_int, C.c_int, C.c_void_p],
+    "mt_bn_bwd_finalize_fold": [C.c_void_p, C.c_int, C.c_double, f32p, f32p, f32p, f32p, f32p, C.c_int, C.c_int, C.c_void_p],
     "mt_se_bwd": [f32p] * 17 + [C.c_int, C.c_int, C.c_int, C.c_int, C.c_int, f32p, C.c_void_p],
     "mt_se_scratch_floats": [C.c_int, C.c_int, C.c_int],
     "mt_dwconv_bwd": [f32p] * 9 + [C.c_void_p, C.c_int, f32p, C.c_int, C.c_int, C.c_int, C.c_int, C.c_int, C.c_int, C.c_int,
@@ -198,7 +201,7 @@
     return LIB_PATH
 
 
-ABI_VERSION = 121
+ABI_VERSION = 122
 
 
 def header_version() -> int:
```

Result: slower. 692.7 clips/s (-2.2%).
